# cristianpjensen/thesis-pai-reconstruction

Hardware: AMD Instinct MI355X
Metric: train images/sec (256x256, bs=64) Pix2Pix step (higher is better)
Workload: dtype bf16; 1 GPU; Pix2Pix generator+PatchGAN GAN step, 256x256x1 pairs, 64 images/GPU (BASELINE configs[1]); global_batch=64, per_gpu_batch=64, loss_type=gan, parallelism=dp1, grad_bucket_dtype=f32

## Files before the change

### include/pai_hip.h

```cpp
#ifndef PAI_HIP_H
#define PAI_HIP_H

#include <stdint.h>

#ifdef __cplusplus
extern "C" {
#endif

#define PAI_F32 0
#define PAI_BF16 1
#define PAI_U8 2

#define PAI_ACT_NONE 0
#define PAI_ACT_LRELU 1
#define PAI_ACT_RELU 2
#define PAI_ACT_TANH 3
#define PAI_ACT_SILU 4

const char* pai_last_error(void);
int pai_version(void);
int pai_build_flags(void);
int pai_device_info(int* cu_count, int* lds_bytes, char* arch_name, int arch_name_len);

#define PAI_TUNABLE_UNSET (-2147483647 - 1)
int pai_set_tunable(const char* name, int value);
int pai_get_tunable(const char* name, int default_value);

int64_t pai_order_dependent_launches(void);

typedef struct pai_conv_desc {
    int32_t dtype;
    int32_t transposed;
    int32_t N, H, W;
    int32_t C1, C2;
    int32_t Cout;
    int32_t kernel;
    int32_t stride;
    int32_t pad;
    int32_t relu1, relu2;
    int32_t epilogue_act;
    int32_t groups;
    int32_t pack_flags;
    int32_t hints;
} pai_conv_desc;
#define PAI_HINT_SOLO 1

int pai_conv_out_hw(const pai_conv_desc* d, int* OH, int* OW);
int pai_conv_fwd_stats_rows(const pai_conv_desc* d);
int pai_conv_fwd_stats_rows_max(const pai_conv_desc* d);
int pai_bn_stats_buffer_rows(int rows);

int pai_conv_kernel_id(const pai_conv_desc* d, int op);
int pai_conv_kernel_name(const pai_conv_desc* d, int op, char* name, int name_len);

int pai_create(int device_id, void** handle_out);
int pai_bind(void* handle);
int pai_destroy(void* handle);
int pai_handle_set_workspace(void* handle, void* zeroed_device_memory, int64_t bytes);
int pai_handle_set_scratch(void* handle, void* device_memory, int64_t bytes);
int pai_handle_set_wgrad_workspace(void* handle, void* device_memory, int64_t bytes);

int pai_set_workspace(void* zeroed_device_memory, int64_t bytes);
int64_t pai_conv_workspace_bytes(const pai_conv_desc* d, int op);
int pai_set_scratch(void* device_memory, int64_t bytes);
int64_t pai_conv_scratch_bytes(const pai_conv_desc* d, int op);
int pai_set_wgrad_workspace(void* device_memory, int64_t bytes);
int64_t pai_conv_wgrad_workspace_bytes(const pai_conv_desc* d);
int pai_conv_wgrad_order_free(const pai_conv_desc* d, int has_dbias);

int pai_conv_fwd(const pai_conv_desc* d, const void* x1, const void* x2, const void* w_fwd,
                 const float* bias, void* y_raw, void* y_act, float* y_f32, float* stats,
                 void* stream);

int pai_conv_dgrad(const pai_conv_desc* d, const void* dy, const void* w_dgrad, void* dx1,
                   void* dx2, int only_c2, void* stream);

int pai_conv_dgrad_f32add_ok(const pai_conv_desc* d);
int pai_conv_dgrad_f32add(const pai_conv_desc* d, const void* dy, const void* w_dgrad, const float* addend,
                          float* dx2_f32, void* stream);

int pai_conv_dgrad_act(const pai_conv_desc* d, const void* dy, const void* w_dgrad, void* dx1,
                       void* dx2, const void* a1, int act1, void* stream);

int pai_conv_dgrad_act_wthin_ok(const pai_conv_desc* d, const pai_conv_desc* d_thin, int need_dx);
int pai_conv_dgrad_act_wthin_order_free(const pai_conv_desc* d, const pai_conv_desc* d_thin);
int64_t pai_conv_dgrad_act_wthin_slab_bytes(const pai_conv_desc* d, const pai_conv_desc* d_thin);
int pai_conv_dgrad_act_wthin_kernel_name(const pai_conv_desc* d, const pai_conv_desc* d_thin, char* name, int name_len);
int pai_conv_dgrad_act_wthin(const pai_conv_desc* d, const void* dy, const void* w_dgrad, const void* a1, int act1,
                             const void* add, int act2, const pai_conv_desc* d_thin, const void* x1, const void* x2,
                             float* dw, float* dbias, int overwrite, float* slabs, int64_t slab_bytes, void* stream);

typedef struct pai_bwd_epilogue {
    const void* z;
    const void* add;
    const float* scale;
    const float* shift;
    const float* mean;
    const float* rstd;
    float* partials;
    int32_t act1, act2;
} pai_bwd_epilogue;
int pai_conv_dgrad_bn_rows_max(const pai_conv_desc* d);
int pai_conv_dgrad_bn(const pai_conv_desc* d, const void* dy, const void* w_dgrad, void* dx1,
                      void* dx2, const pai_bwd_epilogue* e, int* partial_rows, void* stream);

typedef struct pai_bn_train {
// ... 108 lines not shown

int pai_gate_partial_rows(int64_t M);
int pai_gate_hidden(int dtype, const void* ig, const void* sg, int64_t M, int K, const float* scale_i,
                    const float* shift_i, const float* scale_s, const float* shift_s, const float* w_a,
                    const float* b_a, void* h, float* logit, float* partials, void* stream);
int pai_gate_apply(int dtype, const void* x, const float* logit, int64_t M, int C, const float* scale_a,
                   const float* shift_a, void* out, float* att, void* stream);
int pai_gate_apply_bwd(int dtype, const void* dout, const void* x, const float* att, const float* logit,
                       int64_t M, int C, const float* mean_a, const float* rstd_a, void* dx_skip, float* dl,
                       float* partials, int relu_out, void* stream);
int pai_gate_hidden_bwd(int dtype, const float* dl, const float* logit, const void* h, const void* ig,
                        const void* sg, int64_t M, int K, const float* mean_a, const float* rstd_a,
                        const float* gamma_a, const float* sums_a, const float* w_a, const float* mean_i,
                        const float* rstd_i, const float* mean_s, const float* rstd_s, void* dsum,
                        float* partials_i, float* partials_s, float* dw_a, float* db_a, void* stream);
int64_t pai_gate_scratch_bytes(int64_t M, int K);

int pai_bce_logits(const float* logits, int64_t numel, float target, float loss_scale,
                   double* loss, float grad_scale, float* grad, void* stream);
int pai_l1(const float* pred, const float* target, int64_t numel, float loss_scale, double* loss,
           float grad_scale, float* grad, void* stream);
int pai_mse(const float* pred, const float* target, int64_t numel, float loss_scale, double* loss,
            float grad_scale, float* grad, void* stream);
int pai_head_loss_ok(const pai_conv_desc* d, int has_bias);
int pai_head_loss(const pai_conv_desc* d, const void* a3, const void* w_fwd, const void* w_dgrad, int n_first,
                  float target_first, float target_rest, float loss_scale, double* loss, float grad_scale,
                  float* logits, void* dl, float* dl_f32, void* du, const void* act_src, int act, void* stream);
int pai_scalar_take(double* acc, float* out, void* stream);
int pai_metrics_take(double* sums, int64_t n_images, int64_t numel, float* out3, void* stream);
int pai_tanh_bwd(int dtype, const float* pred, const float* g_a, const float* g_b, int64_t numel,
                 void* dh, void* stream);

int pai_denormalize(const float* x, const float* grad_out_or_null, int64_t numel, float* out,
                    void* stream);

int pai_ssim_sse(const float* pred, const float* target, int NC, int H, int W, int denorm,
                 double* out2, double* per_image, float* full_map, void* stream);
int pai_ssim_psnr_bwd(const float* pred, const float* target, int NC, int H, int W, int denorm,
                      float w_ssim, float w_psnr, const double* sse, float* grad, float* workspace,
                      void* stream);
int64_t pai_ssim_bwd_workspace_floats(int NC, int H, int W);
int pai_eval_planes(const float* pred, const float* target, int NC, int H, int W, int denorm,
                    double* ssim_plane, double* sse_plane, unsigned char* ssim_map_u8,
                    const unsigned char* lut_rgb, unsigned char* hot_u8, void* stream);
int pai_eval_kernel_name(int op, char* name, int name_len);

int pai_cast(int src_dtype, const void* src, int dst_dtype, void* dst, int64_t numel, void* stream);
int pai_reduce_rows(const float* partial, int rows, int C, float* out, int accumulate, void* stream);
int pai_adam(float* param, const float* grad, float* exp_avg, float* exp_avg_sq, int64_t numel,
             float lr, float beta1, float beta2, float eps, int step_count, void* stream);
int pai_adam_pack(float* param, const float* grad, float* exp_avg, float* exp_avg_sq, int64_t numel, int64_t w_off,
                  int Cout, int taps, int Cin, void* w_fwd, void* w_dgrad, float lr, float beta1, float beta2, float eps,
                  int step_count, void* stream);
int pai_adam_dev(float* param, const float* grad, float* exp_avg, float* exp_avg_sq, int64_t numel,
                 float lr, float beta1, float beta2, float eps, int64_t* step_dev, float* coeff2_dev, void* stream);
int pai_adam_multi(int count, void* const* params, const void* const* grads, void* const* exp_avgs,
                   void* const* exp_avg_sqs, const int64_t* numels, float lr, float beta1, float beta2, float eps,
                   int step_count, void* stream);
int pai_adam_multi_dev(int count, void* const* params, const void* const* grads, void* const* exp_avgs,
                       void* const* exp_avg_sqs, const int64_t* numels, float lr, float beta1, float beta2, float eps,
                       int64_t* step_dev, float* coeff2_dev, void* stream);

#define PAI_COMM_ID_BYTES 128
int pai_comm_unique_id(void* id_out_host);
int pai_comm_init(const void* id_host, int rank, int world, void** comm_out);
int pai_allreduce(void* comm, void* ptr, int64_t count, int dtype, void* stream);
int pai_comm_destroy(void* comm);

typedef struct pai_plan_s* pai_plan_t;
int pai_plan_create(pai_plan_t* out);
int pai_plan_destroy(pai_plan_t plan);
int pai_plan_begin(pai_plan_t plan);
int pai_plan_end(pai_plan_t plan);
int pai_plan_run(pai_plan_t plan, int64_t step_delta);
int pai_plan_info(pai_plan_t plan, int* launches, int* waits, int* streams, int64_t* runs);
int pai_stream_wait(void* waiting_stream, void* signalling_stream);
int pai_stream_wait_last(void* waiting_stream, void* signalling_stream);
typedef struct pai_event_s* pai_event_t;
int pai_event_create(pai_event_t* out);
int pai_event_destroy(pai_event_t ev);
int pai_event_record(pai_event_t ev, void* stream);
int pai_event_create_timing(pai_event_t* out);
int pai_event_elapsed_ms(pai_event_t start, pai_event_t stop, float* ms_host);
int pai_profile_arm(pai_event_t start, pai_event_t stop);
int pai_stream_wait_event(void* waiting_stream, pai_event_t ev);
int pai_zero_multi(int count, void* const* ptrs, const int64_t* numels, void* stream);
int pai_cast_multi(int count, int src_dtype, const void* const* srcs, int dst_dtype, void* const* dsts,
                   const int64_t* numels, void* stream);
int pai_lerp_multi(int count, void* const* dsts, const void* const* srcs, const int64_t* numels, float weight, void* stream);

int pai_filter_to_dense(const float* w_oihw, int Cout, int Cin_per_group, int taps, int groups, float* dense, void* stream);
int pai_filter_grad_from_dense(const float* dense_dw, int Cout, int Cin_per_group, int taps, int groups, float* dw_oihw,
                               void* stream);

int pai_swap_mid(int elem_bytes, const void* src, int64_t A, int B, int C, int64_t D, void* dst, void* stream);
int pai_scale(float* ptr, int64_t numel, float factor, void* stream);

int pai_resize_aa_u8(const void* src, int n, int H, int W, int S, const int* wbounds, const float* wweights, int KW,
                     const int* hbounds, const float* hweights, int KH, const int* hbounds_host, void* dst, void* stream);
int pai_batch_gather(int src_dtype, const void* cache_a, const void* cache_b, int64_t M, int64_t per_image,
                     const int64_t* indices, int count, const float* table, float* out_a, float* out_b, void* stream);
int pai_data_kernel_name(int op, int src_dtype, char* name, int name_len);

int pai_sattn_fwd(int dtype, const void* qkv, int N, int T, int heads, int ch, void* out, void* stream);
int pai_sattn_fwd_lse(int dtype, const void* qkv, int N, int T, int heads, int ch, void* out, float* lse, void* stream);
int pai_sattn_bwd(int dtype, const void* dout, const void* qkv, const void* out, const float* lse, int N, int T, int heads,
// ... 68 lines not shown
```

### thesis-pai-reconstruction_amd/attention.py

```python
from __future__ import annotations

import torch
import torch.nn as nn

from . import ops
from .engine import GradArena, UnetEngine, _BNState, _Packs, _bn_forward, to_fwd_pack_, wthin_slabs
from .ops import ACT_LRELU, ACT_NONE, ACT_RELU, ACT_TANH


class _Gate:

    def __init__(self, block: nn.Module, gen):
        self.conv_i, self.bn_i = block.input_gate[0], block.input_gate[1]
        self.conv_s, self.bn_s = block.signal_gate[0], block.signal_gate[1]
        self.conv_a, self.bn_a = block.attention[0], block.attention[1]
        self.C = self.conv_i.weight.shape[1]
        self.K = self.conv_i.weight.shape[0]
        self.pack_i = _Packs(self.conv_i, need_dgrad=True, gen=gen)
        self.pack_s = _Packs(self.conv_s, need_dgrad=True, gen=gen)

    def ordered_params(self):
        return [(self.conv_a.weight, None), (self.conv_a.bias, None), (self.bn_a.weight, None), (self.bn_a.bias, None),
                (self.bn_i.weight, None), (self.bn_i.bias, None), (self.bn_s.weight, None), (self.bn_s.bias, None),
                (self.conv_i.weight, None), (self.conv_i.bias, None), (self.conv_s.weight, None),
                (self.conv_s.bias, None)]


class AttentionUnetEngine(UnetEngine):
    overwrites_weight_grads = True

    def __init__(self, unet: nn.Module):
        super().__init__(unet)
        self.gates = [_Gate(b, self.weights_generation) for b in unet.attention_blocks]
        assert len(self.gates) == self.L - 1

    def all_packs(self):
        return self.enc_packs + self.dec_packs + [pk for g in self.gates for pk in (g.pack_i, g.pack_s)]

    def _gate(self, j):
        return self.gates[j - 1]

    def ordered_params(self):
        out = []
        L = self.L
        for j in range(L - 1, -1, -1):
            if self.dec_bn[j] is not None:
                out += [(self.dec_bn[j].weight, None), (self.dec_bn[j].bias, None)]
            out += [(self.dec_conv[j].weight, self.dec_conv[j]), (self.dec_conv[j].bias, None)]
            if j >= 1:
                out += self._gate(j).ordered_params()
        for i in range(L - 1, -1, -1):
            if self.enc_bn[i] is not None:
                out += [(self.enc_bn[i].weight, None), (self.enc_bn[i].bias, None)]
            out += [(self.enc_conv[i].weight, self.enc_conv[i]), (self.enc_conv[i].bias, None)]
        return out

    def _plan(self, N, H, W, dtype, device):
        key = (N, H, W, dtype, str(device))
        if key in self._plans:
            return self._plans[key]
        P = super()._plan(N, H, W, dtype, device)
        L = self.L
        eh, ew = P["eh"], P["ew"]
        P["dec_desc"] = []
        for j in range(L):
            hin, win = eh[L - 1 - j], ew[L - 1 - j]
            if j == 0:
                c1, c2, r1, r2 = self.enc_c[L - 1], 0, 1, 0
            else:
                c1, c2, r1, r2 = self.dec_c[j - 1], self.enc_c[L - 1 - j], 1, 1
            act = ACT_NONE
            if j == L - 1:
                r1, r2, act = 0, 0, ACT_TANH
            P["dec_desc"].append(ops.make_desc(dtype, 1, N, hin, win, c1, c2, self.dec_c[j], 2, r1, r2, act))
        P["gate_desc"] = [None]
        rows = P["stats"].numel()
        mx = P["bwd_partials"].numel()
        for j in range(1, L):
            g = self._gate(j)
            lvl = L - 1 - j
            d = ops.make_desc(dtype, 0, N, eh[lvl], ew[lvl], g.C, 0, g.K, 1, 0, 0, ACT_NONE, kernel=1)
            P["gate_desc"].append(d)
            M = N * eh[lvl] * ew[lvl]
            rows = max(rows, ops.bn_stats_buffer_rows(ops.conv_fwd_stats_rows_max(d)) * 2 * g.K,
                       ops.bn_stats_buffer_rows(ops.gate_partial_rows(M)) * 2)
            mx = max(mx, ops.gate_partial_rows(M) * 2 * g.K, ops.conv_dgrad_bn_rows_max(d) * 2 * g.C)
        P["stats"] = torch.empty(rows, dtype=torch.float32, device=device)
        P["bwd_partials"] = torch.empty(mx, dtype=torch.float32, device=device)
        P["bwd_partials2"] = torch.empty(mx, dtype=torch.float32, device=device)
        ops.ensure_workspace(max(ops.conv_workspace_bytes(d, op) for d in P["dec_desc"] + P["gate_desc"][1:]
                                 for op in (0, 1)), device)
        ops.ensure_scratch(ops.scratch_bytes_for(P["enc_desc"] + P["dec_desc"]), device)
        ops.ensure_wgrad_workspace(P["enc_desc"] + P["dec_desc"], device)
        return P

    def _new_slot(self, P):
        S = super()._new_slot(P)
        L, N, dt, dev = self.L, P["N"], P["dtype"], P["device"]
        eh, ew = P["eh"], P["ew"]
        S["b"] = [None] + [torch.empty_like(S["z"][i]) if i < L - 1 else None for i in range(1, L)]
        S["gate"] = [None]
        for j in range(1, L):
            g = self._gate(j)
            lvl = L - 1 - j
            M = N * eh[lvl] * ew[lvl]
            f32 = dict(dtype=torch.float32, device=dev)
            S["gate"].append({
                "M": M,
                "ig": torch.empty(M * g.K, dtype=dt, device=dev), "sg": torch.empty(M * g.K, dtype=dt, device=dev),
                "h": torch.empty(M * g.K, dtype=dt, device=dev), "s": torch.empty(M * g.C, dtype=dt, device=dev),
                "logit": torch.empty(M, **f32), "att": torch.empty(M, **f32),
# ... 84 lines not shown
        for j in range(L):
            wf, _ = self.dec_packs[j].get(dtype)
            d = P["dec_desc"][j]
            if j == 0:
                x1, x2 = S["z"][L - 1], None
            else:
                x1 = S["r"][j - 1]
                x2 = self._gate_forward(S, j, self._skip(S, L - 1 - j), x1, training, bn_updates, dtype)
            if j < L - 1:
                bn = self.dec_bn[j]
                M = N * S["dh"][j] * S["dw"][j]
                if training:
                    rows = ops.conv_fwd_stats_rows(d)
                    ops.conv_fwd(d, x1, x2, wf, self.dec_conv[j].bias, y_raw=S["w"][j], stats=P["stats"])
                    _bn_forward(bn, S["dbn"][j], P["stats"], rows, M, True, bn_updates)
                else:
                    ops.conv_fwd(d, x1, x2, wf, self.dec_conv[j].bias, y_raw=S["w"][j])
                    _bn_forward(bn, S["dbn"][j], None, 0, M, False, 0)
                ops.bn_apply(dtype, S["w"][j], M, self.dec_c[j], S["dbn"][j].scale, S["dbn"][j].shift, ACT_NONE,
                             S["r"][j])
                if training and self.dec_drop[j] > 0:
                    self._dropout(S, j, M, self.dec_c[j], dtype)
            else:
                S["pred"] = torch.empty_like(S["pred"])
                ops.conv_fwd(d, x1, x2, wf, self.dec_conv[j].bias, y_f32=S["pred"])
        pred = S["pred"]
        if self.out_ch != 1:
            pred = pred.view(N, H, W, self.out_ch).permute(0, 3, 1, 2)
        return pred, S

    def backward(self, S, gpred: torch.Tensor, fresh: bool = False):
        P = S["P"]
        L, N, dtype = self.L, P["N"], P["dtype"]
        eh, ew = P["eh"], P["ew"]
        G = self._grad_bufs(S)
        A = self.arena()
        hook = self.grad_ready_hook
        if self.out_ch != 1:
            gpred = gpred.permute(0, 2, 3, 1)
        gpred = gpred.contiguous()
        if gpred.dtype != torch.float32:
            gpred = gpred.float()
        side = self._side
        part, part2 = P["bwd_partials"], P["bwd_partials2"]

        def done(p):
            if hook is not None:
                hook(A, A.end_of(p))

        def wgrad(d, x1, x2, dz, conv, with_bias, last=None):
            cin, cout = conv.weight.shape[1], conv.weight.shape[0]
            dense = fresh and conv.weight.shape[2] == 4 and min(cin, cout) > 2
            with torch.cuda.stream(side.fork(d)):
                (ops.conv_wgrad_overwrite_w if dense else ops.conv_wgrad)(
                    d, x1, x2, dz, A.seg(conv.weight), A.seg(conv.bias) if with_bias else None)
                done(last if last is not None else conv.bias)

        def gate_backward(j, relu_out):
            g, gs = self._gate(j), S["gate"][j]
            d, M = P["gate_desc"][j], gs["M"]
            lvl = L - 1 - j
            x, signal = self._skip(S, lvl), S["r"][j - 1]
            ba, bi, bs = gs["bn_a"], gs["bn_i"], gs["bn_s"]
            ops.gate_apply_bwd(dtype, G["gs"][j], x, gs["att"], gs["logit"], M, g.C, ba.mean, ba.rstd, G["dxs"][j],
                               G["dl"][j], part, relu_out)
            ops.bn_bwd_finalize(part, ops.gate_partial_rows(M), 1, ba.sums, A.seg(g.bn_a.weight), A.seg(g.bn_a.bias))
            ops.gate_hidden_bwd(dtype, G["dl"][j], gs["logit"], gs["h"], gs["ig"], gs["sg"], M, g.K, ba.mean, ba.rstd,
                                g.bn_a.weight, ba.sums, g.conv_a.weight, bi.mean, bi.rstd, bs.mean, bs.rstd,
                                G["dsum"][j], part, part2, A.seg(g.conv_a.weight), A.seg(g.conv_a.bias))
            rows = ops.gate_partial_rows(M)
            ops.bn_bwd_finalize(part, rows, g.K, bi.sums, A.seg(g.bn_i.weight), A.seg(g.bn_i.bias))
            ops.bn_bwd_finalize(part2, rows, g.K, bs.sums, A.seg(g.bn_s.weight), A.seg(g.bn_s.bias))
            ops.bn_bwd_apply(dtype, G["dsum"][j], gs["ig"], M, g.K, bi.mean, bi.rstd, g.bn_i.weight, bi.sums, G["dig"][j])
            ops.bn_bwd_apply(dtype, G["dsum"][j], gs["sg"], M, g.K, bs.mean, bs.rstd, g.bn_s.weight, bs.sums, G["dsg"][j])
            wgrad(d, x, None, G["dig"][j], g.conv_i, False)
            wgrad(d, signal, None, G["dsg"][j], g.conv_s, False)
            _, wd_i = g.pack_i.get(dtype)
            _, wd_s = g.pack_s.get(dtype)
            ops.conv_dgrad_bn(d, G["dig"][j], wd_i, G["gx"][j], None, x, ACT_NONE, G["dxs"][j], ACT_NONE)
            pst = S["dbn"][j - 1]
            if (j - 1) in S["drop"]:
                ops.conv_dgrad_bn(d, G["dsg"][j], wd_s, G["gr"][j - 1], None, S["r"][j - 1], ACT_NONE,
                                  G["gr_raw"][j - 1], ACT_RELU if relu_out else ACT_NONE)
                ops.dropout2d(dtype, G["gr"][j - 1], S["drop"][j - 1], N, S["dh"][j - 1] * S["dw"][j - 1],
                              self.dec_c[j - 1], G["gr"][j - 1])
                return None
            return ops.conv_dgrad_bn(d, G["dsg"][j], wd_s, G["gr"][j - 1], None, S["w"][j - 1], ACT_NONE,
                                     G["gr_raw"][j - 1], ACT_RELU if relu_out else ACT_NONE, pst.scale, pst.shift,
                                     pst.mean, pst.rstd, part)

        j = L - 1
        dh = G["dz_head"]
        ops.tanh_bwd(dtype, S["pred"], gpred, None, dh)
        d = P["dec_desc"][j]
        wgrad(d, S["r"][j - 1], S["gate"][j]["s"], dh, self.dec_conv[j], True)
        side.mark_scratch()
        _, wd = self.dec_packs[j].get(dtype)
        ops.conv_dgrad(d, dh, wd, G["gr_raw"][j - 1], G["gs"][j])
        fused_rows = gate_backward(j, relu_out=False)
        for j in range(L - 2, -1, -1):
            bn, st, conv = self.dec_bn[j], S["dbn"][j], self.dec_conv[j]
            M = N * S["dh"][j] * S["dw"][j]
            C = self.dec_c[j]
            dz = G["dz_dec"][j]
            du = G["gr"][j]
            if fused_rows is None:
                du = G["du"][:M * C]
                ops.bn_bwd_reduce(dtype, G["gr"][j], ACT_NONE, None, ACT_NONE, None, S["w"][j], M, C, st.mean, st.rstd,
                                  du, part, st.sums, A.seg(bn.weight), A.seg(bn.bias))
            else:
                ops.bn_bwd_finalize(part, fused_rows, C, st.sums, A.seg(bn.weight), A.seg(bn.bias))
            ops.bn_bwd_apply(dtype, du, S["w"][j], M, C, st.mean, st.rstd, bn.weight, st.sums, dz)
            d = P["dec_desc"][j]
            _, wd = self.dec_packs[j].get(dtype)
            if j == 0:
                wgrad(d, S["z"][L - 1], None, dz, conv, False)
                fused_rows = ops.conv_dgrad_bn(d, dz, wd, G["dz_enc"][L - 1], None, S["z"][L - 1], ACT_RELU)
            else:
                wgrad(d, S["r"][j - 1], S["gate"][j]["s"], dz, conv, False)
                ops.conv_dgrad(d, dz, wd, G["gr_raw"][j - 1], G["gs"][j])
                fused_rows = gate_backward(j, relu_out=True)
        i = L - 1
        dz = G["dz_enc"][i]
        wgrad(P["enc_desc"][i], S["a"][i - 1], None, dz, self.enc_conv[i], True)
        _, wd = self.enc_packs[i].get(dtype)

        enc0_fused = ops.conv_dgrad_act_wthin_ok(P["enc_desc"][1], P["enc_desc"][0], False)

        def enc_dgrad(i, dz, wd):
            d = P["enc_desc"][i]
            gx = G["gx"][L - 1 - (i - 1)]
            if i - 1 == 0 and enc0_fused:
                c0, d0 = self.enc_conv[0], P["enc_desc"][0]
                ops.conv_dgrad_act_wthin(d, dz, wd, S["z"][0], ACT_LRELU, gx, ACT_NONE, d0, S["x"], None,
                                         A.seg(c0.weight), A.seg(c0.bias), wthin_slabs(P, d, d0))
                return 0
            if i - 1 == 0:
                if G["dz_enc"][0] is None:
                    G["dz_enc"][0] = torch.empty_like(S["z"][0])
                return ops.conv_dgrad_bn(d, dz, wd, G["dz_enc"][0], None, S["z"][0], ACT_LRELU, gx, ACT_NONE)
            pst = S["ebn"][i - 1]
            return ops.conv_dgrad_bn(d, dz, wd, G["ga"][i - 1], None, S["z"][i - 1], ACT_LRELU, gx, ACT_NONE,
                                     pst.scale, pst.shift, pst.mean, pst.rstd, part)

        fused_rows = enc_dgrad(i, dz, wd)
        for i in range(L - 2, 0, -1):
            bn, st, conv = self.enc_bn[i], S["ebn"][i], self.enc_conv[i]
            M = N * eh[i] * ew[i]
            C = self.enc_c[i]
            du, dz = G["ga"][i], G["dz_enc"][i]
            ops.bn_bwd_finalize(part, fused_rows, C, st.sums, A.seg(bn.weight), A.seg(bn.bias))
            ops.bn_bwd_apply(dtype, du, S["z"][i], M, C, st.mean, st.rstd, bn.weight, st.sums, dz)
            wgrad(P["enc_desc"][i], S["a"][i - 1], None, dz, conv, False)
            _, wd = self.enc_packs[i].get(dtype)
            fused_rows = enc_dgrad(i, dz, wd)
        conv0 = self.enc_conv[0]
        if not enc0_fused:
            with torch.cuda.stream(side.fork_tail()):
                c0_in, c0_out = conv0.weight.shape[1], conv0.weight.shape[0]
                (ops.conv_wgrad_overwrite_w if (fresh and min(c0_in, c0_out) > 2) else ops.conv_wgrad)(
                    P["enc_desc"][0], S["x"], None, G["dz_enc"][0], A.seg(conv0.weight), A.seg(conv0.bias))
        side.join()
        done(conv0.bias)
```

### thesis-pai-reconstruction_amd/csrc/api.hip

```cpp
#include <stdarg.h>

#include "common.h"

static thread_local char g_err[512] = "";

void pai_set_error(const char* fmt, ...) {
    va_list ap;
    va_start(ap, fmt);
    vsnprintf(g_err, sizeof(g_err), fmt, ap);
    va_end(ap);
}

extern "C" const char* pai_last_error(void) { return g_err; }
extern "C" int pai_version(void) { return 141; }

extern "C" int pai_build_flags(void) { return 0; }

extern "C" int pai_device_info(int* cu_count, int* lds_bytes, char* arch_name, int arch_name_len) {
    int dev = 0;
    hipError_t e = hipGetDevice(&dev);
    PAI_CHECK(e == hipSuccess, "hipGetDevice: %s", hipGetErrorString(e));
    hipDeviceProp_t p;
    e = hipGetDeviceProperties(&p, dev);
    PAI_CHECK(e == hipSuccess, "hipGetDeviceProperties: %s", hipGetErrorString(e));
// ... 120 lines not shown
    g->S = S;
    g->nphase = 1;
    g->ntaps = 16;
    g->OS = 1;
    g->poy[0] = g->pox[0] = 0;
    for (int kh = 0; kh < 4; ++kh)
        for (int kw = 0; kw < 4; ++kw) {
            int t = kh * 4 + kw;
            g->dy[0][t] = (signed char)(kh + off0);
            g->dx[0][t] = (signed char)(kw + off0);
            g->wt[0][t] = (signed char)t;
        }
}

static void fill_pointwise(GG* g) {
    g->S = 1; g->nphase = 1; g->ntaps = 1; g->OS = 1; g->wtaps = 1;
    g->poy[0] = g->pox[0] = 0;
    g->dy[0][0] = g->dx[0][0] = g->wt[0][0] = 0;
}

static void fill_3x3(GG* g, int sign) {
    g->S = 1; g->nphase = 1; g->ntaps = 9; g->OS = 1; g->wtaps = 9;
    g->poy[0] = g->pox[0] = 0;
    for (int kh = 0; kh < 3; ++kh)
        for (int kw = 0; kw < 3; ++kw) {
            const int t = kh * 3 + kw;
            g->dy[0][t] = (signed char)(sign * (kh - 1));
            g->dx[0][t] = (signed char)(sign * (kw - 1));
            g->wt[0][t] = (signed char)t;
        }
}

static void fill_phase_taps(GG* g) {
    g->S = 1;
    g->nphase = 4;
    g->ntaps = 4;
    g->OS = 2;
    for (int ph = 0; ph < 2; ++ph)
        for (int pw = 0; pw < 2; ++pw) {
            int p = ph * 2 + pw;
            g->poy[p] = (signed char)ph;
            g->pox[p] = (signed char)pw;
            int khs[2], offy[2], kws[2], offx[2];
            phase_taps(ph, khs, offy);
            phase_taps(pw, kws, offx);
            for (int a = 0; a < 2; ++a)
                for (int b = 0; b < 2; ++b) {
                    int t = a * 2 + b;
                    g->dy[p][t] = (signed char)offy[a];
                    g->dx[p][t] = (signed char)offx[b];
                    g->wt[p][t] = (signed char)(khs[a] * 4 + kws[b]);
                }
        }
}

int gg_build_fwd(const pai_conv_desc* d, GG* g) {
    if (check_desc(d)) return 1;
    memset(g, 0, sizeof(*g));
    g->N = d->N; g->H = d->H; g->W = d->W;
    g->C1 = d->C1; g->C2 = d->C2; g->Cin = d->C1 + d->C2;
    g->Cout = d->Cout;
    g->D1 = d->Cout; g->D2 = 0;
    g->wtaps = 16;
    g->gslice = d->groups > 1 ? 16 : 0;
    g->solo = (d->hints & PAI_HINT_SOLO) ? 1 : 0;
    g->relu1 = d->relu1; g->relu2 = d->relu2;
    int OH, OW;
    pai_conv_out_hw(d, &OH, &OW);
    g->OH = OH; g->OW = OW;
    if (d->kernel == 1) {
        g->OHg = OH; g->OWg = OW;
        fill_pointwise(g);
    } else if (d->kernel == 3) {
        g->OHg = OH; g->OWg = OW;
        fill_3x3(g, +1);
    } else if (!d->transposed) {
        g->OHg = OH; g->OWg = OW;
        fill_conv_taps(g, d->stride, -d->pad);
    } else {
        g->OHg = d->H; g->OWg = d->W;
        fill_phase_taps(g);
    }
    finish_gg(g);
    return 0;
}

int gg_build_dgrad(const pai_conv_desc* d, GG* g) {
    if (check_desc(d)) return 1;
    memset(g, 0, sizeof(*g));
    int OH, OW;
    pai_conv_out_hw(d, &OH, &OW);
    g->N = d->N; g->H = OH; g->W = OW;
    g->C1 = d->Cout; g->C2 = 0; g->Cin = d->Cout;
    g->Cout = d->C1 + d->C2;
    g->D1 = d->C1; g->D2 = d->C2;
    g->wtaps = 16;
    g->gslice = d->groups > 1 ? 16 : 0;
    g->OH = d->H; g->OW = d->W;
    if (d->kernel == 1) {
        g->OHg = d->H; g->OWg = d->W;
        fill_pointwise(g);
    } else if (d->kernel == 3) {
        g->OHg = d->H; g->OWg = d->W;
        fill_3x3(g, -1);
    } else if (!d->transposed) {
        if (d->stride == 2) {
            g->OHg = d->H / 2; g->OWg = d->W / 2;
            fill_phase_taps(g);
        } else {
            g->OHg = d->H; g->OWg = d->W;
            g->S = 1; g->nphase = 1; g->ntaps = 16; g->OS = 1;
            for (int kh = 0; kh < 4; ++kh)
                for (int kw = 0; kw < 4; ++kw) {
                    int t = kh * 4 + kw;
                    g->dy[0][t] = (signed char)(d->pad - kh);
                    g->dx[0][t] = (signed char)(d->pad - kw);
                    g->wt[0][t] = (signed char)t;
                }
        }
    } else {
        g->OHg = d->H; g->OWg = d->W;
        fill_conv_taps(g, 2, -d->pad);
    }
    finish_gg(g);
    return 0;
}

static void finish_gg(GG* g) {
    g->M = g->N * g->OHg * g->OWg;
    auto lg = [](int v) { int l = 0; while ((1 << l) < v) ++l; return (1 << l) == v ? l : -1; };
    g->lw = lg(g->OWg);
    g->lh = lg(g->OHg);
    if (g->lw < 0 || g->lh < 0) g->lw = g->lh = -1;
    g->lsw = lg(g->W); g->lsh = lg(g->H); g->ldw = lg(g->OW); g->ldh = lg(g->OH);
    if (g->lw < 0 || g->lsw < 0 || g->lsh < 0 || g->ldw < 0 || g->ldh < 0)
        g->lsw = g->lsh = g->ldw = g->ldh = -1;
}

constexpr int PAI_MAX_DEVICES = 64;
static pai_handle_s* g_active[PAI_MAX_DEVICES];
static const pai_handle_s g_empty_handle = {-1, nullptr, 0, nullptr, 0, nullptr, 0};

static int current_device() {
    int dev = 0;
    return hipGetDevice(&dev) == hipSuccess && dev >= 0 && dev < PAI_MAX_DEVICES ? dev : -1;
}

const pai_handle_s* pai_ctx() {
    const int dev = current_device();
    return dev >= 0 && g_active[dev] ? g_active[dev] : &g_empty_handle;
}

extern "C" int pai_create(int device_id, void** handle_out) {
    PAI_CHECK(handle_out != nullptr, "pai_create: null handle_out");
    PAI_CHECK(device_id >= 0 && device_id < PAI_MAX_DEVICES, "pai_create: device id %d out of range", device_id);
    pai_handle_s* h = new pai_handle_s{device_id, nullptr, 0, nullptr, 0, nullptr, 0};
    if (!g_active[device_id]) g_active[device_id] = h;
    *handle_out = h;
    return 0;
}

extern "C" int pai_bind(void* handle) {
    PAI_CHECK(handle != nullptr, "pai_bind: null handle");
    pai_handle_s* h = (pai_handle_s*)handle;
    g_active[h->device] = h;
    return 0;
}

extern "C" int pai_destroy(void* handle) {
    PAI_CHECK(handle != nullptr, "pai_destroy: null handle");
    pai_handle_s* h = (pai_handle_s*)handle;
    if (g_active[h->device] == h) g_active[h->device] = nullptr;
    delete h;
    return 0;
}

// ... 191 lines not shown
    memset(&a, 0, sizeof(a));
    a.y1 = (void*)1;
    if (op == 1 && g.D2 > 0) a.y2 = (void*)1;
    return a;
}

extern "C" int64_t pai_conv_wgrad_workspace_bytes(const pai_conv_desc* d) {
    GG g;
    if (gg_build_fwd(d, &g)) return -1;
    return pick_wgrad(d->dtype, g, false, false).workspace_bytes;
}

extern "C" int pai_conv_wgrad_order_free(const pai_conv_desc* d, int has_dbias) {
    GG g;
    if (!d || gg_build_fwd(d, &g)) return 0;
    return pick_wgrad(d->dtype, g, has_dbias != 0, false).order_free ? 1 : 0;
}

extern "C" int64_t pai_conv_workspace_bytes(const pai_conv_desc* d, int op) {
    GG g;
    if (op == 1 ? gg_build_dgrad(d, &g) : gg_build_fwd(d, &g)) return -1;
    return op == 2 ? 0 : pick_fwd(d->dtype, g, query_args(g, op)).workspace_bytes;
}

extern "C" int64_t pai_conv_scratch_bytes(const pai_conv_desc* d, int op) {
    GG g;
    if (op == 1 ? gg_build_dgrad(d, &g) : gg_build_fwd(d, &g)) return -1;
    return op == 2 ? pick_wgrad(d->dtype, g, false, false).scratch_bytes : pick_fwd(d->dtype, g, query_args(g, op)).scratch_bytes;
}

extern "C" int pai_conv_fwd_stats_rows(const pai_conv_desc* d) {
    GG g;
    if (gg_build_fwd(d, &g)) return -1;
    FwdArgs a = query_args(g, 0);
    a.stats = (float*)1;
    return pick_fwd(d->dtype, g, a).rows;
}

extern "C" int pai_conv_kernel_id(const pai_conv_desc* d, int op) {
    GG g;
    if (op == 1 ? gg_build_dgrad(d, &g) : gg_build_fwd(d, &g)) return -1;
    return op == 2 ? pick_wgrad(d->dtype, g, false, false).id : pick_fwd(d->dtype, g, query_args(g, op)).id;
}

extern "C" int pai_conv_kernel_name(const pai_conv_desc* d, int op, char* name, int name_len) {
    GG g;
    if ((op == 1 ? gg_build_dgrad(d, &g) : gg_build_fwd(d, &g)) || !name || name_len <= 0) return -1;
    const char* n = op == 2 ? pick_wgrad(d->dtype, g, false, false).name : pick_fwd(d->dtype, g, query_args(g, op)).name;
    strncpy(name, n, name_len - 1);
    name[name_len - 1] = 0;
    return 0;
}

extern "C" int pai_conv_fwd_stats_rows_max(const pai_conv_desc* d) {
    GG g;
    if (gg_build_fwd(d, &g)) return -1;
    return cdiv(g.M, 16) * g.nphase;
}

extern "C" int pai_conv_fwd(const pai_conv_desc* d, const void* x1, const void* x2,
                            const void* w_fwd, const float* bias, void* y_raw, void* y_act,
                            float* y_f32, float* stats, void* stream) {
    GG g;
    if (gg_build_fwd(d, &g)) return 1;
    PAI_CHECK(x1 && w_fwd, "pai_conv_fwd: null x1 / w");
    PAI_CHECK(d->C2 == 0 || x2, "pai_conv_fwd: C2 > 0 but x2 is null");
    PAI_CHECK(y_raw || y_act || y_f32, "pai_conv_fwd: no output requested");
    FwdArgs a;
    memset(&a, 0, sizeof(a));
    a.x1 = x1; a.x2 = x2; a.w = w_fwd; a.bias = bias;
    a.y1 = y_raw; a.y2 = nullptr; a.yact = y_act; a.yf32 = y_f32; a.stats = stats;
    a.eact = d->epilogue_act;
    return run_fwd(d->dtype, g, a, (hipStream_t)stream);
}

static int conv_wgrad_impl(const pai_conv_desc* d, const void* x1, const void* x2, const void* dy, float* dw,
                           float* dbias, int overwrite, void* stream, const float* pscale = nullptr,
                           const float* pshift = nullptr, int pact = 0);

extern "C" int pai_conv_prologue_ok(const pai_conv_desc* d) {
    GG g;
    if (gg_build_fwd(d, &g)) return 0;
    FwdArgs a = query_args(g, 0);
    a.pscale = a.pshift = (const float*)1;
    a.pact = PAI_ACT_RELU;
    return pick_fwd(d->dtype, g, a).k != FK_NONE && pick_wgrad(d->dtype, g, false, true).k != WK_NONE;
}

extern "C" int pai_conv_fwd_pro(const pai_conv_desc* d, const void* x1, const void* w_fwd, const float* bias, void* y_raw,
                                float* stats, const float* pre_scale, const float* pre_shift, int pre_act, void* stream) {
    GG g;
    if (gg_build_fwd(d, &g)) return 1;
    PAI_CHECK(x1 && w_fwd && y_raw && pre_scale && pre_shift, "pai_conv_fwd_pro: null pointer");
    PAI_CHECK(pre_act == PAI_ACT_NONE || pre_act == PAI_ACT_RELU, "pai_conv_fwd_pro: pre_act=%d (none or ReLU)", pre_act);
    PAI_CHECK(d->C2 == 0, "pai_conv_fwd_pro: one source tensor only");
    FwdArgs a;
    memset(&a, 0, sizeof(a));
    a.x1 = x1; a.w = w_fwd; a.bias = bias;
    a.y1 = y_raw;
    a.stats = stats;
    a.pscale = pre_scale; a.pshift = pre_shift; a.pact = pre_act;
    return run_fwd(d->dtype, g, a, (hipStream_t)stream);
}

extern "C" int pai_conv_wgrad_pro(const pai_conv_desc* d, const void* x1, const void* dy, float* dw, float* dbias,
                                  int overwrite, const float* pre_scale, const float* pre_shift, int pre_act, void* stream) {
// ... 262 lines not shown
                                       e->rstd, gamma, dz, s);
    if (int rc = pai_bn_bwd_finalize(e->partials, rows, g.D1, sums, dgamma, dbeta, stream)) return rc;
    return pai_bn_bwd_apply(d->dtype, du_scratch, e->z, Mo, g.D1, e->mean, e->rstd, gamma, sums, dz, stream);
}


extern "C" int pai_conv_wgrad(const pai_conv_desc* d, const void* x1, const void* x2,
                              const void* dy, float* dw, float* dbias, void* stream) {
    return conv_wgrad_impl(d, x1, x2, dy, dw, dbias, 0, stream);
}

extern "C" int pai_conv_wgrad_overwrite(const pai_conv_desc* d, const void* x1, const void* x2,
                                        const void* dy, float* dw, float* dbias, void* stream) {
    return conv_wgrad_impl(d, x1, x2, dy, dw, dbias, 1, stream);
}

extern "C" int pai_conv_wgrad_overwrite_w(const pai_conv_desc* d, const void* x1, const void* x2,
                                          const void* dy, float* dw, float* dbias, void* stream) {
    return conv_wgrad_impl(d, x1, x2, dy, dw, dbias, 2, stream);
}

static int conv_wgrad_impl(const pai_conv_desc* d, const void* x1, const void* x2, const void* dy, float* dw,
                           float* dbias, int overwrite, void* stream, const float* pscale, const float* pshift, int pact) {
    GG g;
    if (gg_build_fwd(d, &g)) return 1;
    PAI_CHECK(x1 && dy && dw, "pai_conv_wgrad: null pointer");
    PAI_CHECK(d->C2 == 0 || x2, "pai_conv_wgrad: C2 > 0 but x2 is null");
    WgradArgs a;
    a.x1 = x1; a.x2 = x2; a.dy = dy; a.dw = dw; a.dbias = dbias; a.overwrite = 0; a.overwrite_bias = 0; a.slab = nullptr;
    a.pscale = pscale; a.pshift = pshift; a.pact = pact;
    hipStream_t s = (hipStream_t)stream;
    const WgradPick p = pick_wgrad(d->dtype, g, dbias != nullptr, pscale != nullptr);
    PAI_CHECK(p.k != WK_NONE, "pai_conv_wgrad_pro: this layer takes no prologue (ask pai_conv_prologue_ok: the grouped 3 x 3 weight "
                              "gradient needs its workspace, pai_set_wgrad_workspace)");
    float* bias_rows = nullptr;
    if (pai_deterministic()) {
        const pai_handle_s* h = pai_ctx();
        const bool thin = p.k >= WK_THIN_CONV && p.k <= WK_THIN_CONV3T;
        PAI_CHECK(!thin || (h->scratch && h->scratch_bytes >= p.scratch_bytes),
                  "pai_conv_wgrad: deterministic mode needs %lld bytes of scratch for the partial tiles of this thin layer "
                  "(pai_set_scratch; pai_conv_scratch_bytes, op 2)", (long long)p.scratch_bytes);
        const int64_t dwb = (int64_t)g.Cout * g.wtaps * g.Cin * 4;
        const int64_t slabs = p.k == WK_GROUPED3 ? grouped3_wgrad_part_bytes(g)
                              : (p.k == WK_MFMA && p.mfma.variant < WGRAD_PATCH128 && p.mfma.ksplit > 1) ? p.mfma.ksplit * dwb : 0;
        const int64_t rows = p.colsum_bias ? p.bias_part_bytes : 0;
        const int64_t have = h->wslab ? h->wslab_bytes & ~(int64_t)3 : 0;
        PAI_CHECK(slabs + rows == 0 || have >= slabs + rows,
                  "pai_conv_wgrad: deterministic mode needs %lld bytes of weight-gradient workspace (%lld for the pixel-split slabs, "
                  "%lld for the partial rows of the bias gradient; pai_set_wgrad_workspace, pai_conv_wgrad_workspace_bytes)",
                  (long long)(slabs + rows), (long long)slabs, (long long)rows);
        if (rows) bias_rows = (float*)((char*)h->wslab + (have - rows));
    }
    if (overwrite && p.overwrites) {
        a.overwrite = 1;
        a.overwrite_bias = p.k != WK_GROUPED3 && overwrite == 1;
    } else if (overwrite) {
        hipError_t e = pai::memset_async(dw, 0, (size_t)g.Cout * g.wtaps * g.Cin * sizeof(float), s);
        PAI_CHECK(e == hipSuccess, "pai_conv_wgrad_overwrite: hipMemsetAsync: %s", hipGetErrorString(e));
        if (dbias && overwrite == 1) {
            e = pai::memset_async(dbias, 0, (size_t)g.Cout * sizeof(float), s);
            PAI_CHECK(e == hipSuccess, "pai_conv_wgrad_overwrite: hipMemsetAsync: %s", hipGetErrorString(e));
        }
    }
    if (!p.order_free) pai_note_order_dependent();
    if (p.colsum_bias) {
        if (int rc = launch_colsum_det(d->dtype, dy, (int64_t)g.N * g.OH * g.OW, g.Cout, dbias, overwrite != 1, bias_rows, s)) return rc;
        a.dbias = nullptr;
    }
    switch (p.k) {
        case WK_GROUPED3: return launch_grouped3_wgrad(g, a, p.part, s);
        case WK_THIN_CONV: return launch_thin_wgrad_conv(g, a, s);
        case WK_THIN_CONVT: return launch_thin_wgrad_convt(g, a, s);
        case WK_THIN_CONV1: return launch_thin_wgrad_conv1(g, a, s);
        case WK_THIN_CONV3: return launch_thin_wgrad_conv3(g, a, s);
        case WK_THIN_CONV3T: return launch_thin_wgrad_conv3t(g, a, s);
        case WK_ROWDOT: return launch_wgrad_rowdot(d->dtype, g, a, s);
        case WK_MFMA: return launch_wgrad_mfma(g, a, p.mfma, s);
        default: return launch_wgrad_simt(d->dtype, g, a, s);
    }
}
```

### thesis-pai-reconstruction_amd/csrc/common.h

```cpp
#pragma once
#include <hip/hip_runtime.h>
#include <stdint.h>
#include <stdio.h>
#include <string.h>

#include "../../include/pai_hip.h"
#include "plan.h"

typedef unsigned short bf16_t;

void pai_set_error(const char* fmt, ...);

#define PAI_CHECK(cond, ...)                 \
    do {                                     \
        if (!(cond)) {                       \
            pai_set_error(__VA_ARGS__);      \
            return 1;                        \
        }                                    \
    } while (0)

#define PAI_LAUNCH_CHECK()                                              \
    do {                                                                \
        hipError_t e_ = hipGetLastError();                              \
        if (e_ != hipSuccess) {                                         \
// ... 68 lines not shown
__device__ __forceinline__ float act_apply(float v, int act) {
    switch (act) {
        case PAI_ACT_LRELU: return v > 0.f ? v : 0.2f * v;
        case PAI_ACT_RELU: return !(v <= 0.f) ? v : 0.f;
        case PAI_ACT_TANH: return tanhf(v);
        default: return v;
    }
}
__device__ __forceinline__ float act_grad(float a, int act) {
    switch (act) {
        case PAI_ACT_LRELU: return a > 0.f ? 1.f : 0.2f;
        case PAI_ACT_RELU: return a > 0.f ? 1.f : 0.f;
        default: return 1.f;
    }
}

__device__ __forceinline__ float wave_sum(float v) {
#pragma unroll
    for (int o = 32; o > 0; o >>= 1) v += __shfl_xor(v, o, 64);
    return v;
}

static inline int cdiv(int64_t a, int64_t b) { return (int)((a + b - 1) / b); }

struct PerDeviceOnce {
    bool done[32] = {};
    bool first() {
        int dev = 0;
        if (hipGetDevice(&dev) != hipSuccess || dev < 0 || dev >= 32) return true;
        if (done[dev]) return false;
        done[dev] = true;
        return true;
    }
};

struct GG {
    int N, H, W;
    int C1, C2, Cin;
    int OHg, OWg;
    int Cout;
    int S;
    int nphase, ntaps;
    int OH, OW, OS;
    int D1, D2;
    int wtaps;
    int relu1, relu2;
    int M;
    int lw, lh;
    int lsw, lsh, ldw, ldh;
    signed char dy[4][16], dx[4][16], wt[4][16];
    signed char poy[4], pox[4];
    int gslice;
    int solo;
};

struct PatchGeo {
    int groups;
    int TY, TX;
    signed char by[4][4], bx[4][4];
    unsigned toff4[4][4];
    unsigned wt4[4][4];
    unsigned wt_lo[4], wt_hi[4], toff2[4];
};

int gg_build_fwd(const pai_conv_desc* d, GG* g);
int gg_build_dgrad(const pai_conv_desc* d, GG* g);

struct FwdArgs {
    const void *x1, *x2, *w;
    const float* bias;
    void *y1, *y2;
    void* yact;
    float* yf32;
    float* stats;
    int eact;
    int skip_d1;
    const void* bz;
    const void* badd;
    const float *bscale, *bshift, *bmean, *brstd;
    int bact1, bact2;
    float* bpart;
    const float *pscale, *pshift;
    int pact;
};
bool bn_fuse_small_ok(int rows, int64_t M, int C);
int launch_bn_fin_apply(int dtype, const float* stats, int rows, int C, int64_t count, const float* gamma, const float* beta,
                        float eps, float momentum, int n_updates, float* running_mean, float* running_var, int64_t* nbt,
                        float* mean, float* rstd, float* scale, float* shift, const void* z, int act, void* out,
                        hipStream_t s);
int launch_bn_bwd_fin_apply(int dtype, const float* partials, int rows, int C, float* sums, float* dgamma, float* dbeta,
                            const void* du, const void* z, int64_t M, const float* mean, const float* rstd,
                            const float* gamma, void* dz, hipStream_t s);
int ew_stream_bn_apply(int dtype, const void* z, int64_t M, int C, const float* scale, const float* shift, int act, void* out,
                       hipStream_t s);
int ew_stream_bn2_add_act(int dtype, const void* za, const float* sca, const float* sha, const void* zb, const float* scb,
                          const float* shb, int64_t M, int C, int act_a, int act, void* out, hipStream_t s);
int ew_stream_add_act(int dtype, const void* a, const void* b, int64_t numel, int act, void* out, hipStream_t s);
int ew_stream_bn_bwd_reduce(int dtype, const void* g, int act, const void* z, int64_t M, int C, const float* scale,
                            const float* shift, const float* mean, const float* rstd, float* partials, int rows, hipStream_t s);
int ew_stream_bn_bwd_apply(int dtype, const void* g, int act, const void* z, int64_t M, int C, const float* scale,
                           const float* shift, const float* mean, const float* rstd, const float* gamma, const float* sums,
                           void* dz, hipStream_t s);
int ew_stream_bn2_bwd_reduce(int dtype, const void* d, int act_a, const void* za, const void* zb, int64_t M, int C,
                             const float* scale_a, const float* shift_a, const float* mean_a, const float* rstd_a,
                             const float* mean_b, const float* rstd_b, float* part_a, float* part_b, int rows, hipStream_t s);
int ew_stream_bn2_bwd_apply(int dtype, const void* d, int act_a, const void* za, const void* zb, int64_t M, int C,
                            const float* scale_a, const float* shift_a, const float* mean_a, const float* rstd_a,
// ... 31 lines not shown
int launch_fwd_mfma(const GG& g, const FwdArgs& a, const MfmaPlan& p, hipStream_t s, const WThin* wt = nullptr);
int launch_wthin_reduce(const float* slab, int S, int T, float* dw, float* dbias, int overwrite_w, int overwrite_bias, hipStream_t s);
MfmaPlan wgrad_mfma_plan(const GG& g, bool has_dbias, bool has_prologue);
bool wgrad_pro_ok(int dtype, const GG& g);
struct pai_handle_s {
    int device;
    float* workspace;
    int64_t workspace_bytes;
    float* scratch;
    int64_t scratch_bytes;
    float* wslab;
    int64_t wslab_bytes;
};
const pai_handle_s* pai_ctx();
int fwd_simt_mtiles(const GG& g);
bool fwd_mfma_ok(int dtype, const GG& g, const FwdArgs& a);
bool pw_ok(int dtype, const GG& g, const FwdArgs& a);
int pw_rows(const GG& g);
int launch_pw(const GG& g, const FwdArgs& a, hipStream_t s);
bool pwx_ok(int dtype, const GG& g, const FwdArgs& a);
int pwx_rows(const GG& g);
int launch_pwx(const GG& g, const FwdArgs& a, hipStream_t s);
const char* pwx_kernel_name(const GG& g);
bool fwd_rowdot_ok(const GG& g, const FwdArgs& a);
bool small_ok(int dtype, const GG& g, const FwdArgs& a);
int small_rows(const GG& g);
int launch_small(const GG& g, const FwdArgs& a, hipStream_t s);
bool grouped3_ok(int dtype, const GG& g, const FwdArgs& a);
int grouped3_rows(const GG& g);
int launch_grouped3(const GG& g, const FwdArgs& a, hipStream_t s);

bool thin_fwd_ok(int dtype, const GG& g, const FwdArgs& a);
bool thin_dgrad_ok(int dtype, const GG& g, const FwdArgs& a);
bool thin_dgrad_shape_ok(int dtype, const GG& g);
int64_t thin_dgrad_scratch_bytes(const GG& g, const FwdArgs& a);
int launch_thin_fwd(const GG& g, const FwdArgs& a, hipStream_t s);
bool head_dgrad_ok(int dtype, const GG& g, const FwdArgs& a);
int launch_head_dgrad(const GG& g, const FwdArgs& a, hipStream_t s);
int thin_fwd_bwd_rows(int dtype, const GG& g, const FwdArgs& a, int act1, const void* add, const float* scale);
int launch_thin_dgrad(const GG& g, const FwdArgs& a, hipStream_t s);
bool thin_up_f32add_ok(int dtype, const GG& g);

struct WgradArgs {
    const void *x1, *x2, *dy;
    float* dw;
    float* dbias;
    int overwrite;
    int overwrite_bias;
    float* slab;
    const float *pscale, *pshift;
    int pact;
};
float* wgrad_slab_acquire(int64_t bytes);
int launch_wgrad_slab_sum(float* dw, const float* slab, int nsplits, int64_t n, int overwrite, hipStream_t s);
bool grouped3_wgrad_ok(int dtype, const GG& g, const float* dbias);
int64_t grouped3_wgrad_part_bytes(const GG& g);
int launch_grouped3_wgrad(const GG& g, const WgradArgs& a, float* part, hipStream_t s);
int launch_eval_planes(const float* pred, const float* target, int NC, int H, int W, int denorm, double* ssim_plane,
                       double* sse_plane, unsigned char* map_u8, const unsigned char* lut_rgb, unsigned char* hot_u8,
                       hipStream_t stream);
const char* eval_planes_kernel_name();
bool wgrad3_ok(const GG& g);
MfmaPlan wgrad3_plan(const GG& g, bool has_dbias);
int launch_wgrad3(const GG& g, const WgradArgs& a, const MfmaPlan& p, hipStream_t s);
int wgrad_simt_splits(const GG& g, int* rows);
int launch_wgrad_simt(int dtype, const GG& g, const WgradArgs& a, hipStream_t s);
int launch_wgrad_rowdot(int dtype, const GG& g, const WgradArgs& a, hipStream_t s);
int launch_wgrad_mfma(const GG& g, const WgradArgs& a, const MfmaPlan& p, hipStream_t s);
bool wgrad_mfma_ok(int dtype, const GG& g);
bool thin_wgrad_conv_ok(int dtype, const GG& g);
bool thin_wgrad_convt_ok(int dtype, const GG& g);
int launch_thin_wgrad_conv(const GG& g, const WgradArgs& a, hipStream_t s);
int launch_thin_wgrad_convt(const GG& g, const WgradArgs& a, hipStream_t s);
bool thin_wgrad_conv1_ok(int dtype, const GG& g);
int launch_thin_wgrad_conv1(const GG& g, const WgradArgs& a, hipStream_t s);
bool thin_wgrad_conv3_ok(int dtype, const GG& g);
int launch_thin_wgrad_conv3(const GG& g, const WgradArgs& a, hipStream_t s);
bool thin_wgrad_conv3t_ok(int dtype, const GG& g);
int launch_thin_wgrad_conv3t(const GG& g, const WgradArgs& a, hipStream_t s);
int64_t thin_wgrad_scratch_bytes(int64_t M, int T, int WC);
```

### thesis-pai-reconstruction_amd/csrc/gg_mfma.hip

```cpp
#include <type_traits>

#include "gg_tile.h"


bool fwd_mfma_ok(int dtype, const GG& g, const FwdArgs& a) {
    if (dtype != PAI_BF16) return false;
    if (g.C1 % 64 || g.C2 % 64) return false;
    if (g.Cout % 64) return false;
    if (g.D2 > 0 && (g.D1 % 64)) return false;
    if (a.yf32) return false;
    if (a.skip_d1) return false;
    if ((a.y1 || a.y2) && a.yact) return false;
    if (a.yact && a.eact != PAI_ACT_NONE && a.eact != PAI_ACT_LRELU && a.eact != PAI_ACT_RELU) return false;
    return true;
}

struct FwdCfg { int bn, ksplit; };

static FwdCfg fwd_cfg(const GG& g) {
    FwdCfg c;
    c.bn = ((g.Cout % 128) == 0 && (g.D2 == 0 || (g.D1 % 128) == 0)) ? 128 : 64;
    c.ksplit = 1;
    const int ntiles = g.Cout / c.bn;
    const int niter = g.ntaps * g.Cin / MBK;
// ... 1035 lines not shown
        p.block = waves * 64;
        const size_t lds = patch_bytes + (size_t)c.bn * 128 * (db ? 2 : 1);
        const size_t epi = prow * ((size_t)c.bn * 2 + 16) + waves * 2 * c.bn * sizeof(float);
        p.lds = lds > epi ? lds : epi;
    } else {
        p.block = p.bm / 64 * 128;
        p.lds = fwd_lds_bytes(p.bm, c.bn, db);
    }
    p.grid = p.mtiles * p.ntiles * g.nphase * c.ksplit;
    return p;
}

bool fwd_mfma_wthin(MfmaPlan* p, int T) {
    if (p->variant != FWD_PATCH128N || p->ntiles != 1 || (T != 1 && T != 2)) return false;
    p->variant = T == 1 ? FWD_WTHIN1 : FWD_WTHIN2;
    p->name = fwd_mfma_names[p->variant];
    const size_t epi = 128 * (64 * 2 + 16) + 4 * 2 * 64 * sizeof(float) + (size_t)T * WTH_XPLANE;
    if (epi > p->lds) p->lds = epi;
    return true;
}

static int fwd_lds_opt_in();
int launch_fwd_mfma(const GG& g, const FwdArgs& a, const MfmaPlan& p, hipStream_t s, const WThin* wt) {
    float* ws = pai_ctx()->workspace;
    const bool wthin = p.variant == FWD_WTHIN1 || p.variant == FWD_WTHIN2;
    PAI_CHECK(wthin == (wt != nullptr), "launch_fwd_mfma: the weight-gradient store and its arguments go together");
    const WThin wta = wt ? *wt : WThin{};
    if (p.lds > 64 * 1024 && fwd_lds_opt_in()) return 1;
#define FWD_LAUNCH_TILE(k, ...) PAI_LAUNCH((k<__VA_ARGS__>), p.grid, p.block, p.lds, s, g, a, p.mtiles, p.ntiles, p.ksplit, ws)
#define FWD_LAUNCH_PATCH(k, ...) PAI_LAUNCH((k<__VA_ARGS__>), p.grid, p.block, p.lds, s, g, a, p.pg, p.mtiles, p.ntiles)
#define FWD_LAUNCH_WTHIN(k, ...) PAI_LAUNCH((k<__VA_ARGS__>), p.grid, p.block, p.lds, s, g, a, p.pg, p.mtiles, p.ntiles, wta)
#define X(id, form, k, ...) case id: FWD_LAUNCH_##form(k, __VA_ARGS__); break;
    switch (p.variant) { FWD_MFMA_VARIANTS(X) }
#undef X
#undef FWD_LAUNCH_TILE
#undef FWD_LAUNCH_PATCH
#undef FWD_LAUNCH_WTHIN
    PAI_LAUNCH_CHECK();
    if (p.ksplit > 1)
        PAI_LAUNCH(splitk_finish_k, dim3(p.rows, g.nphase, cdiv(g.Cout, FIN_COLS)), dim3(256), 0, s, g, a, ws, p.rows, p.ksplit);
    PAI_LAUNCH_CHECK();
    return 0;
}
static int fwd_lds_opt_in() {
    static PerDeviceOnce attr_set;
    if (!attr_set.first()) return 0;
    const hipError_t e = hipFuncSetAttribute(reinterpret_cast<const void*>(&gg_fwd_patch_k<256, 128, true>),
                                             hipFuncAttributeMaxDynamicSharedMemorySize, 80 * 1024);
    PAI_CHECK(e == hipSuccess, "hipFuncSetAttribute(max dynamic LDS): %s", hipGetErrorString(e));
    return 0;
}

bool pw_ok(int dtype, const GG& g, const FwdArgs& a) {
    if (dtype != PAI_BF16 || g.ntaps != 1 || g.nphase != 1 || g.C2 != 0 || g.D2 != 0) return false;
    if (!((g.C1 == 64 && g.Cout == 32) || (g.C1 == 32 && g.Cout == 64))) return false;
    if (a.yf32 || a.skip_d1) return false;
    if ((a.y1 != nullptr) == (a.yact != nullptr)) return false;
    if (a.yact && a.eact != PAI_ACT_NONE && a.eact != PAI_ACT_LRELU && a.eact != PAI_ACT_RELU) return false;
    return true;
}

int pw_rows(const GG& g) {
    int64_t b = ((int64_t)g.M + 63) / 64;
    return (int)(b > 2048 ? 2048 : (b < 1 ? 1 : b));
}

template <int CIN, int COUT>
__global__ __launch_bounds__(256) void pw_k(GG g, FwdArgs a, int groups_per_wave) {
    constexpr int KB = CIN / 32, NTT = COUT / 16, CL = COUT / 4, NCH = CL / 8;
    __shared__ float sred[4][2][COUT];
    const int tid = threadIdx.x, lane = tid & 63, wid = tid >> 6;
    const int fr = lane & 15, fq = lane >> 4;
    const bf16_t* x = (const bf16_t*)a.x1;
    const bf16_t* w = (const bf16_t*)a.w;
    bf16_t* y = (bf16_t*)(a.yact ? a.yact : a.y1);
    const float eslope = act_slope(a.yact ? a.eact : PAI_ACT_NONE);
    bf8_t wf[NTT][KB];
#pragma unroll
    for (int nt = 0; nt < NTT; ++nt)
#pragma unroll
        for (int kb = 0; kb < KB; ++kb)
            wf[nt][kb] = *(const bf8_t*)(w + (size_t)(CL * (fr >> 2) + 4 * nt + (fr & 3)) * CIN + kb * 32 + fq * 8);
    const int c0 = CL * fq;
    float bias_v[CL], s1[CL], s2[CL];
#pragma unroll
    for (int c = 0; c < CL; ++c) { bias_v[c] = a.bias ? a.bias[c0 + c] : 0.f; s1[c] = s2[c] = 0.f; }
    const bool bwd = a.bz != nullptr && !a.yact;
    const bool bsum = bwd && a.bpart;
    const bf16_t* bzp = (const bf16_t*)a.bz;
    const bf16_t* bap = (const bf16_t*)a.badd;
    BwdParams BP[NCH];
    if (bwd) {
#pragma unroll
        for (int h = 0; h < NCH; ++h) bwd_load_params(a, c0 + 8 * h, BP[h]);
    }
    const int64_t ngroups = ((int64_t)g.M + 15) / 16;
    const int64_t g0 = ((int64_t)blockIdx.x * 4 + wid) * groups_per_wave;
    for (int64_t gi = g0; gi < g0 + groups_per_wave && gi < ngroups; ++gi) {
        const int64_t pix = gi * 16 + fr;
        const bool valid = pix < g.M;
        const int64_t pc = valid ? pix : 0;
        bf8_t xb[KB];
#pragma unroll
        for (int kb = 0; kb < KB; ++kb) {
            xb[kb] = *(const bf8_t*)(x + pc * CIN + kb * 32 + fq * 8);
            if (g.relu1) xb[kb] = relu_frag(xb[kb]);
        }
// ... 25 lines not shown
            }
            pk[2 * nt] = pk2bf(v[0], v[1]);
            pk[2 * nt + 1] = pk2bf(v[2], v[3]);
        }
#pragma unroll
        for (int h = 0; h < NCH; ++h) {
            uint4 o = make_uint4(pk[4 * h], pk[4 * h + 1], pk[4 * h + 2], pk[4 * h + 3]);
            if (bwd && valid)
                o = bwd_chunk(o, zq[h], aq[h], bap != nullptr, a.bscale != nullptr, bsum, a.bact1, a.bact2, BP[h],
                              s1 + 8 * h, s2 + 8 * h);
            if (valid) *(uint4*)(y + pix * COUT + c0 + 8 * h) = o;
        }
    }
    float* prow = a.stats ? a.stats : (bsum ? a.bpart : nullptr);
    if (prow) {
#pragma unroll
        for (int c = 0; c < CL; ++c) {
            float u = s1[c], q = s2[c];
            u += __builtin_bit_cast(float, __builtin_amdgcn_update_dpp(0, __builtin_bit_cast(int, u), 0xB1, 0xF, 0xF, false));
            q += __builtin_bit_cast(float, __builtin_amdgcn_update_dpp(0, __builtin_bit_cast(int, q), 0xB1, 0xF, 0xF, false));
            u += __builtin_bit_cast(float, __builtin_amdgcn_update_dpp(0, __builtin_bit_cast(int, u), 0x4E, 0xF, 0xF, false));
            q += __builtin_bit_cast(float, __builtin_amdgcn_update_dpp(0, __builtin_bit_cast(int, q), 0x4E, 0xF, 0xF, false));
            u += __builtin_bit_cast(float, __builtin_amdgcn_update_dpp(0, __builtin_bit_cast(int, u), 0x141, 0xF, 0xF, false));
            q += __builtin_bit_cast(float, __builtin_amdgcn_update_dpp(0, __builtin_bit_cast(int, q), 0x141, 0xF, 0xF, false));
            u += __builtin_bit_cast(float, __builtin_amdgcn_update_dpp(0, __builtin_bit_cast(int, u), 0x140, 0xF, 0xF, false));
            q += __builtin_bit_cast(float, __builtin_amdgcn_update_dpp(0, __builtin_bit_cast(int, q), 0x140, 0xF, 0xF, false));
            if (fr == 0) { sred[wid][0][c0 + c] = u; sred[wid][1][c0 + c] = q; }
        }
        __syncthreads();
        if (tid < COUT) {
            float u = 0.f, q = 0.f;
#pragma unroll
            for (int wv = 0; wv < 4; ++wv) { u += sred[wv][0][tid]; q += sred[wv][1][tid]; }
            float* dst = prow + (size_t)blockIdx.x * 2 * COUT;
            dst[tid] = u;
            dst[COUT + tid] = a.stats ? q : a.brstd[tid] * (q - a.bmean[tid] * u);
        }
    }
}

int launch_pw(const GG& g, const FwdArgs& a, hipStream_t s) {
    const int blocks = pw_rows(g);
    const int64_t ngroups = ((int64_t)g.M + 15) / 16;
    const int gpw = (int)((ngroups + (int64_t)blocks * 4 - 1) / ((int64_t)blocks * 4));
    if (g.C1 == 64) PAI_LAUNCH((pw_k<64, 32>), dim3(blocks), dim3(256), 0, s, g, a, gpw);
    else PAI_LAUNCH((pw_k<32, 64>), dim3(blocks), dim3(256), 0, s, g, a, gpw);
    PAI_LAUNCH_CHECK();
    return 0;
}

bool wgrad_mfma_ok(int dtype, const GG& g) {
    if (dtype != PAI_BF16) return false;
    if (g.lsw < 0) return false;
    if (g.ntaps == 1 && g.C2 == 0 && ((g.C1 == 64 && g.Cout == 32) || (g.C1 == 32 && g.Cout == 64))) return true;
    if (g.ntaps == 1 && g.C2 == 0 && g.C1 == 64 && (g.Cout % 64) == 0) return true;
    if (g.nphase == 1 && g.S == 1 && g.C2 == 0 && (g.C1 % 8) == 0 && (g.Cout % 8) == 0 && (g.C1 < 64 || g.Cout < 64))
        return true;
    if (g.C1 % 64 || g.C2 % 64) return false;
    if (g.Cout % 64) return false;
    return true;
}

__device__ __forceinline__ int tr_swz(int row) { return ((row & 3) << 2) | ((row >> 2) & 3); }
__device__ __forceinline__ unsigned tr_off(int row, int ch) { return (unsigned)(256 * row + 16 * (ch ^ tr_swz(row))); }

template <int BMC>
__global__ __launch_bounds__(256) void gg_wgrad_mfma_k(GG g, WgradArgs a, int cotiles, int jtiles,
                                                       int splits, int rows_per_split, int stage_lds) {
    constexpr int MT = BMC / 32;
    constexpr int BUF = 64 * 256;
    extern __shared__ __attribute__((aligned(16))) unsigned char smem[];
    unsigned char* Ys = smem;
    unsigned char* Xs = smem + BUF;

    const int tid = threadIdx.x, lane = tid & 63;
    const int wid = __builtin_amdgcn_readfirstlane(tid >> 6);
    const int wm = wid >> 1, wn = wid & 1;
    int bid = xcd_remap(blockIdx.x, gridDim.x);
    const int jt = bid % jtiles; bid /= jtiles;
    const int cot = bid % cotiles; bid /= cotiles;
    const int split = bid % splits;
    const int ph = bid / splits;
    const int co0 = cot * BMC, j0 = jt * 128;
    const bool stage_out = stage_lds != 0;

    const bf16_t* x1 = (const bf16_t*)a.x1;
    const bf16_t* x2 = (const bf16_t*)a.x2;
    const bf16_t* dy = (const bf16_t*)a.dy;
    const bf16_t* zero = (const bf16_t*)g_zero_line;

    const int sc = lane & 15, sr = wid * 4 + (lane >> 4);
    const int gch = sc ^ tr_swz(sr);
    const int J = g.ntaps * g.Cin;
    const bool xvalid = j0 + gch * 8 < J;
    const int jc = xvalid ? j0 + gch * 8 : 0;
    const int xt = jc / g.Cin;
    const int xci = jc - xt * g.Cin;
    const int ddy = g.dy[ph][xt], ddx = g.dx[ph][xt];
    const bf16_t* xsrc;
    int xcs, xcc, xrelu;
    if (xci < g.C1) { xsrc = x1; xcs = g.C1; xcc = xci; xrelu = g.relu1; }
    else { xsrc = x2; xcs = g.C2; xcc = xci - g.C1; xrelu = g.relu2; }
    const bool yvalid = gch < BMC / 8 && (co0 + gch * 8) < g.Cout;
    const bool relu_any = g.relu1 || g.relu2;

    const int mbeg = split * rows_per_split;
    const int mend = min(g.M, mbeg + rows_per_split);
    const int niter = (mend - mbeg + 63) / 64;
// ... 404 lines not shown
                    else if (splits == 1) {
                        if (a.overwrite) *pw = acc[mt][nt][r];
                        else *pw += acc[mt][nt][r];
                    } else {
                        atomicAdd(pw, acc[mt][nt][r]);
                    }
                }
            }
        }
    }
}

int launch_colsum(int dtype, const void* x, int64_t rows, int C, float* out, hipStream_t s);

static bool wgrad_patch_shape_ok(const GG& g) {
    const int64_t xb = (int64_t)g.N * g.H * g.W * (g.C1 > g.C2 ? g.C1 : g.C2) * 2, yb = (int64_t)g.N * g.OH * g.OW * g.Cout * 2;
    if (xb >= (1ll << 31) || yb >= (1ll << 31)) return false;
    return g.lw >= 4 && g.lh >= 2 && (g.C1 % 32) == 0 && (g.C2 % 32) == 0 && (g.Cout % 64) == 0 && g.Cin >= 64;
}

static bool wgrad_mfma_uses_patch(const GG& g, PatchGeo* pg) {
    return pai_tunable("wgrad_patch", 1) && wgrad_patch_shape_ok(g) && patch_geo(g, 4, pg);
}

static bool wgrad_mfma_big(const GG& g, bool patch) {
    if ((g.Cout % 128) != 0) return false;
    const int narrow = pai_tunable("wgrad_narrow", 512);
    if (narrow && !patch) {
        const int tiles128 = (g.Cout / 128) * cdiv(g.ntaps * g.Cin, 128) * g.nphase;
        if (tiles128 <= narrow && g.M <= 2048) return false;
    }
    return true;
}

static int wgrad_mfma_splits(const GG& g, bool patch, int tiles, int* rows_out) {
    const int target_tun = pai_tunable("wgrad_target", 0);
    const double gflop = 2.0 * (double)g.M * g.nphase * g.Cout * g.ntaps * g.Cin * 1e-9;
    const int target_def = (patch && gflop >= 100.0) ? 1024 : 512;
    const int target = target_tun ? target_tun : target_def;
    int splits = cdiv(target, tiles);
    const int max_splits = cdiv(g.M, pai_tunable("wgrad_minrows", 512));
    if (splits > max_splits) splits = max_splits;
    if (splits < 1) splits = 1;
    const int unsplit_rows = pai_tunable("wgrad_unsplit_rows", 2048);
    if ((tiles >= 256 && g.M <= unsplit_rows) || (tiles >= 512 && g.M <= 2 * unsplit_rows)) splits = 1;
    if (pai_deterministic()) splits = 1;
    int rows = cdiv(cdiv(g.M, splits), 64) * 64;
    splits = cdiv(g.M, rows);
    *rows_out = rows;
    return splits;
}

bool wgrad_pro_ok(int dtype, const GG& g) {
    return wgrad_mfma_ok(dtype, g) && g.ntaps == 1 && g.nphase == 1 && g.C2 == 0 && !g.gslice && !g.relu1 && !wgrad3_ok(g);
}

MfmaPlan wgrad_mfma_plan(const GG& g, bool has_dbias, bool has_prologue) {
    MfmaPlan p = wgrad3_plan(g, has_dbias);
    if (p.variant) return p;
    const bool patch = wgrad_mfma_uses_patch(g, &p.pg), big = wgrad_mfma_big(g, patch);
    p.bm = big ? 128 : 64;
    p.mtiles = big ? g.Cout / 128 : cdiv(g.Cout, 64);
    p.ntiles = cdiv(g.ntaps * g.Cin, 128);
    const int tiles = p.mtiles * p.ntiles * g.nphase;
    p.ksplit = wgrad_mfma_splits(g, patch, tiles, &p.rows);
    p.overwrites = !patch && p.ksplit == 1;
    p.block = 256;
    if (patch && !has_prologue) {
        p.variant = big ? WGRAD_PATCH128 : WGRAD_PATCH64;
        p.name = big ? "gg_wgrad_patch_k<128>" : "gg_wgrad_patch_k<64>";
        p.rows /= 64;
        p.ksplit = cdiv(g.M / 64, p.rows);
        p.lds = 64 * 256 + 128 * 64;
    } else {
        p.variant = big ? WGRAD_TILE128 : WGRAD_TILE64;
        p.name = big ? "gg_wgrad_mfma_k<128>" : "gg_wgrad_mfma_k<64>";
        p.db = p.ksplit == 1 && g.ntaps == 1 && g.nphase == 1 && (g.Cin % 4) == 0 && !g.gslice && pai_tunable("wgrad_stage", 1) != 0;
        p.lds = p.db ? 64 * 132 * 4 : 2 * 64 * 256;
    }
    p.grid = tiles * p.ksplit;
    return p;
}

int launch_wgrad_mfma(const GG& g, const WgradArgs& a, const MfmaPlan& p, hipStream_t s) {
    if (p.variant < WGRAD_PATCH128) return launch_wgrad3(g, a, p, s);
    const bool tile = p.variant == WGRAD_TILE128 || p.variant == WGRAD_TILE64;
    if (tile && a.overwrite_bias && a.dbias && g.nphase > 1) {
        hipError_t e = pai::memset_async(a.dbias, 0, (size_t)g.Cout * sizeof(float), s);
        PAI_CHECK(e == hipSuccess, "launch_wgrad_mfma: hipMemsetAsync: %s", hipGetErrorString(e));
    }
    switch (p.variant) {
        case WGRAD_PATCH128: PAI_LAUNCH(gg_wgrad_patch_k<128>, p.grid, p.block, p.lds, s, g, a, p.pg, p.mtiles, p.ntiles, p.ksplit, p.rows); break;
        case WGRAD_PATCH64: PAI_LAUNCH(gg_wgrad_patch_k<64>, p.grid, p.block, p.lds, s, g, a, p.pg, p.mtiles, p.ntiles, p.ksplit, p.rows); break;
        case WGRAD_TILE128: PAI_LAUNCH(gg_wgrad_mfma_k<128>, p.grid, p.block, p.lds, s, g, a, p.mtiles, p.ntiles, p.ksplit, p.rows, p.db); break;
        default: PAI_LAUNCH(gg_wgrad_mfma_k<64>, p.grid, p.block, p.lds, s, g, a, p.mtiles, p.ntiles, p.ksplit, p.rows, p.db); break;
    }
    PAI_LAUNCH_CHECK();
    return 0;
}
```

### thesis-pai-reconstruction_amd/csrc/gg_pw.hip

```cpp
#include "common.h"
#include "gg_tile.h"

namespace {
constexpr int PWX_MAX_BLOCKS = 4096;

__device__ __forceinline__ float dpp_add16(float u) {
    u += __builtin_bit_cast(float, __builtin_amdgcn_update_dpp(0, __builtin_bit_cast(int, u), 0xB1, 0xF, 0xF, false));
    u += __builtin_bit_cast(float, __builtin_amdgcn_update_dpp(0, __builtin_bit_cast(int, u), 0x4E, 0xF, 0xF, false));
    u += __builtin_bit_cast(float, __builtin_amdgcn_update_dpp(0, __builtin_bit_cast(int, u), 0x141, 0xF, 0xF, false));
    u += __builtin_bit_cast(float, __builtin_amdgcn_update_dpp(0, __builtin_bit_cast(int, u), 0x140, 0xF, 0xF, false));
    return u;
}
}

bool pwx_shape_ok(int cin, int cout) {
    return (cin == 64 && (cout == 64 || cout == 128 || cout == 256)) || (cin == 128 && (cout == 64 || cout == 128)) ||
           (cin == 256 && cout == 64) ||
           (pai_tunable("pwx_split", 1) && ((cin == 128 && cout == 256) || (cin == 256 && cout == 128)));
}

bool pwx_ok(int dtype, const GG& g, const FwdArgs& a) {
    if (dtype != PAI_BF16 || g.ntaps != 1 || g.nphase != 1 || g.S != 1 || g.OS != 1 || g.gslice) return false;
    if (!pwx_shape_ok(g.Cin, g.Cout) || (g.C1 % 32) || (g.C2 % 32)) return false;
    if (g.D2 ? ((g.D1 % 8) || (g.D2 % 8) || g.D1 + g.D2 != g.Cout) : false) return false;
    if (g.relu1 || g.relu2 || a.yf32 || a.skip_d1) return false;
    if (a.bz && (g.D2 || a.badd || !a.bscale || !a.bshift || a.stats || a.pscale ||
                 (a.bpart && !(a.bmean && a.brstd)) || (a.bact1 != PAI_ACT_NONE && a.bact1 != PAI_ACT_RELU)))
        return false;
    if (a.pscale && (g.C2 || !a.pshift || (a.pact != PAI_ACT_NONE && a.pact != PAI_ACT_RELU))) return false;
    if (!a.y1 || a.yact) return false;
    if ((int64_t)g.M < 16384) return false;
    return pai_tunable("pwx", 1) != 0;
}

int pwx_rows(const GG& g) {
    const int64_t b = ((int64_t)g.M + 255) / 256;
    const int64_t cap = pai_tunable("pwx_blocks", g.M >= (1 << 21) ? PWX_MAX_BLOCKS : 256);
    return (int)(b > cap ? cap : (b < 1 ? 1 : b));
}

template <int CIN, int COUT, int T, int MODE, bool PRE, int NSPLIT = 1>
__global__ __launch_bounds__(256) void pwx_k(GG g, FwdArgs a, int groups_per_wave) {
    constexpr bool STATS = MODE != 0;
    constexpr int KB = CIN / 32, NTT = COUT / 16, CL = COUT / 4, NCH = CL / 8, CALL = COUT * NSPLIT;
    __shared__ __attribute__((aligned(16))) float sbias[CALL];
    __shared__ float sred[4][2][STATS ? COUT : 1];
    __shared__ __attribute__((aligned(16))) float sbwd[3][MODE == 2 ? CALL : 4];
    __shared__ __attribute__((aligned(16))) float spre[2][PRE ? CIN : 4];
    const int tid = threadIdx.x, lane = tid & 63, wid = tid >> 6;
    const int fr = lane & 15, fq = lane >> 4;
    const int cbase = (wid % NSPLIT) * COUT;
    const int pw = wid / NSPLIT;
    const bf16_t* x1 = (const bf16_t*)a.x1;
    const bf16_t* x2 = (const bf16_t*)a.x2;
    const bf16_t* w = (const bf16_t*)a.w + (size_t)cbase * CIN;
    const int C1 = g.C1, C2 = g.C2;
    for (int c = tid; c < CALL; c += 256) sbias[c] = a.bias ? a.bias[c] : 0.f;
    if (PRE) {
        for (int c = tid; c < CIN; c += 256) { spre[0][c] = a.pscale[c]; spre[1][c] = a.pshift[c]; }
    }
    const float plo = a.pact == PAI_ACT_RELU ? 0.f : -INFINITY;
    if (MODE == 2) {
        for (int c = tid; c < CALL; c += 256) {
            sbwd[0][c] = a.bscale[c];
            sbwd[1][c] = a.bshift[c];
            sbwd[2][c] = a.bmean ? a.bmean[c] : 0.f;
        }
    }
    const bf16_t* bzp = (const bf16_t*)a.bz;
    const bool brelu = a.bact1 == PAI_ACT_RELU;
    bf8_t wf[NTT][KB];
#pragma unroll
    for (int nt = 0; nt < NTT; ++nt)
#pragma unroll
        for (int kb = 0; kb < KB; ++kb)
// ... 194 lines not shown
```

### thesis-pai-reconstruction_amd/csrc/gg_tile.h

```cpp
#pragma once
#include <stdlib.h>

#include "common.h"

typedef __attribute__((ext_vector_type(8))) __bf16 bf8_t;
typedef __attribute__((ext_vector_type(4))) __bf16 bf4_t;
typedef __attribute__((ext_vector_type(4))) float f4_t;
typedef __attribute__((ext_vector_type(2))) short s2_t;
typedef __attribute__((ext_vector_type(4))) unsigned u4_t;

constexpr int MBK = 64;

static __device__ uint4 g_zero_line[16];

#define GLDS16(gptr, lptr)                                                                      \
    __builtin_amdgcn_global_load_lds((const __attribute__((address_space(1))) void*)(gptr),    \
                                     (__attribute__((address_space(3))) void*)(lptr), 16, 0, 0)

typedef __attribute__((ext_vector_type(8))) short s8_t;

#ifndef RELU_ABL
#define RELU_ABL 0
#endif
__device__ __forceinline__ bf8_t relu_frag(bf8_t f) {
// ... 74 lines not shown
template <int BN, int CPR, int NW>
__device__ __forceinline__ void bwd_write_partials(float* sred, const float* s1, const float* s2, int tid,
                                                   float* row_dst, int D1, const float* mean, const float* rstd) {
    const int lane = tid & 63, wid = tid >> 6;
#pragma unroll
    for (int k = 0; k < 8; ++k) {
        float a = s1[k], b = s2[k];
#pragma unroll
        for (int o = CPR; o < 64; o <<= 1) { a += __shfl_xor(a, o, 64); b += __shfl_xor(b, o, 64); }
        if (lane < CPR) {
            sred[(wid * 2 + 0) * BN + lane * 8 + k] = a;
            sred[(wid * 2 + 1) * BN + lane * 8 + k] = b;
        }
    }
    __syncthreads();
    if (tid < BN) {
        float a = 0.f, b = 0.f;
#pragma unroll
        for (int w = 0; w < NW; ++w) { a += sred[(w * 2 + 0) * BN + tid]; b += sred[(w * 2 + 1) * BN + tid]; }
        row_dst[tid] = a;
        row_dst[D1 + tid] = rstd[tid] * (b - mean[tid] * a);
    }
}

constexpr int PATCH_W = 17;
template <int BM, int WN = 2, int WPX = 64> struct PatchDims {
    static constexpr int TH = BM / 16;
    static constexpr int PIX = (TH + 1) * PATCH_W;
    static constexpr int NTHR = BM / WPX * 64 * WN;
    static constexpr int RPP = NTHR / 8;
    static constexpr int PJ = (PIX + RPP - 1) / RPP;
    static constexpr int BYTES = PJ * RPP * 128;
};

static inline void patch_geo_pack(PatchGeo* pg) {
    for (int ph = 0; ph < 4; ++ph) {
        pg->wt_lo[ph] = pg->wt_hi[ph] = pg->toff2[ph] = 0;
        for (int q = 0; q < 4; ++q)
            for (int k = 0; k < 4; ++k) {
                const unsigned slot = (pg->wt4[ph][q] >> (8 * k)) & 15u, to = (pg->toff4[ph][q] >> (8 * k)) & 0xffu;
                if (q < 2) pg->wt_lo[ph] |= slot << (16 * q + 4 * k); else pg->wt_hi[ph] |= slot << (16 * (q - 2) + 4 * k);
                pg->toff2[ph] |= ((to / PATCH_W) * 2u + (to % PATCH_W)) << (8 * q + 2 * k);
            }
    }
}
static inline bool patch_geo_raw(const GG& g, int th, PatchGeo* pg, int tw);
static inline bool patch_geo(const GG& g, int th, PatchGeo* pg, int tw = 16) {
    if (!patch_geo_raw(g, th, pg, tw)) return false;
    patch_geo_pack(pg);
    return true;
}
static inline bool patch_geo_raw(const GG& g, int th, PatchGeo* pg, int tw) {
    if ((g.OWg % tw) || (g.OHg % th)) return false;
    memset(pg, 0, sizeof(*pg));
    pg->TY = g.OHg / th;
    pg->TX = g.OWg / tw;
    if (g.S == 1 && g.ntaps == 4) {
        pg->groups = 1;
        for (int ph = 0; ph < g.nphase; ++ph) {
            int by = 127, bx = 127;
            for (int t = 0; t < 4; ++t) { by = g.dy[ph][t] < by ? g.dy[ph][t] : by; bx = g.dx[ph][t] < bx ? g.dx[ph][t] : bx; }
            unsigned seen = 0;
            for (int t = 0; t < 4; ++t) {
                const int ty = g.dy[ph][t] - by, tx = g.dx[ph][t] - bx;
                if (ty > 1 || tx > 1) return false;
                const int k = ty * 2 + tx;
                if (seen & (1u << k)) return false;
                seen |= 1u << k;
                pg->toff4[ph][0] |= (unsigned)(ty * PATCH_W + tx) << (8 * k);
                pg->wt4[ph][0] |= (unsigned)g.wt[ph][t] << (8 * k);
            }
            if (seen != 15u) return false;
            pg->by[ph][0] = (signed char)by;
            pg->bx[ph][0] = (signed char)bx;
        }
        return true;
    }
    if (g.S == 2 && g.ntaps == 16 && g.nphase == 1) {
        pg->groups = 4;
        int ymin = 127, xmin = 127;
        for (int t = 0; t < 16; ++t) { ymin = g.dy[0][t] < ymin ? g.dy[0][t] : ymin; xmin = g.dx[0][t] < xmin ? g.dx[0][t] : xmin; }
        for (int q = 0; q < 4; ++q) {
            const int by = ymin + (q >> 1), bx = xmin + (q & 1);
            int n = 0;
            unsigned seen = 0;
            for (int t = 0; t < 16; ++t) {
                const int ry = g.dy[0][t] - by, rx = g.dx[0][t] - bx;
                if (ry < 0 || rx < 0 || (ry & 1) || (rx & 1)) continue;
                const int ty = ry / 2, tx = rx / 2;
                if (ty > 1 || tx > 1 || n == 4) return false;
                const int k = ty * 2 + tx;
                if (seen & (1u << k)) return false;
                seen |= 1u << k;
                pg->toff4[0][q] |= (unsigned)(ty * PATCH_W + tx) << (8 * k);
                pg->wt4[0][q] |= (unsigned)g.wt[0][t] << (8 * k);
                ++n;
            }
            if (n != 4 || seen != 15u) return false;
            pg->by[0][q] = (signed char)by;
            pg->bx[0][q] = (signed char)bx;
        }
        return true;
    }
    return false;
}

// ... 33 lines not shown
```

### thesis-pai-reconstruction_amd/csrc/misc.hip

```cpp
#include "common.h"

template <typename S, typename D>
__global__ __launch_bounds__(256) void cast_k(const S* src, D* dst, int64_t numel) {
    for (int64_t i = (int64_t)blockIdx.x * 256 + threadIdx.x; i < numel; i += (int64_t)gridDim.x * 256)
        Conv<D>::st(dst + i, Conv<S>::ld(src + i));
}

extern "C" int pai_cast(int src_dtype, const void* src, int dst_dtype, void* dst, int64_t numel,
                        void* stream) {
    PAI_CHECK(src && dst, "pai_cast: null pointer");
    int64_t blocks = (numel + 1023) / 1024;
    if (blocks > 4096) blocks = 4096;
    if (blocks < 1) blocks = 1;
    hipStream_t s = (hipStream_t)stream;
    dim3 g((int)blocks), b(256);
    if (src_dtype == PAI_F32 && dst_dtype == PAI_BF16)
        PAI_LAUNCH((cast_k<float, bf16_t>), g, b, 0, s, (const float*)src, (bf16_t*)dst, numel);
    else if (src_dtype == PAI_BF16 && dst_dtype == PAI_F32)
        PAI_LAUNCH((cast_k<bf16_t, float>), g, b, 0, s, (const bf16_t*)src, (float*)dst, numel);
    else if (src_dtype == PAI_F32 && dst_dtype == PAI_F32)
        PAI_LAUNCH((cast_k<float, float>), g, b, 0, s, (const float*)src, (float*)dst, numel);
    else if (src_dtype == PAI_BF16 && dst_dtype == PAI_BF16)
        PAI_LAUNCH((cast_k<bf16_t, bf16_t>), g, b, 0, s, (const bf16_t*)src, (bf16_t*)dst, numel);
    else
// ... 284 lines not shown
}

extern "C" int pai_colsum(int dtype, const void* x, int64_t rows, int C, float* out, void* stream) {
    PAI_CHECK(dtype == PAI_F32 || dtype == PAI_BF16, "pai_colsum: bad dtype %d", dtype);
    PAI_CHECK(x && out && rows > 0 && C > 0, "pai_colsum: bad arguments");
    if (pai_deterministic()) {
        const int64_t need = colsum_part_bytes(rows, C);
        const pai_handle_s* ctx = pai_ctx();
        PAI_CHECK(ctx->scratch && ctx->scratch_bytes >= need,
                  "pai_colsum: deterministic mode needs %lld bytes of scratch for the partial rows (pai_set_scratch; pai_colsum_scratch_bytes)",
                  (long long)need);
        return launch_colsum_det(dtype, x, rows, C, out, 1, ctx->scratch, (hipStream_t)stream);
    }
    return launch_colsum(dtype, x, rows, C, out, (hipStream_t)stream);
}

__device__ __forceinline__ void adam1(float& p, float& m, float& v, float g, float lr_over_bc1, float beta1, float beta2,
                                      float omb1, float omb2, float eps, float inv_sqrt_bc2) {
#pragma clang fp contract(off)
    const float mi = __builtin_fmaf(beta1, m, omb1 * g);
    const float vi = __builtin_fmaf(beta2, v, omb2 * g * g);
    m = mi;
    v = vi;
    p = p - lr_over_bc1 * mi / __builtin_fmaf(sqrtf(vi), inv_sqrt_bc2, eps);
}

__global__ __launch_bounds__(256) void adam_k(float* p, const float* g, float* m, float* v, int64_t numel,
                                              float lr_over_bc1, float beta1, float beta2, float omb1, float omb2,
                                              float eps, float inv_sqrt_bc2) {
    for (int64_t i = (int64_t)blockIdx.x * 256 + threadIdx.x; i < numel; i += (int64_t)gridDim.x * 256) {
        adam1(p[i], m[i], v[i], g[i], lr_over_bc1, beta1, beta2, omb1, omb2, eps, inv_sqrt_bc2);
    }
}

extern "C" int pai_adam(float* param, const float* grad, float* exp_avg, float* exp_avg_sq, int64_t numel,
                        float lr, float beta1, float beta2, float eps, int step_count, void* stream) {
    PAI_CHECK(param && grad && exp_avg && exp_avg_sq && step_count >= 1, "pai_adam: bad arguments");
    float lr_over_bc1, inv_sqrt_bc2;
    pai::adam_coeffs(lr, beta1, beta2, step_count, &lr_over_bc1, &inv_sqrt_bc2);
    int64_t blocks = (numel + 1023) / 1024;
    if (blocks > 8192) blocks = 8192;
    if (blocks < 1) blocks = 1;
    pai::plan_mark_adam(5, 11, lr, beta1, beta2, step_count);
    PAI_LAUNCH(adam_k, dim3((int)blocks), dim3(256), 0, (hipStream_t)stream, param, grad, exp_avg,
                       exp_avg_sq, numel, lr_over_bc1, beta1, beta2, (float)(1.0 - (double)beta1),
                       (float)(1.0 - (double)beta2), eps, inv_sqrt_bc2);
    PAI_LAUNCH_CHECK();
    return 0;
}

__global__ __launch_bounds__(256) void adam_pack64_k(float* p, const float* g, float* m, float* v, int64_t numel,
                                                     int64_t w_off, int Cout, int taps, int Cin, bf16_t* wf, bf16_t* wd,
                                                     int ntiles, float lr_over_bc1, float beta1, float beta2, float omb1,
                                                     float omb2, float eps, float inv_sqrt_bc2) {
    __shared__ float tile[64][65];
    const int tid = threadIdx.x;
    if ((int)blockIdx.x >= ntiles) {
        const int64_t wn = (int64_t)Cout * taps * Cin;
        const int64_t rest = numel - wn;
        for (int64_t k = (int64_t)(blockIdx.x - ntiles) * 256 + tid; k < rest; k += (int64_t)(gridDim.x - ntiles) * 256) {
            const int64_t i = k < w_off ? k : k + wn;
            adam1(p[i], m[i], v[i], g[i], lr_over_bc1, beta1, beta2, omb1, omb2, eps, inv_sqrt_bc2);
        }
        return;
    }
    const int nci = Cin / 64, nco = Cout / 64;
    const int lb = blockIdx.x;
    const int ci0 = (lb % nci) * 64, co0 = ((lb / nci) % nco) * 64, t = lb / (nci * nco);
    const int q = tid & 15, r0 = tid >> 4;
#pragma unroll
    for (int j = 0; j < 4; ++j) {
        const int r = r0 + 16 * j;
        const int64_t i = w_off + ((int64_t)(co0 + r) * taps + t) * Cin + ci0 + 4 * q;
        const float4 g4 = *(const float4*)(g + i);
        float4 m4 = *(const float4*)(m + i), v4 = *(const float4*)(v + i), p4 = *(const float4*)(p + i);
        float* pe = &p4.x; float* me = &m4.x; float* ve = &v4.x; const float* ge = &g4.x;
#pragma unroll
        for (int e = 0; e < 4; ++e) {
            adam1(pe[e], me[e], ve[e], ge[e], lr_over_bc1, beta1, beta2, omb1, omb2, eps, inv_sqrt_bc2);
            tile[r][4 * q + e] = pe[e];
        }
        *(float4*)(m + i) = m4;
        *(float4*)(v + i) = v4;
        *(float4*)(p + i) = p4;
    }
    __syncthreads();
    const int c = tid & 7, s0 = tid >> 3;
#pragma unroll
    for (int j = 0; j < 2; ++j) {
        const int r = s0 + 32 * j;
        if (wf) {
            unsigned u[4];
#pragma unroll
            for (int e = 0; e < 4; ++e) u[e] = pk2bf(tile[r][8 * c + 2 * e], tile[r][8 * c + 2 * e + 1]);
            *(uint4*)(wf + ((size_t)(co0 + r) * taps + t) * Cin + ci0 + 8 * c) = make_uint4(u[0], u[1], u[2], u[3]);
        }
        if (wd) {
            unsigned u[4];
#pragma unroll
            for (int e = 0; e < 4; ++e) u[e] = pk2bf(tile[8 * c + 2 * e][r], tile[8 * c + 2 * e + 1][r]);
            *(uint4*)(wd + ((size_t)(ci0 + r) * taps + t) * Cout + co0 + 8 * c) = make_uint4(u[0], u[1], u[2], u[3]);
        }
    }
}

extern "C" int pai_adam_pack(float* param, const float* grad, float* exp_avg, float* exp_avg_sq, int64_t numel,
                             int64_t w_off, int Cout, int taps, int Cin, void* w_fwd, void* w_dgrad, float lr,
                             float beta1, float beta2, float eps, int step_count, void* stream) {
    PAI_CHECK(param && grad && exp_avg && exp_avg_sq && step_count >= 1 && (w_fwd || w_dgrad), "pai_adam_pack: bad arguments");
    PAI_CHECK(Cin > 0 && Cout > 0 && taps > 0 && (Cin % 64) == 0 && (Cout % 64) == 0,
              "pai_adam_pack: Cin=%d, Cout=%d must be multiples of 64 (bf16 packs)", Cin, Cout);
    const int64_t wn = (int64_t)Cout * taps * Cin;
    PAI_CHECK(w_off >= 0 && (w_off % 4) == 0 && w_off + wn <= numel, "pai_adam_pack: weight [%lld, %lld) outside the range of %lld",
              (long long)w_off, (long long)(w_off + wn), (long long)numel);
    PAI_CHECK((((uintptr_t)param | (uintptr_t)grad | (uintptr_t)exp_avg | (uintptr_t)exp_avg_sq | (uintptr_t)w_fwd | (uintptr_t)w_dgrad) & 15) == 0,
              "pai_adam_pack: pointers must be 16-byte aligned");
    const int64_t ntiles = (int64_t)(Cin / 64) * (Cout / 64) * taps;
    const int64_t rest = numel - wn;
    int64_t extra = (rest + 1023) / 1024;
    if (extra > 256) extra = 256;
    PAI_CHECK(ntiles + extra < (1ll << 31), "pai_adam_pack: too many tiles");
    float lr_over_bc1, inv_sqrt_bc2;
    pai::adam_coeffs(lr, beta1, beta2, step_count, &lr_over_bc1, &inv_sqrt_bc2);
    pai::plan_mark_adam(12, 18, lr, beta1, beta2, step_count);
    PAI_LAUNCH(adam_pack64_k, dim3((unsigned)(ntiles + extra)), dim3(256), 0, (hipStream_t)stream, param, grad,
                       exp_avg, exp_avg_sq, numel, w_off, Cout, taps, Cin, (bf16_t*)w_fwd, (bf16_t*)w_dgrad, (int)ntiles,
                       lr_over_bc1, beta1, beta2, (float)(1.0 - (double)beta1), (float)(1.0 - (double)beta2), eps,
                       inv_sqrt_bc2);
    PAI_LAUNCH_CHECK();
    return 0;
}

__global__ void adam_coeff_k(long long* step, float* coeff, float lr, float beta1, float beta2) {
    const long long t = *step + 1;
    *step = t;
    const double bc1 = 1.0 - pow((double)beta1, (double)t);
    const double bc2 = 1.0 - pow((double)beta2, (double)t);
    coeff[0] = (float)((double)lr / bc1);
    coeff[1] = (float)(1.0 / sqrt(bc2));
}

__global__ __launch_bounds__(256) void adam_dev_k(float* p, const float* g, float* m, float* v, int64_t numel,
                                                  const float* coeff, float beta1, float beta2, float omb1, float omb2,
                                                  float eps) {
    const float lr_over_bc1 = coeff[0], inv_sqrt_bc2 = coeff[1];
    for (int64_t i = (int64_t)blockIdx.x * 256 + threadIdx.x; i < numel; i += (int64_t)gridDim.x * 256) {
        adam1(p[i], m[i], v[i], g[i], lr_over_bc1, beta1, beta2, omb1, omb2, eps, inv_sqrt_bc2);
    }
}

extern "C" int pai_adam_dev(float* param, const float* grad, float* exp_avg, float* exp_avg_sq, int64_t numel,
                            float lr, float beta1, float beta2, float eps, int64_t* step_dev, float* coeff2_dev,
                            void* stream) {
    PAI_CHECK(param && grad && exp_avg && exp_avg_sq && step_dev && coeff2_dev, "pai_adam_dev: null pointer");
    hipStream_t s = (hipStream_t)stream;
    PAI_LAUNCH(adam_coeff_k, dim3(1), dim3(1), 0, s, (long long*)step_dev, coeff2_dev, lr, beta1, beta2);
    PAI_LAUNCH_CHECK();
    int64_t blocks = (numel + 1023) / 1024;
    if (blocks > 8192) blocks = 8192;
    if (blocks < 1) blocks = 1;
    PAI_LAUNCH(adam_dev_k, dim3((int)blocks), dim3(256), 0, s, param, grad, exp_avg, exp_avg_sq, numel,
                       (const float*)coeff2_dev, beta1, beta2, (float)(1.0 - (double)beta1), (float)(1.0 - (double)beta2), eps);
    PAI_LAUNCH_CHECK();
    return 0;
}

#define ADAM_CHUNK 48
struct AdamChunk {
    float* p[ADAM_CHUNK];
    const float* g[ADAM_CHUNK];
    float* m[ADAM_CHUNK];
    float* v[ADAM_CHUNK];
    int64_t n[ADAM_CHUNK];
};

typedef float f32x4_t __attribute__((ext_vector_type(4)));
template <bool NT>
__device__ __forceinline__ void adam_tensor(float* p, const float* g, float* m, float* v, int64_t numel, float lr_over_bc1,
                                            float beta1, float beta2, float omb1, float omb2, float eps, float inv_sqrt_bc2) {
    const bool vec = (((uintptr_t)p | (uintptr_t)g | (uintptr_t)m | (uintptr_t)v) & 15) == 0;
    const int64_t n4 = vec ? numel / 4 : 0;
    auto ld = [](const f32x4_t* q) { return NT ? __builtin_nontemporal_load(q) : *q; };
    auto st = [](f32x4_t* q, f32x4_t x) { if (NT) __builtin_nontemporal_store(x, q); else *q = x; };
// ... 96 lines not shown
                          (params[i0 + i] && grads[i0 + i] && exp_avgs[i0 + i] && exp_avg_sqs[i0 + i] && numels[i0 + i] > 0),
                      "pai_adam_multi: null tensor %d", i0 + i);
            c.p[i] = (float*)params[i0 + i];
            c.g[i] = (const float*)grads[i0 + i];
            c.m[i] = (float*)exp_avgs[i0 + i];
            c.v[i] = (float*)exp_avg_sqs[i0 + i];
            c.n[i] = numels[i0 + i];
            if (c.n[i] > big) big = c.n[i];
        }
        int64_t bx = (big + 2047) / 2048;
        if (bx > 2048) bx = 2048;
        pai::plan_mark_adam(1, 7, lr, beta1, beta2, step_count);
        PAI_LAUNCH(adam_multi_k, dim3((unsigned)bx, (unsigned)nt), dim3(256), 0, (hipStream_t)stream, c,
                           lr_over_bc1, beta1, beta2, (float)(1.0 - (double)beta1), (float)(1.0 - (double)beta2), eps,
                           inv_sqrt_bc2);
        PAI_LAUNCH_CHECK();
    }
    return 0;
}

#define ZERO_CHUNK 96
struct ZeroChunk {
    float* p[ZERO_CHUNK];
    int64_t n[ZERO_CHUNK];
};

__global__ __launch_bounds__(256) void zero_multi_k(ZeroChunk c) {
    float* p = c.p[blockIdx.y];
    const int64_t n = c.n[blockIdx.y];
    for (int64_t i = (int64_t)blockIdx.x * 256 + threadIdx.x; i < n; i += (int64_t)gridDim.x * 256) p[i] = 0.f;
}

extern "C" int pai_zero_multi(int count, void* const* ptrs, const int64_t* numels, void* stream) {
    PAI_CHECK(count >= 0 && (count == 0 || (ptrs && numels)), "pai_zero_multi: bad arguments");
    for (int i0 = 0; i0 < count; i0 += ZERO_CHUNK) {
        const int nt = count - i0 < ZERO_CHUNK ? count - i0 : ZERO_CHUNK;
        ZeroChunk c;
        memset(&c, 0, sizeof(c));
        int64_t big = 1;
        for (int i = 0; i < nt; ++i) {
            PAI_CHECK(numels[i0 + i] == 0 || (ptrs[i0 + i] && numels[i0 + i] > 0), "pai_zero_multi: null tensor %d", i0 + i);
            c.p[i] = (float*)ptrs[i0 + i];
            c.n[i] = numels[i0 + i];
            if (c.n[i] > big) big = c.n[i];
        }
        int64_t bx = (big + 1023) / 1024;
        if (bx > 256) bx = 256;
        PAI_LAUNCH(zero_multi_k, dim3((unsigned)bx, (unsigned)nt), dim3(256), 0, (hipStream_t)stream, c);
        PAI_LAUNCH_CHECK();
    }
    return 0;
}

struct LerpChunk {
    float* d[ADAM_CHUNK];
    const float* s[ADAM_CHUNK];
    int64_t n[ADAM_CHUNK];
};

__device__ __forceinline__ float ema1(float sh, float p, float w) {
#pragma clang fp contract(off)
    const float t = (sh - p) * w;
    return sh - t;
}

__global__ __launch_bounds__(256) void lerp_multi_k(LerpChunk c, float w) {
    float* d = c.d[blockIdx.y];
    const float* s = c.s[blockIdx.y];
    const int64_t n = c.n[blockIdx.y];
    for (int64_t i = (int64_t)blockIdx.x * 256 + threadIdx.x; i < n; i += (int64_t)gridDim.x * 256) {
        d[i] = ema1(d[i], s[i], w);
    }
}

extern "C" int pai_lerp_multi(int count, void* const* dsts, const void* const* srcs, const int64_t* numels, float weight,
                              void* stream) {
    PAI_CHECK(count >= 0 && (count == 0 || (dsts && srcs && numels)), "pai_lerp_multi: bad arguments");
    for (int i0 = 0; i0 < count; i0 += ADAM_CHUNK) {
        const int nt = count - i0 < ADAM_CHUNK ? count - i0 : ADAM_CHUNK;
        LerpChunk c;
        memset(&c, 0, sizeof(c));
        int64_t big = 1;
        for (int i = 0; i < nt; ++i) {
            PAI_CHECK(numels[i0 + i] == 0 || (dsts[i0 + i] && srcs[i0 + i] && numels[i0 + i] > 0), "pai_lerp_multi: null tensor %d", i0 + i);
            c.d[i] = (float*)dsts[i0 + i];
            c.s[i] = (const float*)srcs[i0 + i];
            c.n[i] = numels[i0 + i];
            if (c.n[i] > big) big = c.n[i];
        }
        int64_t bx = (big + 1023) / 1024;
        if (bx > 2048) bx = 2048;
        PAI_LAUNCH(lerp_multi_k, dim3((unsigned)bx, (unsigned)nt), dim3(256), 0, (hipStream_t)stream, c, weight);
        PAI_LAUNCH_CHECK();
    }
    return 0;
}

__global__ __launch_bounds__(256) void scale_k(float* p, int64_t n4, int64_t n, float f) {
    for (int64_t i = (int64_t)blockIdx.x * 256 + threadIdx.x; i < n4; i += (int64_t)gridDim.x * 256) {
        float4 v = ((float4*)p)[i];
        v.x *= f; v.y *= f; v.z *= f; v.w *= f;
        ((float4*)p)[i] = v;
    }
    if (blockIdx.x == 0 && threadIdx.x < (n & 3)) p[n4 * 4 + threadIdx.x] *= f;
}

// ... 147 lines not shown
```

### thesis-pai-reconstruction_amd/engine.py

```python
from __future__ import annotations

import os
from typing import Callable, List, Optional

import torch
import torch.nn as nn

from . import ops
from .ops import ACT_LRELU, ACT_NONE, ACT_RELU, ACT_TANH

BN_EPS_DEFAULT = 1e-5


def _fwd_pack_strides(mod) -> tuple:
    if isinstance(mod, nn.ConvTranspose2d):
        cin, cout, kh, kw = mod.weight.shape
        return (1, kh * kw * cin, kw * cin, cin)
    cout, cin, kh, kw = mod.weight.shape
    return (kh * kw * cin, 1, kw * cin, cin)


def _strides_match(t: torch.Tensor, want: tuple) -> bool:
    return all(s == w or n == 1 for s, w, n in zip(t.stride(), want, t.shape))


def to_fwd_pack_(mod) -> None:
    w = mod.weight
    if _strides_match(w, _fwd_pack_strides(mod)) and w.permute(_phys_perm(mod)).is_contiguous():
        return
    with torch.no_grad():
        w.data = w.data.permute(_phys_perm(mod)).contiguous().permute(_logical_perm(mod))


def _phys_perm(mod):
    return (1, 2, 3, 0) if isinstance(mod, nn.ConvTranspose2d) else (0, 2, 3, 1)


def _logical_perm(mod):
    return (3, 0, 1, 2) if isinstance(mod, nn.ConvTranspose2d) else (0, 3, 1, 2)


def _cin_cout(mod):
    if isinstance(mod, nn.ConvTranspose2d):
        return mod.weight.shape[0], mod.weight.shape[1]
    return mod.weight.shape[1], mod.weight.shape[0]


class GradArena:

    ALIGN = 64

    def __init__(self, entries, device):
        self.offsets = {}
        off = 0
        for p, _ in entries:
            self.offsets[id(p)] = (off, p.numel())
            off += (p.numel() + self.ALIGN - 1) // self.ALIGN * self.ALIGN
        self.flat = torch.zeros(off, dtype=torch.float32, device=device)
        self.views = {}
        self.params = []
        self._zero_small = self._zero_all = None
        self._small = []
        for p, mod in entries:
            o, n = self.offsets[id(p)]
            seg = self.flat[o:o + n]
            if mod is not None and p.dim() == 4:
                cin, cout = _cin_cout(mod)
                v = seg.view(cout, 4, 4, cin).permute(_logical_perm(mod))
                if min(cin, cout) <= 2:
                    self._small.append(seg)
            else:
                v = seg.view(p.shape)
                self._small.append(seg)
            self.views[id(p)] = v
            self.params.append(p)

    def view(self, p):
        return self.views[id(p)]

    def seg(self, p):
        o, n = self.offsets[id(p)]
        return self.flat[o:o + n]

    def end_of(self, p) -> int:
        o, n = self.offsets[id(p)]
        return (o + n + self.ALIGN - 1) // self.ALIGN * self.ALIGN

    def begin_backward(self, params, overwrite_weights: bool = False) -> bool:
        grads = [p.grad for p in params if p.requires_grad]
        if all(g is None for g in grads):
            if overwrite_weights and self._small:
                if self.flat.is_cuda:
                    if self._zero_small is None:
                        self._zero_small = ops.ZeroList(self._small)
                    self._zero_small()
                else:
                    torch._foreach_zero_(self._small)
            elif self.flat.is_cuda:
                if self._zero_all is None:
                    self._zero_all = ops.ZeroList([self.flat])
                self._zero_all()
            else:
                self.flat.zero_()
            return True
        for p in params:
            if p.requires_grad and (p.grad is None or p.grad.data_ptr() != self.view(p).data_ptr()):
                raise ops.PaiError("gradient arena: parameters carry foreign .grad tensors; call "
                                   "zero_grad(set_to_none=True) before backward")
        return False

    def attach(self, params) -> None:
        for p in params:
            if p.requires_grad:
                p.grad = self.view(p)

    def adopt_parameters(self) -> bool:
        dev = self.flat.device
        if any(p.device != dev for p in self.params):
            return False
        if getattr(self, "pflat", None) is not None and self.params_adopted():
            return True
        pflat = torch.zeros_like(self.flat)
        with torch.no_grad():
            for p in self.params:
                o, n = self.offsets[id(p)]
                v = self.views[id(p)]
                pv = pflat[o:o + n].as_strided(v.shape, v.stride(), o)
                pv.copy_(p.data)
                p.data = pv
        self.pflat = pflat
        if getattr(self, "mflat", None) is None:
            self.mflat = torch.zeros_like(self.flat)
            self.vflat = torch.zeros_like(self.flat)
        return True

    def params_adopted(self) -> bool:
        pf = getattr(self, "pflat", None)
        if pf is None:
            return False
        base = pf.data_ptr()
        return all(p.data_ptr() == base + 4 * self.offsets[id(p)][0] for p in self.params)

    def moment_views(self, p):
        o, n = self.offsets[id(p)]
        v = self.views[id(p)]
        return (self.mflat[o:o + n].as_strided(v.shape, v.stride(), o),
                self.vflat[o:o + n].as_strided(v.shape, v.stride(), o))


class _Packs:

    def __init__(self, mod, need_dgrad: bool, gen):
        self.mod = mod
        self.need_dgrad = need_dgrad
        self.gen = gen
        self.version = None
        self.dtype = None
        self.wf = None
        self.wd = None

    def _stale(self, dtype):
        w = self.mod.weight
        return self.version != (w._version, w.data_ptr(), self.gen[0]) or self.dtype != dtype

    def _prepare(self, dtype):
        to_fwd_pack_(self.mod)
        w = self.mod.weight
        cin, cout = _cin_cout(self.mod)
        if dtype == torch.float32:
            self.wf = w
            wf_out = None
        else:
            if self.wf is None or self.wf.dtype != dtype or self.wf is w:
                self.wf = torch.empty(w.numel(), dtype=dtype, device=w.device)
            wf_out = self.wf
        wd_out = None
        if self.need_dgrad:
            if self.wd is None or self.wd.dtype != dtype:
                self.wd = torch.empty(w.numel(), dtype=dtype, device=w.device)
            wd_out = self.wd
        return w, cout, w.shape[2] * w.shape[3], cin, wf_out, wd_out

    def _mark(self, dtype):
        w = self.mod.weight
        self.version = (w._version, w.data_ptr(), self.gen[0])
        self.dtype = dtype

    def spare(self):
        if self.dtype != torch.bfloat16 or self.wf is None or self.wf is self.mod.weight:
            return None
        if getattr(self, "_spare", None) is None:
            self._spare = (torch.empty_like(self.wf), torch.empty_like(self.wd) if self.wd is not None else None)
        return self._spare

    def commit(self):
        (self.wf, self.wd), self._spare = self._spare, (self.wf, self.wd)
        self._mark(self.dtype)

    def commit_replayed(self):
        self.commit()

    def get(self, dtype):
        if self._stale(dtype):
            w, cout, taps, cin, wf_out, wd_out = self._prepare(dtype)
            if wf_out is not None or wd_out is not None:
                ops.pack_weights(dtype, w, cout, taps, cin, wf_out, wd_out)
            self._mark(dtype)
        return self.wf, self.wd


def refresh_packs(packs, dtype) -> None:
    if dtype != torch.bfloat16:
        return
    batch, todo = [], []
    for pk in packs:
        if not pk._stale(dtype):
            continue
        cin, cout = _cin_cout(pk.mod)
        if cin % 64 or cout % 64:
            continue
        item = pk._prepare(dtype)
        batch.append(item)
        todo.append(pk)
    if batch:
        ops.pack_weights_multi(batch)
        for pk in todo:
            pk._mark(dtype)


def pack_targets(arena, packs):
    out = []
    for pk in packs:
        cin, cout = _cin_cout(pk.mod)
        if cin % 64 or cout % 64 or id(pk.mod.weight) not in arena.offsets:
            continue
        o, n = arena.offsets[id(pk.mod.weight)]
        out.append((o, n, cout, n // (cin * cout), cin, pk))
    out.sort(key=lambda t: t[0])
    return out


class _BNState:

    def __init__(self, C, device):
        self.mean = torch.empty(C, dtype=torch.float32, device=device)
        self.rstd = torch.empty(C, dtype=torch.float32, device=device)
        self.scale = torch.empty(C, dtype=torch.float32, device=device)
        self.shift = torch.empty(C, dtype=torch.float32, device=device)
        self.sums = torch.empty(2 * C, dtype=torch.float32, device=device)
# ... 89 lines not shown
        self.dec_packs = [_Packs(c, need_dgrad=True, gen=self.weights_generation) for c in self.dec_conv]
        self._plans = {}
        self._arena: Optional[GradArena] = None
        self._side = _SideStream()
        self.grad_ready_hook: Optional[Callable[[GradArena, int], None]] = None
        self.debug_capture: Optional[dict] = None

    def _dbg(self, name, t):
        if self.debug_capture is not None:
            self.debug_capture[name] = t.detach().clone()

    def _dropout(self, S, j, M, C, dtype):
        p = self.dec_drop[j]
        N = S["P"]["N"]
        if self.dropout_mask_fn is not None:
            mask = self.dropout_mask_fn(j, N, C, p, S["r"][j].device).to(torch.float32).contiguous()
        else:
            keep = torch.full((N, C), 1.0 - p, dtype=torch.float32, device=S["r"][j].device)
            mask = torch.bernoulli(keep) / (1.0 - p)
        S["drop"][j] = mask
        ops.dropout2d(dtype, S["r"][j], mask, N, M // N, C, S["r"][j])

    def ordered_params(self):
        out = []
        L = self.L
        for j in range(L - 1, -1, -1):
            if self.dec_bn[j] is not None:
                out += [(self.dec_bn[j].weight, None), (self.dec_bn[j].bias, None)]
            out += [(self.dec_conv[j].weight, self.dec_conv[j]), (self.dec_conv[j].bias, None)]
        for i in range(L - 1, -1, -1):
            if self.enc_bn[i] is not None:
                out += [(self.enc_bn[i].weight, None), (self.enc_bn[i].bias, None)]
            out += [(self.enc_conv[i].weight, self.enc_conv[i]), (self.enc_conv[i].bias, None)]
        return out

    def arena(self) -> GradArena:
        dev = self.enc_conv[0].weight.device
        if self._arena is None or self._arena.flat.device != dev:
            for c in self.enc_conv + self.dec_conv:
                to_fwd_pack_(c)
            self._arena = GradArena(self.ordered_params(), dev)
        return self._arena

    def pack_targets(self):
        arena = self.arena()
        if getattr(self, "_pt_cache", (None, None))[0] is not arena:
            self._pt_cache = (arena, pack_targets(arena, self.enc_packs + self.dec_packs))
        return self._pt_cache[1]

    def all_packs(self):
        return self.enc_packs + self.dec_packs

    def _plan(self, N, H, W, dtype, device):
        key = (N, H, W, dtype, str(device))
        if key in self._plans:
            return self._plans[key]
        L = self.L
        if H % (1 << L) or W % (1 << L):
            raise ops.PaiError(f"input {H}x{W} must be divisible by 2^{L}")
        P = {"N": N, "H": H, "W": W, "dtype": dtype, "device": device, "slots": [], "free": []}
        eh = [H >> (i + 1) for i in range(L)]
        ew = [W >> (i + 1) for i in range(L)]
        P["eh"], P["ew"] = eh, ew
        P["enc_desc"] = []
        cin = self.in_ch
        for i in range(L):
            hin = H >> i
            win = W >> i
            act = ACT_LRELU if i == 0 else ACT_NONE
            P["enc_desc"].append(ops.make_desc(dtype, 0, N, hin, win, cin, 0, self.enc_c[i], 2, 0, 0, act))
            cin = self.enc_c[i]
        P["dec_desc"] = []
        for j in range(L):
            hin, win = eh[L - 1 - j], ew[L - 1 - j]
            if j == 0:
                c1, c2, r1, r2 = self.enc_c[L - 1], 0, 1, 0
            else:
                c1, c2 = self.dec_c[j - 1], self.enc_c[L - 1 - j]
                r1, r2 = 0, 1
            act = ACT_NONE
            if j == L - 1:
                r1, r2, act = 0, 0, ACT_TANH
            P["dec_desc"].append(ops.make_desc(dtype, 1, N, hin, win, c1, c2, self.dec_c[j], 2, r1, r2, act))
        rows = 1
        for i in range(L):
            if self.enc_bn[i] is not None:
                rows = max(rows, ops.bn_stats_buffer_rows(ops.conv_fwd_stats_rows_max(P["enc_desc"][i]))
                           * 2 * self.enc_c[i])
        for j in range(L):
            if self.dec_bn[j] is not None:
                rows = max(rows, ops.bn_stats_buffer_rows(ops.conv_fwd_stats_rows_max(P["dec_desc"][j]))
                           * 2 * self.dec_c[j])
        P["stats"] = torch.empty(rows, dtype=torch.float32, device=device)
        mx = 1
        for i in range(L):
            if self.enc_bn[i] is not None:
                mx = max(mx, ops.bn_bwd_partial_rows(N * eh[i] * ew[i]) * 2 * self.enc_c[i])
        for j in range(L):
            if self.dec_bn[j] is not None:
                mx = max(mx, ops.bn_bwd_partial_rows(N * 4 * eh[L - 1 - j] * ew[L - 1 - j]) * 2 * self.dec_c[j])
        for i in range(2, L):
            if self.enc_bn[i - 1] is not None:
                mx = max(mx, ops.conv_dgrad_bn_rows_max(P["enc_desc"][i]) * 2 * self.enc_c[i - 1])
        for j in range(1, L):
            if self.dec_bn[j - 1] is not None:
                mx = max(mx, ops.conv_dgrad_bn_rows_max(P["dec_desc"][j]) * 2 * self.dec_c[j - 1])
        P["bwd_partials"] = torch.empty(mx, dtype=torch.float32, device=device)
        ops.ensure_workspace(max(ops.conv_workspace_bytes(d, op) for d in P["enc_desc"] + P["dec_desc"]
                                 for op in (0, 1)), device)
        ops.ensure_scratch(ops.scratch_bytes_for(P["enc_desc"] + P["dec_desc"]), device)
        ops.ensure_wgrad_workspace(P["enc_desc"] + P["dec_desc"], device)
        self._plans[key] = P
        return P
# ... 97 lines not shown
            if j == 0:
                x1, x2 = S["z"][L - 1], None
            else:
                x1 = S["r"][j - 1]
                skip = L - 1 - j
                x2 = S["a"][skip] if skip > 0 else S["z"][0]
                if j == L - 1:
                    x2 = S["z"][0]
            if j < L - 1:
                bn = self.dec_bn[j]
                M = N * S["dh"][j] * S["dw"][j]
                act = ACT_RELU if j < L - 2 else ACT_NONE
                if training:
                    _conv_bn_train(d, x1, x2, wf, self.dec_conv[j].bias, S["w"][j], S["r"][j], act, bn, S["dbn"][j],
                                   bn_updates, P["stats"])
                else:
                    ops.conv_fwd(d, x1, x2, wf, self.dec_conv[j].bias, y_raw=S["w"][j])
                    _bn_forward(bn, S["dbn"][j], None, 0, M, False, 0)
                    ops.bn_apply(dtype, S["w"][j], M, self.dec_c[j], S["dbn"][j].scale, S["dbn"][j].shift, act,
                                 S["r"][j])
                if training and self.dec_drop[j] > 0:
                    self._dropout(S, j, M, self.dec_c[j], dtype)
            else:
                S["pred"] = torch.empty_like(S["pred"])
                ops.conv_fwd(d, x1, x2, wf, self.dec_conv[j].bias, y_f32=S["pred"])
        if L == 1:
            raise ops.PaiError("Unet needs at least two levels")
        pred = S["pred"]
        if self.out_ch != 1:
            pred = pred.view(N, H, W, self.out_ch).permute(0, 3, 1, 2)
        return pred, S

    def backward(self, S, gpred: torch.Tensor, fresh: bool = False):
        P = S["P"]
        L, N, dtype = self.L, P["N"], P["dtype"]
        eh, ew = P["eh"], P["ew"]
        G = self._grad_bufs(S)
        A = self.arena()
        hook = self.grad_ready_hook
        if self.out_ch != 1:
            gpred = gpred.permute(0, 2, 3, 1)
        gpred = gpred.contiguous()
        if gpred.dtype != torch.float32:
            gpred = gpred.float()

        def done(p):
            if hook is not None:
                hook(A, A.end_of(p))

        side = self._side

        conv_wgrad = ops.conv_wgrad_overwrite_w if fresh else ops.conv_wgrad

        batch_n = int(os.environ.get("PAI_WGRAD_BATCH", "3"))
        held = []

        def flush_held():
            if held:
                with torch.cuda.stream(side.fork()):
                    for run in held:
                        run()
                held.clear()

        def wgrad(d, x1, x2, dz, conv, with_bias):
            def run():
                thin = min(_cin_cout(conv)) <= 2
                fn = ops.conv_wgrad if thin else conv_wgrad
                fn(d, x1, x2, dz, A.seg(conv.weight), A.seg(conv.bias) if with_bias else None)
                if thin:
                    side.mark_scratch()
                done(conv.bias)
            if batch_n > 1 and dz.numel() // max(1, conv.weight.shape[1] if isinstance(conv, nn.ConvTranspose2d) else conv.weight.shape[0]) <= int(os.environ.get("PAI_WGRAD_BATCH_PIX", "1024")):
                held.append(run)
                if len(held) >= batch_n:
                    flush_held()
                return
            flush_held()
            with torch.cuda.stream(side.fork(d)):
                run()

        j = L - 1
        dh = G["dz_head"]
        ops.tanh_bwd(dtype, S["pred"], gpred, None, dh)
        d = P["dec_desc"][j]
        x1 = S["r"][j - 1]
        x2 = S["z"][0]
        wgrad(d, x1, x2, dh, self.dec_conv[j], True)
        _, wd = self.dec_packs[j].get(dtype)
        part = P["bwd_partials"]
        fused_rows = None
        if (j - 1) in S["drop"] or self.dec_bn[j - 1] is None:
            ops.conv_dgrad(d, dh, wd, G["gr"][j - 1], G["gskip"][0])
            if (j - 1) in S["drop"]:
                ops.dropout2d(dtype, G["gr"][j - 1], S["drop"][j - 1], N, S["dh"][j - 1] * S["dw"][j - 1], self.dec_c[j - 1],
                              G["gr"][j - 1])
        else:
            pst, pbn = S["dbn"][j - 1], self.dec_bn[j - 1]
            ops.conv_dgrad_bn_apply(d, dh, wd, G["gr"][j - 1], G["gskip"][0], S["w"][j - 1], ACT_NONE, None, ACT_NONE,
                                    None, None, pst.mean, pst.rstd, part, pbn.weight, pst.sums, A.seg(pbn.weight),
                                    A.seg(pbn.bias), G["dz_dec"][j - 1])
            fused_rows = -1
        for j in range(L - 2, -1, -1):
            bn, st, conv = self.dec_bn[j], S["dbn"][j], self.dec_conv[j]
            M = N * S["dh"][j] * S["dw"][j]
            C = self.dec_c[j]
            n = M * C
            act = ACT_RELU if j < L - 2 else ACT_NONE
            dz = G["dz_dec"][j]
            if fused_rows is None:
                du = G["du"][:n] if act != ACT_NONE else G["gr"][j]
                ops.bn_bwd_reduce(dtype, G["gr"][j], act, None, ACT_NONE, S["r"][j] if act != ACT_NONE else None,
                                  S["w"][j], M, C, st.mean, st.rstd, du if act != ACT_NONE else None, part, st.sums,
                                  A.seg(bn.weight), A.seg(bn.bias))
                ops.bn_bwd_apply(dtype, du, S["w"][j], M, C, st.mean, st.rstd, bn.weight, st.sums, dz)
            self._dbg(f"dec{j}.dz", dz)
            d = P["dec_desc"][j]
            if j == 0:
                x1, x2 = S["z"][L - 1], None
            else:
                skip = L - 1 - j
                x1, x2 = S["r"][j - 1], (S["a"][skip] if skip > 0 else S["z"][0])
            wgrad(d, x1, x2, dz, conv, False)
            _, wd = self.dec_packs[j].get(dtype)
            if j == 0:
                fused_rows = ops.conv_dgrad_bn(d, dz, wd, G["dz_enc"][L - 1], None, S["z"][L - 1], ACT_RELU)
            elif (j - 1) in S["drop"]:
                ops.conv_dgrad(d, dz, wd, G["gr"][j - 1], G["gskip"][L - 1 - j])
                ops.dropout2d(dtype, G["gr"][j - 1], S["drop"][j - 1], N, S["dh"][j - 1] * S["dw"][j - 1],
                              self.dec_c[j - 1], G["gr"][j - 1])
                fused_rows = None
            else:
                pst, pbn = S["dbn"][j - 1], self.dec_bn[j - 1]
                ops.conv_dgrad_bn_apply(d, dz, wd, G["gr"][j - 1], G["gskip"][L - 1 - j], S["w"][j - 1], ACT_RELU, None,
                                        ACT_NONE, pst.scale, pst.shift, pst.mean, pst.rstd, part, pbn.weight, pst.sums,
                                        A.seg(pbn.weight), A.seg(pbn.bias), G["dz_dec"][j - 1])
                fused_rows = -1
        i = L - 1
        conv = self.enc_conv[i]
        dz = G["dz_enc"][i]
        d = P["enc_desc"][i]
        wgrad(d, S["a"][i - 1], None, dz, conv, True)
        _, wd = self.enc_packs[i].get(dtype)

        enc0_fused = ops.conv_dgrad_act_wthin_ok(P["enc_desc"][1], P["enc_desc"][0], False)

        def enc_dgrad(i, dz, wd):
            d = P["enc_desc"][i]
            if i - 1 == 0 and enc0_fused:
                c0, d0 = self.enc_conv[0], P["enc_desc"][0]
                ops.conv_dgrad_act_wthin(d, dz, wd, S["z"][0], ACT_LRELU, G["gskip"][0], ACT_NONE, d0, S["x"], None,
                                         A.seg(c0.weight), A.seg(c0.bias), wthin_slabs(P, d, d0))
                return 0
            if i - 1 == 0:
                if G["dz_enc"][0] is None:
                    G["dz_enc"][0] = torch.empty_like(S["z"][0])
                return ops.conv_dgrad_bn(d, dz, wd, G["dz_enc"][0], None, S["z"][0], ACT_LRELU, G["gskip"][0], ACT_NONE)
            pst, pbn = S["ebn"][i - 1], self.enc_bn[i - 1]
            ops.conv_dgrad_bn_apply(d, dz, wd, G["ga"][i - 1], None, S["z"][i - 1], ACT_LRELU, G["gskip"][i - 1], ACT_RELU,
                                    pst.scale, pst.shift, pst.mean, pst.rstd, part, pbn.weight, pst.sums,
                                    A.seg(pbn.weight), A.seg(pbn.bias), G["dz_enc"][i - 1])
            return -1

        fused_rows = enc_dgrad(i, dz, wd)
        for i in range(L - 2, 0, -1):
            bn, st, conv = self.enc_bn[i], S["ebn"][i], self.enc_conv[i]
            M = N * eh[i] * ew[i]
            C = self.enc_c[i]
            dz = G["dz_enc"][i]
            d = P["enc_desc"][i]
            wgrad(P["enc_desc"][i], S["a"][i - 1], None, dz, conv, False)
            _, wd = self.enc_packs[i].get(dtype)
            fused_rows = enc_dgrad(i, dz, wd)
        conv0 = self.enc_conv[0]
        flush_held()
        if not enc0_fused:
            with torch.cuda.stream(side.fork_tail()):
                (ops.conv_wgrad if min(_cin_cout(conv0)) <= 2 else conv_wgrad)(
                    P["enc_desc"][0], S["x"], None, G["dz_enc"][0], A.seg(conv0.weight), A.seg(conv0.bias))
        side.join()
        done(conv0.bias)


def wthin_slabs(P, d, d_thin):
    if "wthin_slabs" not in P:
        P["wthin_slabs"] = torch.empty(ops.conv_dgrad_act_wthin_slab_bytes(d, d_thin) // 4, dtype=torch.float32,
                                       device=P["device"])
    return P["wthin_slabs"]


class DiscEngine:
    def __init__(self, disc: nn.Module):
        seq = disc.discriminator
        self.convs = [seq[i].block[0] for i in range(4)] + [seq[4]]
        self.in_ch = self.convs[0].weight.shape[1] // 2
        self.chans = [c.weight.shape[0] for c in self.convs]
        self.weights_generation = [0]
        self.packs = [_Packs(c, need_dgrad=True, gen=self.weights_generation) for c in self.convs]
        self._plans = {}
        self._arena = None
        self._side = _SideStream()
        self.grad_ready_hook = None

    def ordered_params(self):
        out = [(self.convs[4].weight, self.convs[4])]
        for k in range(3, -1, -1):
            out += [(self.convs[k].weight, self.convs[k]), (self.convs[k].bias, None)]
        return out

    def arena(self) -> GradArena:
        dev = self.convs[0].weight.device
        if self._arena is None or self._arena.flat.device != dev:
            for c in self.convs:
                to_fwd_pack_(c)
            self._arena = GradArena(self.ordered_params(), dev)
        return self._arena

    def pack_targets(self):
        arena = self.arena()
        if getattr(self, "_pt_cache", (None, None))[0] is not arena:
            self._pt_cache = (arena, pack_targets(arena, self.packs))
        return self._pt_cache[1]

    def all_packs(self):
        return self.packs

    def _plan(self, N, H, W, dtype, device):
        key = (N, H, W, dtype, str(device))
        if key in self._plans:
            return self._plans[key]
# ... 116 lines not shown
        S["head_done"] = need_grad
        return S

    def _wgrad_desc(self, P, k):
        if os.environ.get("PAI_D_WGRAD_SOLO", "1") in ("", "0"):
            return P["desc"][k]
        solo = P.setdefault("desc_solo", {})
        if k not in solo:
            import copy
            d = copy.copy(P["desc"][k])
            d.hints = 1
            solo[k] = d
        return solo[k]

    def backward(self, S, glogits, need_params: bool, need_dy: bool, fresh: bool = False, head_done: bool = False,
                 addend=None):
        conv_wgrad = ops.conv_wgrad_overwrite_w if fresh else ops.conv_wgrad
        P = S["P"]
        N, H, W, dtype, dev = P["N"], P["H"], P["W"], P["dtype"], P["device"]
        G = self._grads(S)
        A = self.arena() if need_params else None
        hook = self.grad_ready_hook
        if head_done:
            if not S.get("head_done"):
                raise ops.PaiError("DiscEngine.backward(head_done=True) without a forward_loss that kept its gradients")
            dl = G["dl"]
        else:
            glogits = glogits.contiguous().float()
            if dtype == torch.float32:
                dl = glogits.reshape(-1)
            else:
                ops.cast(glogits, G["dl"])
                dl = G["dl"]
        d = P["desc"][4]
        side = self._side
        gy = None
        if need_params:
            with torch.cuda.stream(side.fork(d)):
                ops.conv_wgrad(d, S["a"][3], None, dl, A.seg(self.convs[4].weight), None)
                if hook is not None:
                    hook(A, A.end_of(self.convs[4].weight))
            side.mark_scratch()
        _, wd = self.packs[4].get(dtype)
        if not head_done:
            ops.conv_dgrad_act(d, dl, wd, G["du"][3], None, S["a"][3], ACT_LRELU)
        wthin = need_params and not need_dy and ops.conv_dgrad_act_wthin_ok(P["desc"][1], P["desc"][0], need_dy)
        for k in range(3, -1, -1):
            conv = self.convs[k]
            d = P["desc"][k]
            if wthin and k == 0:
                break
            if need_params and k == 0:
                with torch.cuda.stream(side.fork_tail()):
                    (ops.conv_wgrad if min(_cin_cout(conv)) <= 2 else conv_wgrad)(
                        d, S["xin"], S["yin"], self._du0(S), A.seg(conv.weight), A.seg(conv.bias))
            elif need_params:
                with torch.cuda.stream(side.fork(d)):
                    conv_wgrad(self._wgrad_desc(P, k), S["a"][k - 1], None, G["du"][k], A.seg(conv.weight), A.seg(conv.bias))
                    if hook is not None:
                        hook(A, A.end_of(conv.bias))
            if k == 1 and wthin:
                _, wd = self.packs[1].get(dtype)
                c0, d0 = self.convs[0], P["desc"][0]
                ops.conv_dgrad_act_wthin(d, G["du"][1], wd, S["a"][0], ACT_LRELU, None, ACT_NONE, d0, S["xin"], S["yin"],
                                         A.seg(c0.weight), A.seg(c0.bias), wthin_slabs(P, d, d0))
            elif k > 0:
                _, wd = self.packs[k].get(dtype)
                ops.conv_dgrad_act(d, G["du"][k], wd, self._du0(S) if k == 1 else G["du"][k - 1], None, S["a"][k - 1], ACT_LRELU)
            elif need_dy:
                _, wd = self.packs[0].get(dtype)
                if addend is not None and self.in_ch == 1 and self.fused_enabled() and addend.dtype == torch.float32 \
                        and addend.is_contiguous() and addend.numel() == N * H * W and ops.conv_dgrad_f32add_ok(d):
                    gy = torch.empty(N * H * W, dtype=torch.float32, device=dev)
                    ops.conv_dgrad_f32add(d, self._du0(S), wd, addend, gy)
                else:
                    ops.conv_dgrad(d, self._du0(S), wd, None, G["dy"], only_c2=True)
        side.join()
        if need_params and hook is not None:
            hook(A, A.end_of(self.convs[0].bias))
        if not need_dy:
            return None
        if gy is not None:
            return gy.view(N, 1, H, W)
        gy = torch.empty(N * H * W * self.in_ch, dtype=torch.float32, device=dev)
        ops.cast(G["dy"], gy)
        gy = gy.view(N, 1, H, W) if self.in_ch == 1 else gy.view(N, H, W, self.in_ch).permute(0, 3, 1, 2)
        if addend is not None:
            if gy.is_contiguous() and gy.numel() % 8 == 0:
                ops.add_act(torch.float32, gy, addend, ops.ACT_NONE, gy)
            else:
                gy = gy + addend
        return gy
```

### thesis-pai-reconstruction_amd/lib.py

```python
from __future__ import annotations

import ctypes as C
import os

HERE = os.path.dirname(os.path.abspath(__file__))
LIB_PATH = os.environ.get("PAI_HIP_LIB") or os.path.join(HERE, "libpai_hip.so")

F32, BF16 = 0, 1
U8 = 2
ACT_NONE, ACT_LRELU, ACT_RELU, ACT_TANH = 0, 1, 2, 3
ACT_SILU = 4
HINT_SOLO = 1


class PaiError(RuntimeError):
    pass


class ConvDesc(C.Structure):
    _fields_ = [("dtype", C.c_int32), ("transposed", C.c_int32),
                ("N", C.c_int32), ("H", C.c_int32), ("W", C.c_int32),
                ("C1", C.c_int32), ("C2", C.c_int32), ("Cout", C.c_int32),
                ("kernel", C.c_int32), ("stride", C.c_int32), ("pad", C.c_int32),
                ("relu1", C.c_int32), ("relu2", C.c_int32), ("epilogue_act", C.c_int32),
                ("groups", C.c_int32), ("pack_flags", C.c_int32), ("hints", C.c_int32)]


class BwdEpilogue(C.Structure):
    _fields_ = [("z", C.c_void_p), ("add", C.c_void_p), ("scale", C.c_void_p), ("shift", C.c_void_p),
                ("mean", C.c_void_p), ("rstd", C.c_void_p), ("partials", C.c_void_p),
                ("act1", C.c_int32), ("act2", C.c_int32)]


class BnTrain(C.Structure):
    _fields_ = [("gamma", C.c_void_p), ("beta", C.c_void_p), ("eps", C.c_float), ("momentum", C.c_float),
                ("n_updates", C.c_int32), ("running_mean", C.c_void_p), ("running_var", C.c_void_p),
                ("num_batches_tracked", C.c_void_p), ("mean", C.c_void_p), ("rstd", C.c_void_p),
                ("scale", C.c_void_p), ("shift", C.c_void_p)]


_P = C.c_void_p
_I = C.c_int
_L = C.c_int64
_F = C.c_float
_U32 = C.c_uint32
_U64 = C.c_uint64
_D = C.POINTER(ConvDesc)

SIGNATURES = {
    "pai_last_error": (C.c_char_p, []),
    "pai_version": (_I, []),
    "pai_device_info": (_I, [C.POINTER(_I), C.POINTER(_I), C.c_char_p, _I]),
    "pai_set_tunable": (_I, [C.c_char_p, _I]),
    "pai_get_tunable": (_I, [C.c_char_p, _I]),
    "pai_order_dependent_launches": (_L, []),
    "pai_create": (_I, [_I, C.POINTER(C.c_void_p)]),
    "pai_bind": (_I, [C.c_void_p]),
    "pai_destroy": (_I, [C.c_void_p]),
    "pai_handle_set_workspace": (_I, [C.c_void_p, C.c_void_p, C.c_int64]),
    "pai_handle_set_scratch": (_I, [C.c_void_p, C.c_void_p, C.c_int64]),
    "pai_handle_set_wgrad_workspace": (_I, [C.c_void_p, C.c_void_p, C.c_int64]),
    "pai_conv_out_hw": (_I, [_D, C.POINTER(_I), C.POINTER(_I)]),
    "pai_conv_fwd_stats_rows": (_I, [_D]),
    "pai_conv_fwd_stats_rows_max": (_I, [_D]),
    "pai_bn_stats_buffer_rows": (_I, [_I]),
    "pai_conv_kernel_id": (_I, [_D, _I]),
    "pai_conv_kernel_name": (_I, [_D, _I, C.c_char_p, _I]),
    "pai_set_workspace": (_I, [_P, _L]),
    "pai_conv_workspace_bytes": (_L, [_D, _I]),
    "pai_set_scratch": (_I, [_P, _L]),
    "pai_conv_scratch_bytes": (_L, [_D, _I]),
    "pai_set_wgrad_workspace": (_I, [_P, _L]),
    "pai_conv_wgrad_workspace_bytes": (_L, [_D]),
    "pai_conv_wgrad_order_free": (_I, [_D, _I]),
    "pai_conv_fwd": (_I, [_D, _P, _P, _P, _P, _P, _P, _P, _P, _P]),
    "pai_conv_dgrad": (_I, [_D, _P, _P, _P, _P, _I, _P]),
    "pai_conv_dgrad_act": (_I, [_D, _P, _P, _P, _P, _P, _I, _P]),
    "pai_conv_dgrad_act_wthin_ok": (_I, [_D, _D, _I]),
    "pai_conv_dgrad_act_wthin_order_free": (_I, [_D, _D]),
    "pai_conv_dgrad_act_wthin_slab_bytes": (_L, [_D, _D]),
    "pai_conv_dgrad_act_wthin_kernel_name": (_I, [_D, _D, C.c_char_p, _I]),
    "pai_conv_dgrad_act_wthin": (_I, [_D, _P, _P, _P, _I, _P, _I, _D, _P, _P, _P, _P, _I, _P, _L, _P]),
    "pai_conv_dgrad_f32add_ok": (_I, [_D]),
    "pai_conv_dgrad_f32add": (_I, [_D, _P, _P, _P, _P, _P]),
    "pai_head_loss_ok": (_I, [_D, _I]),
    "pai_head_loss": (_I, [_D, _P, _P, _P, _I, _F, _F, _F, _P, _F, _P, _P, _P, _P, _P, _I, _P]),
    "pai_conv_dgrad_bn_rows_max": (_I, [_D]),
    "pai_conv_dgrad_bn": (_I, [_D, _P, _P, _P, _P, C.POINTER(BwdEpilogue), C.POINTER(_I), _P]),
    "pai_bn_bwd_finalize": (_I, [_P, _I, _I, _P, _P, _P, _P]),
    "pai_conv_fwd_bn": (_I, [_D, _P, _P, _P, _P, _P, _P, _I, C.POINTER(BnTrain), _P, _P]),
    "pai_conv_dgrad_bn_apply": (_I, [_D, _P, _P, _P, _P, C.POINTER(BwdEpilogue), _P, _P, _P, _P, _P, _P]),
    "pai_conv_bn_fused": (_I, [_D, _I]),
    "pai_conv_wgrad": (_I, [_D, _P, _P, _P, _P, _P, _P]),
    "pai_conv_wgrad_overwrite": (_I, [_D, _P, _P, _P, _P, _P, _P]),
    "pai_conv_wgrad_overwrite_w": (_I, [_D, _P, _P, _P, _P, _P, _P]),
    "pai_conv_prologue_ok": (_I, [_D]),
    "pai_conv_fwd_pro": (_I, [_D, _P, _P, _P, _P, _P, _P, _P, _I, _P]),
    "pai_conv_wgrad_pro": (_I, [_D, _P, _P, _P, _P, _I, _P, _P, _I, _P]),
    "pai_pack_weights": (_I, [_I, _P, _I, _I, _I, _P, _P, _P]),
    "pai_build_flags": (_I, []),
    "pai_pack_weights_multi": (_I, [_I, _P, _P, _P, _P, _P, _P, _P]),
    "pai_bn_finalize": (_I, [_P, _I, _I, _L, _P, _P, _F, _F, _I, _P, _P, _P, _P, _P, _P, _P, _P]),
    "pai_bn_eval_coeffs": (_I, [_I, _P, _P, _P, _P, _F, _P, _P, _P]),
    "pai_bn_apply": (_I, [_I, _P, _L, _I, _P, _P, _I, _P, _P]),
    "pai_bn2_add_act": (_I, [_I, _P, _P, _P, _P, _P, _P, _L, _I, _I, _I, _P, _P]),
    "pai_bn_bwd_partial_rows": (_I, [_L]),
    "pai_bn_bwd_reduce": (_I, [_I, _P, _I, _P, _I, _P, _P, _L, _I, _P, _P, _P, _P, _P, _P, _P, _P]),
    "pai_bn_bwd_reduce_affine": (_I, [_I, _P, _I, _P, _I, _P, _L, _I, _P, _P, _P, _P, _P, _P, _P, _P, _P, _P]),
    "pai_bn_bwd_apply": (_I, [_I, _P, _P, _L, _I, _P, _P, _P, _P, _P, _P]),
    "pai_bn_bwd_apply_affine": (_I, [_I, _P, _I, _P, _L, _I, _P, _P, _P, _P, _P, _P, _P, _P]),
    "pai_act_bwd": (_I, [_I, _P, _I, _P, _I, _P, _L, _P, _P]),
    "pai_maxpool2": (_I, [_I, _P, _I, _I, _I, _I, _P, _P, _P]),
    "pai_maxpool2_bwd": (_I, [_I, _P, _P, _I, _I, _I, _I, _P, _P]),
    "pai_upsample2": (_I, [_I, _P, _I, _I, _I, _I, _P, _P]),
    "pai_upsample2_bwd": (_I, [_I, _P, _I, _I, _I, _I, _P, _P]),
    "pai_add_act": (_I, [_I, _P, _P, _L, _I, _P, _P]),
    "pai_bn2_bwd_reduce": (_I, [_I, _P, _I, _P, _P, _L, _I, _P, _P, _P, _P, _P, _P, _P, _P, _P, _P, _P]),
    "pai_bn2_bwd_apply": (_I, [_I, _P, _I, _P, _P, _L, _I, _P, _P, _P, _P, _P, _P, _P, _P, _P, _P, _P, _P, _P]),
    "pai_instnorm_fwd": (_I, [_I, _P, _I, _I, _I, _F, _I, _P, _P, _P, _P]),
    "pai_instnorm_bwd": (_I, [_I, _P, _P, _I, _I, _I, _I, _P, _P, _P, _P]),
    "pai_dropout2d": (_I, [_I, _P, _P, _I, _L, _I, _P, _P]),
    "pai_layernorm_partial_rows": (_I, [_L]),
    "pai_layernorm_fwd": (_I, [_I, _P, _P, _L, _I, _P, _P, _F, _P, _I, _P, _P, _P, _P, _P]),
    "pai_layernorm_bwd": (_I, [_I, _P, _P, _L, _I, _P, _P, _P, _P, _P, _P, _P]),
    "pai_gelu": (_I, [_I, _P, _L, _P, _P]),
    "pai_gelu_bwd": (_I, [_I, _P, _P, _L, _P, _P]),
    "pai_mha_fwd": (_I, [_I, _P, _I, _I, _I, _I, _P, _P, _P, _P]),
    "pai_mha_bwd": (_I, [_I, _P, _P, _P, _I, _I, _I, _I, _P, _P, _P, _P]),
    "pai_mha_kernel_name": (_I, [_I, _I, _I, _I, C.c_char_p, _I]),
    "pai_subsample2": (_I, [_I, _P, _I, _I, _I, _I, _P, _P]),
    "pai_subsample2_bwd": (_I, [_I, _P, _I, _I, _I, _I, _P, _P]),
    "pai_bn_stats_rows": (_I, [_L]),
    "pai_bn_stats": (_I, [_I, _P, _L, _I, _P, _P]),
    "pai_colsum": (_I, [_I, _P, _L, _I, _P, _P]),
    "pai_colsum_scratch_bytes": (_L, [_L, _I]),
    "pai_gate_partial_rows": (_I, [_L]),
    "pai_gate_scratch_bytes": (_L, [_L, _I]),
    "pai_gate_hidden": (_I, [_I, _P, _P, _L, _I, _P, _P, _P, _P, _P, _P, _P, _P, _P, _P]),
    "pai_gate_apply": (_I, [_I, _P, _P, _L, _I, _P, _P, _P, _P, _P]),
    "pai_gate_apply_bwd": (_I, [_I, _P, _P, _P, _P, _L, _I, _P, _P, _P, _P, _P, _I, _P]),
    "pai_gate_hidden_bwd": (_I, [_I, _P, _P, _P, _P, _P, _L, _I] + [_P] * 15),
    "pai_bce_logits": (_I, [_P, _L, _F, _F, _P, _F, _P, _P]),
    "pai_l1": (_I, [_P, _P, _L, _F, _P, _F, _P, _P]),
    "pai_mse": (_I, [_P, _P, _L, _F, _P, _F, _P, _P]),
    "pai_scalar_take": (_I, [_P, _P, _P]),
    "pai_metrics_take": (_I, [_P, _L, _L, _P, _P]),
    "pai_tanh_bwd": (_I, [_I, _P, _P, _P, _L, _P, _P]),
    "pai_denormalize": (_I, [_P, _P, _L, _P, _P]),
    "pai_ssim_sse": (_I, [_P, _P, _I, _I, _I, _I, _P, _P, _P, _P]),
    "pai_ssim_psnr_bwd": (_I, [_P, _P, _I, _I, _I, _I, _F, _F, _P, _P, _P, _P]),
    "pai_ssim_bwd_workspace_floats": (_L, [_I, _I, _I]),
    "pai_eval_planes": (_I, [_P, _P, _I, _I, _I, _I, _P, _P, _P, _P, _P, _P]),
    "pai_eval_kernel_name": (_I, [_I, C.c_char_p, _I]),
    "pai_cast": (_I, [_I, _P, _I, _P, _L, _P]),
    "pai_reduce_rows": (_I, [_P, _I, _I, _P, _I, _P]),
    "pai_adam": (_I, [_P, _P, _P, _P, _L, _F, _F, _F, _F, _I, _P]),
    "pai_adam_dev": (_I, [_P, _P, _P, _P, _L, _F, _F, _F, _F, _P, _P, _P]),
    "pai_adam_pack": (_I, [_P, _P, _P, _P, _L, _L, _I, _I, _I, _P, _P, _F, _F, _F, _F, _I, _P]),
    "pai_comm_unique_id": (_I, [_P]),
    "pai_comm_init": (_I, [_P, _I, _I, C.POINTER(_P)]),
    "pai_allreduce": (_I, [_P, _P, _L, _I, _P]),
    "pai_comm_destroy": (_I, [_P]),
    "pai_adam_multi": (_I, [_I, _P, _P, _P, _P, _P, _F, _F, _F, _F, _I, _P]),
    "pai_adam_multi_dev": (_I, [_I, _P, _P, _P, _P, _P, _F, _F, _F, _F, _P, _P, _P]),
    "pai_plan_create": (_I, [C.POINTER(_P)]),
    "pai_plan_destroy": (_I, [_P]),
    "pai_plan_begin": (_I, [_P]),
    "pai_plan_end": (_I, [_P]),
    "pai_plan_run": (_I, [_P, _L]),
    "pai_plan_info": (_I, [_P, C.POINTER(_I), C.POINTER(_I), C.POINTER(_I), C.POINTER(_L)]),
    "pai_stream_wait": (_I, [_P, _P]),
    "pai_stream_wait_last": (_I, [_P, _P]),
    "pai_event_create": (_I, [C.POINTER(_P)]),
    "pai_event_destroy": (_I, [_P]),
    "pai_event_record": (_I, [_P, _P]),
    "pai_event_create_timing": (_I, [C.POINTER(_P)]),
    "pai_event_elapsed_ms": (_I, [_P, _P, C.POINTER(_F)]),
    "pai_profile_arm": (_I, [_P, _P]),
    "pai_stream_wait_event": (_I, [_P, _P]),
    "pai_zero_multi": (_I, [_I, _P, _P, _P]),
    "pai_lerp_multi": (_I, [_I, _P, _P, _P, _F, _P]),
    "pai_scale": (_I, [_P, _L, _F, _P]),
    "pai_cast_multi": (_I, [_I, _I, _P, _I, _P, _P, _P]),
    "pai_filter_to_dense": (_I, [_P, _I, _I, _I, _I, _P, _P]),
    "pai_filter_grad_from_dense": (_I, [_P, _I, _I, _I, _I, _P, _P]),
    "pai_swap_mid": (_I, [_I, _P, C.c_int64, _I, _I, C.c_int64, _P, _P]),
    "pai_resize_aa_u8": (_I, [_P, _I, _I, _I, _I, _P, _P, _I, _P, _P, _I, _P, _P, _P]),
    "pai_batch_gather": (_I, [_I, _P, _P, _L, _L, _P, _I, _P, _P, _P, _P]),
    "pai_data_kernel_name": (_I, [_I, _I, C.c_char_p, _I]),
    "pai_sattn_fwd": (_I, [_I, _P, _I, _I, _I, _I, _P, _P]),
    "pai_sattn_fwd_lse": (_I, [_I, _P, _I, _I, _I, _I, _P, _P, _P]),
    "pai_sattn_bwd": (_I, [_I, _P, _P, _P, _P, _I, _I, _I, _I, _P, _P, _P]),
    "pai_sattn_kernel_name": (_I, [_I, _I, _I, C.c_char_p, _I]),
    "pai_affine_act": (_I, [_I, _P, _L, _I, _I, _P, _P, _I, _I, _P, _P]),
    "pai_film_coeffs": (_I, [_I, _I, _I, _P, _P, _P, _L, _P, _P, _P]),
    "pai_avgpool2": (_I, [_I, _P, _I, _I, _I, _I, _P, _P]),
    "pai_avgpool2_bwd": (_I, [_I, _P, _I, _I, _I, _I, _P, _P]),
    "pai_silu_bwd": (_I, [_I, _P, _P, _L, _P, _P]),
    "pai_gamma_embedding": (_I, [_I, _P, _I, _I, _P, _P]),
    "pai_palette_step": (_I, [_I, _P, _P, _P, _L, _I, _I, _I, _F, _F, _F, _F, _F, _F, _P, _P, _P]),
    "pai_film_norm_slabs": (_I, [_L]),
    "pai_film_norm_ws_floats": (_L, [_I, _L, _I]),
    "pai_film_norm_fwd": (_I, [_I, _P, _L, _I, _I, _P, _P, _P, _P, _P, _L, _P, _F, _I, _P, _P]),
    "pai_film_norm_bwd": (_I, [_I, _P, _P, _L, _I, _I, _P, _P, _P, _P, _P, _L, _P, _F, _I, _P, _P, _P, _P, _P, _P]),
    "pai_palette_noise": (_I, [_P, _P, _P, _P, _P, _P, _I, _I, _L, _I, _P, _P, _P, _P]),
    "pai_palette_objective_slabs": (_I, [_L]),
    "pai_palette_objective_ws_floats": (_L, [_I, _L]),
    "pai_palette_objective": (_I, [_P, _P, _P, _P, _P, _P, _I, _I, _L, _I, _I, _F, _P, _P, _P, _P]),
    "pai_philox_fill": (_I, [_I, _P, _L, _U64, _U32, _U32, _U32, _U32, _P]),
    "pai_film_norm_fwd_rng": (_I, [_I, _P, _L, _I, _I, _P, _P, _P, _P, _P, _L, _U64, _U32, _U32, _U32, _F, _I, _P, _P]),
    "pai_film_norm_bwd_rng": (_I, [_I, _P, _P, _L, _I, _I, _P, _P, _P, _P, _P, _L, _U64, _U32, _U32, _U32, _F, _I, _P, _P, _P, _P,
# ... 39 lines not shown
```

### thesis-pai-reconstruction_amd/ops.py

```python
from __future__ import annotations

import ctypes as C

import threading
from typing import Optional

import torch

from . import lib as L
from .lib import ACT_LRELU, ACT_NONE, ACT_RELU, ACT_SILU, ACT_TANH, BF16, F32, U8, ConvDesc, PaiError


def code_of(dtype: torch.dtype) -> int:
    if dtype == torch.float32:
        return F32
    if dtype == torch.bfloat16:
        return BF16
    raise PaiError(f"unsupported storage dtype {dtype}")


_TLS = threading.local()


def _stream():
# ... 20 lines not shown
        return None
    if not t.is_cuda:
        raise PaiError("pai ops need HIP device tensors (no CPU fallback exists)")
    if dtype is not None and t.dtype != dtype:
        raise PaiError(f"expected {dtype}, got {t.dtype}")
    return t.data_ptr()


def make_desc(dtype, transposed, N, H, W, C1, C2, Cout, stride=2, relu1=0, relu2=0, act=ACT_NONE,
              kernel=4, groups=1) -> ConvDesc:
    d = ConvDesc()
    d.dtype = code_of(dtype)
    d.transposed = int(transposed)
    d.N, d.H, d.W, d.C1, d.C2, d.Cout = N, H, W, C1, C2, Cout
    d.kernel, d.stride, d.pad = {4: (4, stride, 1), 3: (3, 1, 1), 1: (1, 1, 0)}[kernel]
    d.relu1, d.relu2, d.epilogue_act = int(relu1), int(relu2), int(act)
    d.groups = int(groups) if groups and groups > 1 else 0
    return d


def conv_out_hw(d: ConvDesc):
    oh, ow = C.c_int(), C.c_int()
    L.check(L.load().pai_conv_out_hw(C.byref(d), C.byref(oh), C.byref(ow)), "pai_conv_out_hw")
    return oh.value, ow.value


def conv_fwd_stats_rows(d: ConvDesc) -> int:
    r = L.load().pai_conv_fwd_stats_rows(C.byref(d))
    if r < 0:
        L.check(1, "pai_conv_fwd_stats_rows")
    return r


def conv_fwd_stats_rows_max(d: ConvDesc) -> int:
    return L.load().pai_conv_fwd_stats_rows_max(C.byref(d))


def bn_stats_buffer_rows(rows: int) -> int:
    return L.load().pai_bn_stats_buffer_rows(rows)


PROFILE = None


def conv_kernel_id(d: ConvDesc, op: int) -> int:
    return L.load().pai_conv_kernel_id(C.byref(d), op)


def conv_kernel_name(d: ConvDesc, op: int) -> str:
    buf = C.create_string_buffer(96)
    if L.load().pai_conv_kernel_name(C.byref(d), op, buf, 96) != 0:
        L.check(1, "pai_conv_kernel_name")
    return buf.value.decode()


def conv_flops(d: ConvDesc) -> int:
    groups = max(1, int(getattr(d, "groups", 1)))
    if d.transposed:
        return 2 * d.N * d.H * d.W * 16 * (d.C1 + d.C2) * d.Cout // groups
    oh = (d.H + 2 * d.pad - d.kernel) // d.stride + 1
    ow = (d.W + 2 * d.pad - d.kernel) // d.stride + 1
    return 2 * d.N * oh * ow * d.kernel * d.kernel * (d.C1 + d.C2) * d.Cout // groups


class LaunchTimer:

    def __init__(self):
        self.h0, self.h1 = C.c_void_p(), C.c_void_p()
        L.check(L.load().pai_event_create_timing(C.byref(self.h0)), "pai_event_create_timing")
        L.check(L.load().pai_event_create_timing(C.byref(self.h1)), "pai_event_create_timing")

    def arm(self):
        L.check(L.load().pai_profile_arm(self.h0, self.h1), "pai_profile_arm")

    @staticmethod
    def disarm():
        L.check(L.load().pai_profile_arm(None, None), "pai_profile_arm")

    def elapsed_time(self, _other=None) -> float:
        ms = C.c_float()
        L.check(L.load().pai_event_elapsed_ms(self.h0, self.h1, C.byref(ms)), "pai_event_elapsed_ms")
        return ms.value

    def __del__(self):
        try:
            L.load().pai_event_destroy(self.h0)
            L.load().pai_event_destroy(self.h1)
        except Exception:
            pass


class _Timed:

    def __init__(self, d, op):
        self.on = PROFILE is not None
        if self.on:
            self.d, self.op = d, op
            self.t = LaunchTimer()

    def __enter__(self):
        if self.on:
            self.t.arm()

    def __exit__(self, *exc):
        if self.on:
            LaunchTimer.disarm()
# ... 664 lines not shown
def ssim_psnr_bwd(pred, target, NC, H, W, denorm, w_ssim, w_psnr, sse, grad, workspace):
    L.check(L.load().pai_ssim_psnr_bwd(_p(pred, torch.float32), _p(target, torch.float32), NC, H, W, int(denorm),
                                       float(w_ssim), float(w_psnr), _p(sse, torch.float64),
                                       _p(grad, torch.float32), _p(workspace, torch.float32), _stream()),
            "pai_ssim_psnr_bwd")


def cast(src, dst):
    assert src.numel() == dst.numel()
    L.check(L.load().pai_cast(code_of(src.dtype), _p(src), code_of(dst.dtype), _p(dst), src.numel(), _stream()),
            "pai_cast")


def cast_multi(pairs) -> None:
    pairs = list(pairs)
    ok = len(pairs) > 1 and len(pairs) <= 8 and len({(s.dtype, d.dtype) for s, d in pairs}) == 1 and all(
        s.numel() == d.numel() and s.numel() % 8 == 0 and s.data_ptr() % 16 == 0 and d.data_ptr() % 16 == 0 and s.is_cuda
        and d.is_cuda and s.is_contiguous() and d.is_contiguous() for s, d in pairs)
    if not ok:
        for s, d in pairs:
            cast(s, d)
        return
    n = len(pairs)
    srcs = (C.c_void_p * n)(*[s.data_ptr() for s, _ in pairs])
    dsts = (C.c_void_p * n)(*[d.data_ptr() for _, d in pairs])
    numels = (C.c_int64 * n)(*[s.numel() for s, _ in pairs])
    L.check(L.load().pai_cast_multi(n, code_of(pairs[0][0].dtype), srcs, code_of(pairs[0][1].dtype), dsts, numels, _stream()),
            "pai_cast_multi")


def reduce_rows(partial, rows, C_, out, accumulate=False):
    L.check(L.load().pai_reduce_rows(_p(partial, torch.float32), rows, C_, _p(out, torch.float32),
                                     int(accumulate), _stream()), "pai_reduce_rows")


def adam(param, grad, exp_avg, exp_avg_sq, lr, beta1, beta2, eps, step):
    with _TimedBytes("adam", 28 * param.numel()):
        L.check(L.load().pai_adam(_p(param, torch.float32), _p(grad, torch.float32), _p(exp_avg, torch.float32),
                                  _p(exp_avg_sq, torch.float32), param.numel(), lr, beta1, beta2, eps, step,
                                  _stream()), "pai_adam")


def adam_pack(param, grad, exp_avg, exp_avg_sq, w_off, cout, taps, cin, w_fwd, w_dgrad, lr, beta1, beta2, eps, step):
    dt = torch.bfloat16
    packs = 2 * cout * taps * cin * ((w_fwd is not None) + (w_dgrad is not None))
    with _TimedBytes("adam", 28 * param.numel() + packs):
        L.check(L.load().pai_adam_pack(_p(param, torch.float32), _p(grad, torch.float32), _p(exp_avg, torch.float32),
                                       _p(exp_avg_sq, torch.float32), param.numel(), int(w_off), cout, taps, cin,
                                       _p(w_fwd, dt) if w_fwd is not None else None,
                                       _p(w_dgrad, dt) if w_dgrad is not None else None, lr, beta1, beta2, eps, step,
                                       _stream()), "pai_adam_pack")


def adam_dev(param, grad, exp_avg, exp_avg_sq, lr, beta1, beta2, eps, step_dev, coeff_dev):
    L.check(L.load().pai_adam_dev(_p(param, torch.float32), _p(grad, torch.float32), _p(exp_avg, torch.float32),
                                  _p(exp_avg_sq, torch.float32), param.numel(), lr, beta1, beta2, eps,
                                  _p(step_dev, torch.int64), _p(coeff_dev, torch.float32), _stream()), "pai_adam_dev")


def adam_multi(params, grads, exp_avgs, exp_avg_sqs, lr, beta1, beta2, eps, step):
    n = len(params)
    for t in (*params, *grads, *exp_avgs, *exp_avg_sqs):
        if not t.is_cuda or t.dtype != torch.float32 or not t.is_contiguous():
            raise PaiError("adam_multi needs contiguous fp32 HIP tensors")
    arr = lambda ts: (C.c_void_p * n)(*[t.data_ptr() for t in ts])
    numels = (C.c_int64 * n)(*[p.numel() for p in params])
    with _TimedBytes("adam", 28 * sum(p.numel() for p in params)):
        L.check(L.load().pai_adam_multi(n, arr(params), arr(grads), arr(exp_avgs), arr(exp_avg_sqs), numels, lr, beta1,
                                        beta2, eps, step, _stream()), "pai_adam_multi")


def adam_multi_dev(params, grads, exp_avgs, exp_avg_sqs, lr, beta1, beta2, eps, step_dev, coeff_dev):
    n = len(params)
    for t in (*params, *grads, *exp_avgs, *exp_avg_sqs):
        if not t.is_cuda or t.dtype != torch.float32 or not t.is_contiguous():
            raise PaiError("adam_multi_dev needs contiguous fp32 HIP tensors")
    arr = lambda ts: (C.c_void_p * n)(*[t.data_ptr() for t in ts])
    numels = (C.c_int64 * n)(*[p.numel() for p in params])
    L.check(L.load().pai_adam_multi_dev(n, arr(params), arr(grads), arr(exp_avgs), arr(exp_avg_sqs), numels, lr, beta1,
                                        beta2, eps, _p(step_dev, torch.int64), _p(coeff_dev, torch.float32), _stream()),
            "pai_adam_multi_dev")


def _raw(stream) -> int:
    return stream.cuda_stream if hasattr(stream, "cuda_stream") else int(stream)


def stream_wait(waiting, signalling) -> None:
    L.check(L.load().pai_stream_wait(_raw(waiting), _raw(signalling)), "pai_stream_wait")


def stream_wait_last(waiting, signalling) -> None:
    L.check(L.load().pai_stream_wait_last(_raw(waiting), _raw(signalling)), "pai_stream_wait_last")


class Event:

    def __init__(self):
        self._h = C.c_void_p()
        L.check(L.load().pai_event_create(C.byref(self._h)), "pai_event_create")

    def record(self, stream=None):
        L.check(L.load().pai_event_record(self._h, _raw(stream) if stream is not None else _stream()), "pai_event_record")

    def wait(self, stream=None):
        L.check(L.load().pai_stream_wait_event(_raw(stream) if stream is not None else _stream(), self._h),
# ... 416 lines not shown
```

### thesis-pai-reconstruction_amd/optim.py

```python
from __future__ import annotations

import os

import torch

from . import ops


class ArenaAdam(torch.optim.Adam):
    def __init__(self, params, engine, lr=2e-4, betas=(0.5, 0.999), eps=1e-7):
        super().__init__(list(params), lr=lr, betas=betas, eps=eps, foreach=True)
        self._engine = engine
        self._arena_steps = 0
        self._dev_step = None
        self._dev_coeff = None
        self._streamed = None
        self._stream_step = 0
        self._reducer = None
        self._fuse_packs = os.environ.get("PAI_ADAM_PACK", "1") not in ("", "0")
        self._pack_targets = None
        self._packs_written = []
        self._last_commits = []

    def enable_device_step(self):
        if self._dev_step is None:
            dev = self.param_groups[0]["params"][0].device
            self._dev_step = torch.tensor(self.total_steps, dtype=torch.int64, device=dev)
            self._dev_coeff = torch.zeros(2, dtype=torch.float32, device=dev)

    def note_replays(self, n: int = 1):
        self._arena_steps += n

    def plan_state(self):
        eng = self._engine
        arena = eng.arena()
        if self._dev_step is not None or self._streamed is not None or not arena.params_adopted():
            return None
        if len(self.param_groups) != 1:
            return None
        g = self.param_groups[0]
        ptrs = []
        for pk in eng.all_packs():
            if pk.wf is None or pk.dtype is None:
                return None
            ptrs.append(pk.wf.data_ptr())
        mode, _ = self._stream_mode()
        if mode == "hook" and self._fuse_packs:
            for t in eng.pack_targets():
                if t[5].dtype == torch.bfloat16 and t[5]._stale(t[5].dtype):
                    return None
        return (mode, float(g["lr"]), float(g["betas"][0]), float(g["betas"][1]), float(g["eps"]), arena.flat.data_ptr(),
                arena.pflat.data_ptr(), tuple(ptrs))

    def plan_commits(self):
        return list(self._last_commits)

    def plan_replayed(self, commits):
        self._arena_steps += 1
        self._engine.weights_generation[0] += 1
        for pk in commits:
            pk.commit_replayed()

    def arm_streaming(self) -> bool:
        mode, reducer = self._stream_mode()
        if mode is None:
            return False
        arena = self._engine.arena()
        self._pack_targets = None
        if reducer is not None:
            if not reducer.subscribe(arena, self._on_reduced):
                return False
            self._reducer = reducer
        else:
            self._engine.grad_ready_hook = self._on_ready
            targets = getattr(self._engine, "pack_targets", None)
            self._pack_targets = targets() if (targets is not None and self._fuse_packs) else None
        self._packs_written = []
        self._streamed = 0
        self._stream_step = self.total_steps + 1
        return True

    def _stream_mode(self):
        if os.environ.get("PAI_NO_STREAM_ADAM", "0") not in ("", "0"):
            return None, None
        hook = getattr(self._engine, "grad_ready_hook", None)
        if hook is not None and getattr(hook, "__func__", None) is getattr(self._on_ready, "__func__", object()) \
                and getattr(hook, "__self__", None) is self:
            hook = None
        reducer = getattr(hook, "__self__", None) if hook is not None else None
        if self._dev_step is not None or (hook is not None and not hasattr(reducer, "subscribe")):
            return None, None
        group = self.param_groups[0]
        if len(self.param_groups) != 1 or group["weight_decay"] != 0 or group["amsgrad"] or group["maximize"]:
            return None, None
        params = group["params"]
        if not params or not params[0].is_cuda:
            return None, None
        arena = self._engine.arena()
        if len(params) != len(arena.params) or not arena.params_adopted():
            return None, None
        if reducer is not None:
            if os.environ.get("PAI_DDP_STREAM_ADAM", "0") in ("", "0") or reducer.world < 2:
                return None, None
            return "reducer", reducer
        return "hook", None

    def _adam_range(self, arena, a, b, step):
        group = self.param_groups[0]
        if b > a:
            ops.adam(arena.pflat[a:b], arena.flat[a:b], arena.mflat[a:b], arena.vflat[a:b], float(group["lr"]),
                     float(group["betas"][0]), float(group["betas"][1]), float(group["eps"]), step)

    def _adam_range_packing(self, arena, a, b, step):
        inside = [t for t in (self._pack_targets or ()) if a <= t[0] and t[0] + t[1] <= b]
        group = self.param_groups[0]
        cur = a
        for k, (o, n, cout, taps, cin, pk) in enumerate(inside):
            spare = pk.spare()
            if spare is None:
                continue
            end = inside[k + 1][0] if k + 1 < len(inside) else b
            ops.adam_pack(arena.pflat[cur:end], arena.flat[cur:end], arena.mflat[cur:end], arena.vflat[cur:end], o - cur,
                          cout, taps, cin, spare[0], spare[1], float(group["lr"]), float(group["betas"][0]),
                          float(group["betas"][1]), float(group["eps"]), step)
            self._packs_written.append(pk)
            cur = end
        self._adam_range(arena, cur, b, step)

    def _on_ready(self, arena, end_offset):
        if int(end_offset) < self._streamed:
            raise ops.PaiError("ArenaAdam: a streaming step is armed and a second backward pass reached this arena "
                               "before step(); use one backward pass per optimizer step or do not arm_streaming()")
        with torch.no_grad():
            self._adam_range_packing(arena, self._streamed, int(end_offset), self._stream_step)
        self._streamed = max(self._streamed, int(end_offset))

    def _on_reduced(self, arena, lo, hi):
        if lo != self._streamed:
            raise ops.PaiError(f"ArenaAdam: reduced bucket [{lo}, {hi}) does not continue the updated range "
                               f"[0, {self._streamed})")
        with torch.no_grad():
            self._adam_range(arena, lo, hi, self._stream_step)
        self._streamed = hi

    def _disarm(self):
        if getattr(self._engine, "grad_ready_hook", None) == self._on_ready:
            self._engine.grad_ready_hook = None
        reducer = getattr(self, "_reducer", None)
        if reducer is not None:
            reducer.unsubscribe(self._engine.arena())
            self._reducer = None
        self._streamed = None

    def _arena_ready(self):
        group = self.param_groups[0]
        if len(self.param_groups) != 1 or group["weight_decay"] != 0 or group["amsgrad"] or group["maximize"]:
            return None
        params = group["params"]
        if not params or not params[0].is_cuda:
            return None
        arena = self._engine.arena()
        if len(params) != len(arena.params) or not arena.adopt_parameters():
            return None
        for p in params:
            if p.grad is None or p.grad.data_ptr() != arena.view(p).data_ptr():
                return None
        return arena

    def _mirror_state(self, arena):
        for p in self.param_groups[0]["params"]:
            st = self.state[p]
            if "exp_avg" not in st:
                m, v = arena.moment_views(p)
                st["step"] = torch.tensor(0.0, dtype=torch.float32)
                st["exp_avg"], st["exp_avg_sq"] = m, v
            st["step"] += self._arena_steps
        self._arena_steps = 0

    @property
    def total_steps(self) -> int:
        any_state = next(iter(self.state.values()), None)
        done = int(any_state["step"]) if any_state and "step" in any_state else 0
        return done + self._arena_steps

    @torch.no_grad()
    def step(self, closure=None):
        streamed = self._streamed
        if streamed is not None:
            self._disarm()
        self._last_commits = []
        arena = self._arena_ready()
        if arena is None:
            if streamed:
                raise ops.PaiError("ArenaAdam: a streaming step was armed and partly applied, but the gradients are "
                                   "not the arena's any more")
            if self._arena_steps:
                self._mirror_state(self._engine.arena())
            return super().step(closure)
        group = self.param_groups[0]
        if streamed is not None:
            self._adam_range(arena, streamed, arena.flat.numel(), self._stream_step)
            self._arena_steps += 1
            self._engine.weights_generation[0] += 1
            for pk in self._packs_written:
                pk.commit()
            self._last_commits = self._packs_written
            self._packs_written = []
            return None
        if self._dev_step is not None:
            ops.adam_dev(arena.pflat, arena.flat, arena.mflat, arena.vflat, float(group["lr"]), float(group["betas"][0]),
                         float(group["betas"][1]), float(group["eps"]), self._dev_step, self._dev_coeff)
        else:
            step = self.total_steps + 1
            ops.adam(arena.pflat, arena.flat, arena.mflat, arena.vflat, float(group["lr"]), float(group["betas"][0]),
                     float(group["betas"][1]), float(group["eps"]), step)
        self._arena_steps += 1
        self._engine.weights_generation[0] += 1
        return None

    def state_dict(self):
        if self._arena_steps:
            self._mirror_state(self._engine.arena())
        return super().state_dict()

    def load_state_dict(self, state_dict):
        if self._arena_steps:
            self._mirror_state(self._engine.arena())
        super().load_state_dict(state_dict)
        params = self.param_groups[0]["params"]
        if not params or not params[0].is_cuda:
            return
        arena = self._engine.arena()
        if len(params) != len(arena.params) or not arena.adopt_parameters():
            return
        with torch.no_grad():
            for p in params:
                st = self.state.get(p)
                if not st or "exp_avg" not in st:
                    continue
                m, v = arena.moment_views(p)
                m.copy_(st["exp_avg"].to(m.device).reshape(m.shape))
                v.copy_(st["exp_avg_sq"].to(v.device).reshape(v.shape))
                st["exp_avg"], st["exp_avg_sq"] = m, v
                st["step"] = torch.as_tensor(float(st["step"]), dtype=torch.float32)
        self._arena_steps = 0
        if self._dev_step is not None:
            self._dev_step.fill_(self.total_steps)


class MultiAdam(torch.optim.Adam):

    def __init__(self, params, lr=2e-4, betas=(0.5, 0.999), eps=1e-7):
        super().__init__(list(params), lr=lr, betas=betas, eps=eps, foreach=True)
        self._dev_step = None
        self._dev_coeff = None
        self._arena_steps = 0

    def _total_steps(self) -> int:
        st = next(iter(self.state.values()), None)
        return (int(st["step"]) if st and "step" in st else 0) + self._arena_steps

    def enable_device_step(self):
        if self._dev_step is None:
            dev = self.param_groups[0]["params"][0].device
            self._dev_step = torch.tensor(self._total_steps(), dtype=torch.int64, device=dev)
            self._dev_coeff = torch.zeros(2, dtype=torch.float32, device=dev)

    def note_replays(self, n: int = 1):
        self._arena_steps += n

    @property
    def total_steps(self) -> int:
        return self._total_steps()

    def plan_state(self):
        if len(self.param_groups) != 1 or self._dev_step is not None:
            return None
        group = self.param_groups[0]
        if group["weight_decay"] != 0 or group["amsgrad"] or group["maximize"]:
            return None
        ps = [p for p in group["params"] if p.requires_grad]
        if not ps or any("exp_avg" not in self.state.get(p, ()) for p in ps):
            return None
        return ("multi", float(group["lr"]), tuple(float(b) for b in group["betas"]), float(group["eps"]), len(ps))

    def plan_commits(self):
        return [(p, p.grad) for p in self.param_groups[0]["params"] if p.grad is not None]

    def plan_replayed(self, commits):
        self._arena_steps += 1
        for p, g in commits:
            if p.grad is not g:
                p.grad = g

    def _mirror_steps(self):
        if self._arena_steps:
            for st in self.state.values():
# ... 70 lines not shown
```

### thesis-pai-reconstruction_amd/plan.py

```python
from __future__ import annotations

import os

import torch
from torch.utils._python_dispatch import TorchDispatchMode

from . import ops

_NO_KERNEL = {
    "empty", "empty_like", "empty_strided", "new_empty", "new_empty_strided", "view", "_unsafe_view", "reshape", "alias",
    "detach", "detach_", "as_strided", "permute", "transpose", "t", "slice", "select", "expand", "squeeze", "unsqueeze",
    "unbind", "split", "split_with_sizes", "narrow", "contiguous", "_reshape_alias", "view_as", "lift_fresh",
    "is_pinned", "record_stream", "sym_size", "sym_stride", "sym_numel", "sym_storage_offset", "size", "stride",
    "numel", "dim", "is_contiguous", "unfold", "diagonal", "flatten", "unflatten", "movedim", "chunk", "set_",
    "result_type", "_has_compatible_shallow_copy_type", "is_same_size", "is_nonzero", "_to_copy_noop",
}


_ACTIVE = None


def host_op(fn):
    rec = _ACTIVE
    if rec is None:
# ... 135 lines not shown
            if len(self.plans) >= self.max_plans:
                oldest = min(self.plans, key=lambda k: self.plans[k].last_use)
                del self.plans[oldest]
                self.evictions += 1
            return self._record(sig, batch, batch_idx)
        rec.last_use = self.calls
        if not self._replayable(rec):
            self.plans.clear()
            return m.training_step(batch, batch_idx)
        return self._replay(rec, batch)

    def _total_steps(self):
        return tuple(opt.total_steps for opt in self.model._all_optimizers())

    def _record(self, sig, batch, batch_idx):
        m = self.model
        rec = _Recorded()
        rec.static = tuple(torch.empty_like(b) for b in batch)
        for s, b in zip(rec.static, batch):
            s.copy_(b)
        rec.step0 = self._total_steps()
        before = m._pai_opt_steps
        logs, orig_log = [], m.log

        def record_log(name, value, *a, **k):
            logs.append((name, value.detach() if torch.is_tensor(value) else value, a, k))
            return orig_log(name, value, *a, **k)
        m.log = record_log
        global _ACTIVE
        recorder = _Recorder()
        try:
            with recorder:
                recorder.begin()
                _ACTIVE = recorder
                try:
                    out = m.training_step(rec.static, batch_idx)
                finally:
                    _ACTIVE = None
                    recorder.end()
        finally:
            del m.log
        rec.items = recorder.items
        rec.keep = recorder.keep
        rec.logs = logs
        rec.opt_steps = m._pai_opt_steps - before
        rec.commits = [opt.plan_commits() for opt in m._all_optimizers()]
        self.records += 1
        if recorder.foreign:
            kinds = sorted(set(recorder.foreign))
            self.disabled = ("the step launches kernels outside the C ABI (" + ", ".join(kinds[:8]) +
                             (", ..." if len(kinds) > 8 else "") + "): it cannot be replayed from a plan")
            self.plans.clear()
            return out
        after = self._total_steps()
        if any(b - a != 1 for a, b in zip(rec.step0, after)):
            self.disabled = "an optimizer did not take exactly one step in the recorded call"
            self.plans.clear()
            return out
        rec.last_use = self.calls
        self.plans[sig] = rec
        return out

    def _replayable(self, rec) -> bool:
        now = self._total_steps()
        delta = now[0] - rec.step0[0]
        return delta >= 0 and all(n - s0 == delta for n, s0 in zip(now, rec.step0))

    def _replay(self, rec, batch):
        m = self.model
        for s, b in zip(rec.static, batch):
            if s.data_ptr() != b.data_ptr():
                s.copy_(b, non_blocking=True)
        now = self._total_steps()
        delta = now[0] - rec.step0[0]
        if any(n - s0 != delta for n, s0 in zip(now, rec.step0)) or delta < 0:
            raise ops.PaiError("PlannedStep: the optimizers' step counts moved apart since the plan was recorded")
        for it in rec.items:
            if it[0] == "plan":
                it[1].run(delta)
            elif it[2].cuda_stream == torch.cuda.current_stream().cuda_stream:
                it[1]()
            else:
                with torch.cuda.stream(it[2]):
                    it[1]()
        for opt, commits in zip(m._all_optimizers(), rec.commits):
            opt.plan_replayed(commits)
        m._pai_opt_steps += rec.opt_steps
        for name, value, a, k in rec.logs:
            m.log(name, value, *a, **k)
        self.replays += 1
        return None

    def describe(self) -> dict:
        return {"plans": len(self.plans), "records": self.records, "replays": self.replays, "evictions": self.evictions,
                "disabled": self.disabled,
                "nodes": [r.info() for r in self.plans.values()]}


def enabled_by_default() -> bool:
    return os.environ.get("PAI_PLAN", "1") not in ("", "0")
```

Before: 11770 images/s.

## Prune dead 4x4 conv taps that only ever read padding, and skip their Adam updates

Builds a per-phase live-tap mask for 4x4 convs, where at small spatial sizes some taps only ever touch padding. It compacts the tap tables so the forward and dgrad kernels loop over fewer taps. Weight-gradient zeroing and the fused Adam+pack kernel then skip dead taps, since their gradients are always zero, and the weight and moment state of those taps is left untouched. This saves MFMA work and optimizer bandwidth on the deep 2x2/1x1 layers. The cost is extra bookkeeping: the tiled patch paths are disabled for pruned geometries, and it relies on dead taps staying exactly zero (guards, plan settling, and moment folding on load).

```diff
diff --git a/include/pai_hip.h b/include/pai_hip.h
--- a/include/pai_hip.h
+++ b/include/pai_hip.h
@@ -52,6 +52,7 @@
 
 int pai_conv_kernel_id(const pai_conv_desc* d, int op);
 int pai_conv_kernel_name(const pai_conv_desc* d, int op, char* name, int name_len);
+int pai_conv_live_taps(const pai_conv_desc* d, int op, uint32_t* mask_per_phase);
 
 int pai_create(int device_id, void** handle_out);
 int pai_bind(void* handle);
@@ -266,6 +267,9 @@
 int pai_adam_pack(float* param, const float* grad, float* exp_avg, float* exp_avg_sq, int64_t numel, int64_t w_off,
                   int Cout, int taps, int Cin, void* w_fwd, void* w_dgrad, float lr, float beta1, float beta2, float eps,
                   int step_count, void* stream);
+int pai_adam_pack_taps(float* param, const float* grad, float* exp_avg, float* exp_avg_sq, int64_t numel, int64_t w_off,
+                       int Cout, int taps, int Cin, void* w_fwd, void* w_dgrad, float lr, float beta1, float beta2,
+                       float eps, int step_count, uint32_t tap_mask, void* stream);
 int pai_adam_dev(float* param, const float* grad, float* exp_avg, float* exp_avg_sq, int64_t numel,
                  float lr, float beta1, float beta2, float eps, int64_t* step_dev, float* coeff2_dev, void* stream);
 int pai_adam_multi(int count, void* const* params, const void* const* grads, void* const* exp_avgs,
diff --git a/thesis-pai-reconstruction_amd/attention.py b/thesis-pai-reconstruction_amd/attention.py
--- a/thesis-pai-reconstruction_amd/attention.py
+++ b/thesis-pai-reconstruction_amd/attention.py
@@ -56,7 +56,7 @@
         return out
 
     def _plan(self, N, H, W, dtype, device):
-        key = (N, H, W, dtype, str(device))
+        key = (N, H, W, dtype, str(device), ops.get_tunable("prune_taps", 1))
         if key in self._plans:
             return self._plans[key]
         P = super()._plan(N, H, W, dtype, device)
@@ -247,6 +247,8 @@
             cin, cout = conv.weight.shape[1], conv.weight.shape[0]
             dense = fresh and conv.weight.shape[2] == 4 and min(cin, cout) > 2
             with torch.cuda.stream(side.fork(d)):
+                if conv.weight.shape[2] == 4:
+                    A.guard_dead_taps(conv.weight, d, dense)
                 (ops.conv_wgrad_overwrite_w if dense else ops.conv_wgrad)(
                     d, x1, x2, dz, A.seg(conv.weight), A.seg(conv.bias) if with_bias else None)
                 done(last if last is not None else conv.bias)
@@ -353,6 +355,7 @@
         if not enc0_fused:
             with torch.cuda.stream(side.fork_tail()):
                 c0_in, c0_out = conv0.weight.shape[1], conv0.weight.shape[0]
+                A.guard_dead_taps(conv0.weight, P["enc_desc"][0], fresh and min(c0_in, c0_out) > 2)
                 (ops.conv_wgrad_overwrite_w if (fresh and min(c0_in, c0_out) > 2) else ops.conv_wgrad)(
                     P["enc_desc"][0], S["x"], None, G["dz_enc"][0], A.seg(conv0.weight), A.seg(conv0.bias))
         side.join()
diff --git a/thesis-pai-reconstruction_amd/csrc/api.hip b/thesis-pai-reconstruction_amd/csrc/api.hip
--- a/thesis-pai-reconstruction_amd/csrc/api.hip
+++ b/thesis-pai-reconstruction_amd/csrc/api.hip
@@ -196,6 +196,41 @@
                     g->wt[p][t] = (signed char)(khs[a] * 4 + kws[b]);
                 }
         }
+}
+
+static unsigned live_table_taps(const GG& g, int ph) {
+    unsigned m = 0;
+    for (int t = 0; t < g.ntaps; ++t) {
+        bool ylive = false, xlive = false;
+        for (int gy = 0; gy < g.OHg && !ylive; ++gy) ylive = (unsigned)(gy * g.S + g.dy[ph][t]) < (unsigned)g.H;
+        for (int gx = 0; gx < g.OWg && !xlive; ++gx) xlive = (unsigned)(gx * g.S + g.dx[ph][t]) < (unsigned)g.W;
+        if (ylive && xlive) m |= 1u << t;
+    }
+    return m;
+}
+
+void gg_prune_dead_taps(GG* g) {
+    if (g->wtaps != 16 || g->ntaps > 16 || g->Cin <= 2 || g->Cout <= 2 || !pai_tunable("prune_taps", 1)) return;
+    unsigned live[4];
+    int n = -1;
+    for (int ph = 0; ph < g->nphase; ++ph) {
+        live[ph] = live_table_taps(*g, ph);
+        const int c = __builtin_popcount(live[ph]);
+        if (n >= 0 && c != n) return;
+        n = c;
+    }
+    if (n <= 0 || n >= g->ntaps) return;
+    for (int ph = 0; ph < g->nphase; ++ph) {
+        int k = 0;
+        for (int t = 0; t < g->ntaps; ++t)
+            if (live[ph] & (1u << t)) {
+                g->dy[ph][k] = g->dy[ph][t]; g->dx[ph][k] = g->dx[ph][t]; g->wt[ph][k] = g->wt[ph][t];
+                ++k;
+            }
+        for (; k < g->ntaps; ++k) g->dy[ph][k] = g->dx[ph][k] = g->wt[ph][k] = 0;
+    }
+    g->ntaps = n;
+    g->pruned = 1;
 }
 
 int gg_build_fwd(const pai_conv_desc* d, GG* g) {
@@ -225,6 +260,7 @@
         g->OHg = d->H; g->OWg = d->W;
         fill_phase_taps(g);
     }
+    gg_prune_dead_taps(g);
     finish_gg(g);
     return 0;
 }
@@ -266,6 +302,7 @@
         g->OHg = d->H; g->OWg = d->W;
         fill_conv_taps(g, 2, -d->pad);
     }
+    gg_prune_dead_taps(g);
     finish_gg(g);
     return 0;
 }
@@ -563,6 +600,17 @@
     return 0;
 }
 
+extern "C" int pai_conv_live_taps(const pai_conv_desc* d, int op, uint32_t* mask_per_phase) {
+    GG g;
+    if (!mask_per_phase || op < 0 || op > 2) { pai_set_error("pai_conv_live_taps: bad arguments"); return -1; }
+    if (op == 1 ? gg_build_dgrad(d, &g) : gg_build_fwd(d, &g)) return -1;
+    for (int ph = 0; ph < 4; ++ph) {
+        mask_per_phase[ph] = 0;
+        for (int t = 0; ph < g.nphase && t < g.ntaps; ++t) mask_per_phase[ph] |= 1u << g.wt[ph][t];
+    }
+    return g.ntaps;
+}
+
 extern "C" int pai_conv_fwd_stats_rows_max(const pai_conv_desc* d) {
     GG g;
     if (gg_build_fwd(d, &g)) return -1;
@@ -931,13 +979,24 @@
         if (rows) bias_rows = (float*)((char*)h->wslab + (have - rows));
     }
     if (overwrite && p.overwrites) {
+        if (g.pruned && overwrite == 1) {
+            hipError_t e = pai::memset_async(dw, 0, (size_t)g.Cout * g.wtaps * g.Cin * sizeof(float), s);
+            PAI_CHECK(e == hipSuccess, "pai_conv_wgrad_overwrite: hipMemsetAsync: %s", hipGetErrorString(e));
+        }
         a.overwrite = 1;
         a.overwrite_bias = p.k != WK_GROUPED3 && overwrite == 1;
     } else if (overwrite) {
-        hipError_t e = pai::memset_async(dw, 0, (size_t)g.Cout * g.wtaps * g.Cin * sizeof(float), s);
-        PAI_CHECK(e == hipSuccess, "pai_conv_wgrad_overwrite: hipMemsetAsync: %s", hipGetErrorString(e));
+        if (g.pruned && overwrite == 2) {
+            unsigned live = 0;
+            for (int ph = 0; ph < g.nphase; ++ph)
+                for (int t = 0; t < g.ntaps; ++t) live |= 1u << g.wt[ph][t];
+            if (int rc = launch_zero_taps(dw, g.Cout, g.wtaps, g.Cin, live, s)) return rc;
+        } else {
+            hipError_t e = pai::memset_async(dw, 0, (size_t)g.Cout * g.wtaps * g.Cin * sizeof(float), s);
+            PAI_CHECK(e == hipSuccess, "pai_conv_wgrad_overwrite: hipMemsetAsync: %s", hipGetErrorString(e));
+        }
         if (dbias && overwrite == 1) {
-            e = pai::memset_async(dbias, 0, (size_t)g.Cout * sizeof(float), s);
+            hipError_t e = pai::memset_async(dbias, 0, (size_t)g.Cout * sizeof(float), s);
             PAI_CHECK(e == hipSuccess, "pai_conv_wgrad_overwrite: hipMemsetAsync: %s", hipGetErrorString(e));
         }
     }
diff --git a/thesis-pai-reconstruction_amd/csrc/common.h b/thesis-pai-reconstruction_amd/csrc/common.h
--- a/thesis-pai-reconstruction_amd/csrc/common.h
+++ b/thesis-pai-reconstruction_amd/csrc/common.h
@@ -144,7 +144,10 @@
     signed char poy[4], pox[4];
     int gslice;
     int solo;
-};
+    int pruned;
+};
+
+void gg_prune_dead_taps(GG* g);
 
 struct PatchGeo {
     int groups;
@@ -282,6 +285,7 @@
     int pact;
 };
 float* wgrad_slab_acquire(int64_t bytes);
+int launch_zero_taps(float* dw, int Cout, int wtaps, int Cin, unsigned mask, hipStream_t s);
 int launch_wgrad_slab_sum(float* dw, const float* slab, int nsplits, int64_t n, int overwrite, hipStream_t s);
 bool grouped3_wgrad_ok(int dtype, const GG& g, const float* dbias);
 int64_t grouped3_wgrad_part_bytes(const GG& g);
diff --git a/thesis-pai-reconstruction_amd/csrc/gg_mfma.hip b/thesis-pai-reconstruction_amd/csrc/gg_mfma.hip
--- a/thesis-pai-reconstruction_amd/csrc/gg_mfma.hip
+++ b/thesis-pai-reconstruction_amd/csrc/gg_mfma.hip
@@ -1111,7 +1111,7 @@
 }
 
 bool pw_ok(int dtype, const GG& g, const FwdArgs& a) {
-    if (dtype != PAI_BF16 || g.ntaps != 1 || g.nphase != 1 || g.C2 != 0 || g.D2 != 0) return false;
+    if (dtype != PAI_BF16 || g.wtaps != 1 || g.nphase != 1 || g.C2 != 0 || g.D2 != 0) return false;
     if (!((g.C1 == 64 && g.Cout == 32) || (g.C1 == 32 && g.Cout == 64))) return false;
     if (a.yf32 || a.skip_d1) return false;
     if ((a.y1 != nullptr) == (a.yact != nullptr)) return false;
@@ -1243,8 +1243,8 @@
 bool wgrad_mfma_ok(int dtype, const GG& g) {
     if (dtype != PAI_BF16) return false;
     if (g.lsw < 0) return false;
-    if (g.ntaps == 1 && g.C2 == 0 && ((g.C1 == 64 && g.Cout == 32) || (g.C1 == 32 && g.Cout == 64))) return true;
-    if (g.ntaps == 1 && g.C2 == 0 && g.C1 == 64 && (g.Cout % 64) == 0) return true;
+    if (g.wtaps == 1 && g.C2 == 0 && ((g.C1 == 64 && g.Cout == 32) || (g.C1 == 32 && g.Cout == 64))) return true;
+    if (g.wtaps == 1 && g.C2 == 0 && g.C1 == 64 && (g.Cout % 64) == 0) return true;
     if (g.nphase == 1 && g.S == 1 && g.C2 == 0 && (g.C1 % 8) == 0 && (g.Cout % 8) == 0 && (g.C1 < 64 || g.Cout < 64))
         return true;
     if (g.C1 % 64 || g.C2 % 64) return false;
@@ -1755,7 +1755,7 @@
 }
 
 bool wgrad_pro_ok(int dtype, const GG& g) {
-    return wgrad_mfma_ok(dtype, g) && g.ntaps == 1 && g.nphase == 1 && g.C2 == 0 && !g.gslice && !g.relu1 && !wgrad3_ok(g);
+    return wgrad_mfma_ok(dtype, g) && g.wtaps == 1 && g.nphase == 1 && g.C2 == 0 && !g.gslice && !g.relu1 && !wgrad3_ok(g);
 }
 
 MfmaPlan wgrad_mfma_plan(const GG& g, bool has_dbias, bool has_prologue) {
@@ -1778,7 +1778,7 @@
     } else {
         p.variant = big ? WGRAD_TILE128 : WGRAD_TILE64;
         p.name = big ? "gg_wgrad_mfma_k<128>" : "gg_wgrad_mfma_k<64>";
-        p.db = p.ksplit == 1 && g.ntaps == 1 && g.nphase == 1 && (g.Cin % 4) == 0 && !g.gslice && pai_tunable("wgrad_stage", 1) != 0;
+        p.db = p.ksplit == 1 && g.wtaps == 1 && g.nphase == 1 && (g.Cin % 4) == 0 && !g.gslice && pai_tunable("wgrad_stage", 1) != 0;
         p.lds = p.db ? 64 * 132 * 4 : 2 * 64 * 256;
     }
     p.grid = tiles * p.ksplit;
diff --git a/thesis-pai-reconstruction_amd/csrc/gg_pw.hip b/thesis-pai-reconstruction_amd/csrc/gg_pw.hip
--- a/thesis-pai-reconstruction_amd/csrc/gg_pw.hip
+++ b/thesis-pai-reconstruction_amd/csrc/gg_pw.hip
@@ -20,7 +20,7 @@
 }
 
 bool pwx_ok(int dtype, const GG& g, const FwdArgs& a) {
-    if (dtype != PAI_BF16 || g.ntaps != 1 || g.nphase != 1 || g.S != 1 || g.OS != 1 || g.gslice) return false;
+    if (dtype != PAI_BF16 || g.wtaps != 1 || g.nphase != 1 || g.S != 1 || g.OS != 1 || g.gslice) return false;
     if (!pwx_shape_ok(g.Cin, g.Cout) || (g.C1 % 32) || (g.C2 % 32)) return false;
     if (g.D2 ? ((g.D1 % 8) || (g.D2 % 8) || g.D1 + g.D2 != g.Cout) : false) return false;
     if (g.relu1 || g.relu2 || a.yf32 || a.skip_d1) return false;
diff --git a/thesis-pai-reconstruction_amd/csrc/gg_tile.h b/thesis-pai-reconstruction_amd/csrc/gg_tile.h
--- a/thesis-pai-reconstruction_amd/csrc/gg_tile.h
+++ b/thesis-pai-reconstruction_amd/csrc/gg_tile.h
@@ -150,6 +150,7 @@
 }
 static inline bool patch_geo_raw(const GG& g, int th, PatchGeo* pg, int tw) {
     if ((g.OWg % tw) || (g.OHg % th)) return false;
+    if (g.pruned) return false;
     memset(pg, 0, sizeof(*pg));
     pg->TY = g.OHg / th;
     pg->TX = g.OWg / tw;
diff --git a/thesis-pai-reconstruction_amd/csrc/misc.hip b/thesis-pai-reconstruction_amd/csrc/misc.hip
--- a/thesis-pai-reconstruction_amd/csrc/misc.hip
+++ b/thesis-pai-reconstruction_amd/csrc/misc.hip
@@ -360,7 +360,7 @@
 __global__ __launch_bounds__(256) void adam_pack64_k(float* p, const float* g, float* m, float* v, int64_t numel,
                                                      int64_t w_off, int Cout, int taps, int Cin, bf16_t* wf, bf16_t* wd,
                                                      int ntiles, float lr_over_bc1, float beta1, float beta2, float omb1,
-                                                     float omb2, float eps, float inv_sqrt_bc2) {
+                                                     float omb2, float eps, float inv_sqrt_bc2, unsigned tap_mask) {
     __shared__ float tile[64][65];
     const int tid = threadIdx.x;
     if ((int)blockIdx.x >= ntiles) {
@@ -374,7 +374,13 @@
     }
     const int nci = Cin / 64, nco = Cout / 64;
     const int lb = blockIdx.x;
-    const int ci0 = (lb % nci) * 64, co0 = ((lb / nci) % nco) * 64, t = lb / (nci * nco);
+    const int ci0 = (lb % nci) * 64, co0 = ((lb / nci) % nco) * 64;
+    int t = lb / (nci * nco);
+    if (tap_mask) {
+        unsigned left = tap_mask;
+        for (int k = 0; k < t; ++k) left &= left - 1;
+        t = __builtin_ctz(left);
+    }
     const int q = tid & 15, r0 = tid >> 4;
 #pragma unroll
     for (int j = 0; j < 4; ++j) {
@@ -412,9 +418,9 @@
     }
 }
 
-extern "C" int pai_adam_pack(float* param, const float* grad, float* exp_avg, float* exp_avg_sq, int64_t numel,
-                             int64_t w_off, int Cout, int taps, int Cin, void* w_fwd, void* w_dgrad, float lr,
-                             float beta1, float beta2, float eps, int step_count, void* stream) {
+static int adam_pack_impl(float* param, const float* grad, float* exp_avg, float* exp_avg_sq, int64_t numel,
+                          int64_t w_off, int Cout, int taps, int Cin, void* w_fwd, void* w_dgrad, float lr,
+                          float beta1, float beta2, float eps, int step_count, unsigned tap_mask, void* stream) {
     PAI_CHECK(param && grad && exp_avg && exp_avg_sq && step_count >= 1 && (w_fwd || w_dgrad), "pai_adam_pack: bad arguments");
     PAI_CHECK(Cin > 0 && Cout > 0 && taps > 0 && (Cin % 64) == 0 && (Cout % 64) == 0,
               "pai_adam_pack: Cin=%d, Cout=%d must be multiples of 64 (bf16 packs)", Cin, Cout);
@@ -423,7 +429,7 @@
               (long long)w_off, (long long)(w_off + wn), (long long)numel);
     PAI_CHECK((((uintptr_t)param | (uintptr_t)grad | (uintptr_t)exp_avg | (uintptr_t)exp_avg_sq | (uintptr_t)w_fwd | (uintptr_t)w_dgrad) & 15) == 0,
               "pai_adam_pack: pointers must be 16-byte aligned");
-    const int64_t ntiles = (int64_t)(Cin / 64) * (Cout / 64) * taps;
+    const int64_t ntiles = (int64_t)(Cin / 64) * (Cout / 64) * (tap_mask ? __builtin_popcount(tap_mask) : taps);
     const int64_t rest = numel - wn;
     int64_t extra = (rest + 1023) / 1024;
     if (extra > 256) extra = 256;
@@ -434,9 +440,25 @@
     PAI_LAUNCH(adam_pack64_k, dim3((unsigned)(ntiles + extra)), dim3(256), 0, (hipStream_t)stream, param, grad,
                        exp_avg, exp_avg_sq, numel, w_off, Cout, taps, Cin, (bf16_t*)w_fwd, (bf16_t*)w_dgrad, (int)ntiles,
                        lr_over_bc1, beta1, beta2, (float)(1.0 - (double)beta1), (float)(1.0 - (double)beta2), eps,
-                       inv_sqrt_bc2);
-    PAI_LAUNCH_CHECK();
-    return 0;
+                       inv_sqrt_bc2, tap_mask);
+    PAI_LAUNCH_CHECK();
+    return 0;
+}
+
+extern "C" int pai_adam_pack(float* param, const float* grad, float* exp_avg, float* exp_avg_sq, int64_t numel,
+                             int64_t w_off, int Cout, int taps, int Cin, void* w_fwd, void* w_dgrad, float lr,
+                             float beta1, float beta2, float eps, int step_count, void* stream) {
+    return adam_pack_impl(param, grad, exp_avg, exp_avg_sq, numel, w_off, Cout, taps, Cin, w_fwd, w_dgrad, lr, beta1, beta2,
+                          eps, step_count, 0u, stream);
+}
+
+extern "C" int pai_adam_pack_taps(float* param, const float* grad, float* exp_avg, float* exp_avg_sq, int64_t numel,
+                                  int64_t w_off, int Cout, int taps, int Cin, void* w_fwd, void* w_dgrad, float lr,
+                                  float beta1, float beta2, float eps, int step_count, uint32_t tap_mask, void* stream) {
+    PAI_CHECK(taps > 0 && taps <= 32 && tap_mask != 0 && (taps == 32 || (tap_mask >> taps) == 0),
+              "pai_adam_pack_taps: mask 0x%x names no tap or one beyond the %d of the layer", tap_mask, taps);
+    return adam_pack_impl(param, grad, exp_avg, exp_avg_sq, numel, w_off, Cout, taps, Cin, w_fwd, w_dgrad, lr, beta1, beta2,
+                          eps, step_count, tap_mask, stream);
 }
 
 __global__ void adam_coeff_k(long long* step, float* coeff, float lr, float beta1, float beta2) {
@@ -639,6 +661,30 @@
     return 0;
 }
 
+__global__ __launch_bounds__(256) void zero_taps_k(float* dw, int Cout, int wtaps, int Cin, unsigned mask, int nlive) {
+    const int64_t total = (int64_t)Cout * nlive * Cin;
+    for (int64_t i = (int64_t)blockIdx.x * 256 + threadIdx.x; i < total; i += (int64_t)gridDim.x * 256) {
+        const int ci = (int)(i % Cin);
+        const int k = (int)((i / Cin) % nlive);
+        const int64_t co = i / ((int64_t)Cin * nlive);
+        unsigned left = mask;
+        for (int j = 0; j < k; ++j) left &= left - 1;
+        const int t = __builtin_ctz(left);
+        dw[(co * wtaps + t) * Cin + ci] = 0.f;
+    }
+}
+
+int launch_zero_taps(float* dw, int Cout, int wtaps, int Cin, unsigned mask, hipStream_t s) {
+    mask &= wtaps >= 32 ? ~0u : ((1u << wtaps) - 1u);
+    const int nlive = __builtin_popcount(mask);
+    if (!nlive) return 0;
+    int64_t blocks = ((int64_t)Cout * nlive * Cin + 1023) / 1024;
+    if (blocks > 1024) blocks = 1024;
+    PAI_LAUNCH(zero_taps_k, dim3((unsigned)blocks), dim3(256), 0, s, dw, Cout, wtaps, Cin, mask, nlive);
+    PAI_LAUNCH_CHECK();
+    return 0;
+}
+
 struct LerpChunk {
     float* d[ADAM_CHUNK];
     const float* s[ADAM_CHUNK];
diff --git a/thesis-pai-reconstruction_amd/engine.py b/thesis-pai-reconstruction_amd/engine.py
--- a/thesis-pai-reconstruction_amd/engine.py
+++ b/thesis-pai-reconstruction_amd/engine.py
@@ -60,6 +60,12 @@
         self.views = {}
         self.params = []
         self._zero_small = self._zero_all = None
+        self.tap_written = {}
+        self.tap_union = {}
+        self.taps_cleared = False
+        self._zero_seg = {}
+        self._no_skip = False
+        self._conv_cout = {}
         self._small = []
         for p, mod in entries:
             o, n = self.offsets[id(p)]
@@ -67,6 +73,7 @@
             if mod is not None and p.dim() == 4:
                 cin, cout = _cin_cout(mod)
                 v = seg.view(cout, 4, 4, cin).permute(_logical_perm(mod))
+                self._conv_cout[id(p)] = cout
                 if min(cin, cout) <= 2:
                     self._small.append(seg)
             else:
@@ -88,6 +95,7 @@
 
     def begin_backward(self, params, overwrite_weights: bool = False) -> bool:
         grads = [p.grad for p in params if p.requires_grad]
+        self.taps_cleared = False
         if all(g is None for g in grads):
             if overwrite_weights and self._small:
                 if self.flat.is_cuda:
@@ -96,18 +104,61 @@
                     self._zero_small()
                 else:
                     torch._foreach_zero_(self._small)
-            elif self.flat.is_cuda:
-                if self._zero_all is None:
-                    self._zero_all = ops.ZeroList([self.flat])
-                self._zero_all()
             else:
-                self.flat.zero_()
+                if self.flat.is_cuda:
+                    if self._zero_all is None:
+                        self._zero_all = ops.ZeroList([self.flat])
+                    self._zero_all()
+                else:
+                    self.flat.zero_()
+                for k in self.tap_written:
+                    self.tap_written[k] = 0
             return True
         for p in params:
             if p.requires_grad and (p.grad is None or p.grad.data_ptr() != self.view(p).data_ptr()):
                 raise ops.PaiError("gradient arena: parameters carry foreign .grad tensors; call "
                                    "zero_grad(set_to_none=True) before backward")
         return False
+
+    ALL_TAPS = 0xFFFF
+
+    def guard_dead_taps(self, p, d, overwriting: bool) -> int:
+        live = ops.conv_live_mask(d, 2)
+        k = id(p)
+        written = self.tap_written.get(k, self.ALL_TAPS)
+        if overwriting:
+            if written & ~live:
+                z = self._zero_seg.get(k)
+                if z is None:
+                    z = self._zero_seg[k] = ops.ZeroList([self.seg(p)])
+                z()
+                self.taps_cleared = True
+            written = live
+        else:
+            written |= live
+        self.tap_written[k] = written
+        self.tap_union[k] = self.tap_union.get(k, 0) | live
+        return live
+
+    def no_tap_skipping(self) -> None:
+        self._no_skip = True
+
+    def fold_loaded_moments(self) -> None:
+        for p in self.params:
+            if p.dim() != 4 or id(p) not in self.offsets:
+                continue
+            o, n = self.offsets[id(p)]
+            cout = self._conv_cout.get(id(p))
+            if cout is None:
+                continue
+            nz = (self.mflat[o:o + n] != 0) | (self.vflat[o:o + n] != 0)
+            taps = nz.view(cout, 16, n // (16 * cout)).any(dim=2).any(dim=0).tolist()
+            mask = sum(1 << t for t, on in enumerate(taps) if on)
+            self.tap_union[id(p)] = self.tap_union.get(id(p), 0) | mask
+
+    def skippable_taps(self, p, taps: int) -> int:
+        u = self.tap_union.get(id(p))
+        return 0 if (u is None or self._no_skip) else ((1 << taps) - 1) & ~u
 
     def attach(self, params) -> None:
         for p in params:
@@ -158,6 +209,9 @@
         self.dtype = None
         self.wf = None
         self.wd = None
+        self._full = []
+        self._repacked = None
+        self._spare_write_full = False
 
     def _stale(self, dtype):
         w = self.mod.weight
@@ -179,9 +233,13 @@
             if self.wd is None or self.wd.dtype != dtype:
                 self.wd = torch.empty(w.numel(), dtype=dtype, device=w.device)
             wd_out = self.wd
+        self._full = []
+        self._repacked = self.wf
         return w, cout, w.shape[2] * w.shape[3], cin, wf_out, wd_out
 
     def _mark(self, dtype):
+        if self._repacked is not None:
+            self._full, self._repacked = [self._repacked], None
         w = self.mod.weight
         self.version = (w._version, w.data_ptr(), self.gen[0])
         self.dtype = dtype
@@ -193,8 +251,17 @@
             self._spare = (torch.empty_like(self.wf), torch.empty_like(self.wd) if self.wd is not None else None)
         return self._spare
 
+    def spare_holds_all(self) -> bool:
+        sp = getattr(self, "_spare", None)
+        return sp is not None and any(t is sp[0] for t in self._full)
+
+    def note_spare_write(self, full: bool):
+        self._spare_write_full = bool(full)
+
     def commit(self):
         (self.wf, self.wd), self._spare = self._spare, (self.wf, self.wd)
+        if self._spare_write_full and not any(t is self.wf for t in self._full):
+            self._full.append(self.wf)
         self._mark(self.dtype)
 
     def commit_replayed(self):
@@ -390,13 +457,14 @@
         return self.enc_packs + self.dec_packs
 
     def _plan(self, N, H, W, dtype, device):
-        key = (N, H, W, dtype, str(device))
+        key = (N, H, W, dtype, str(device), ops.get_tunable("prune_taps", 1))
         if key in self._plans:
             return self._plans[key]
         L = self.L
         if H % (1 << L) or W % (1 << L):
             raise ops.PaiError(f"input {H}x{W} must be divisible by 2^{L}")
         P = {"N": N, "H": H, "W": W, "dtype": dtype, "device": device, "slots": [], "free": []}
+        P["wgrad_batch"] = (int(os.environ.get("PAI_WGRAD_BATCH", "3")), int(os.environ.get("PAI_WGRAD_BATCH_PIX", "1024")))
         eh = [H >> (i + 1) for i in range(L)]
         ew = [W >> (i + 1) for i in range(L)]
         P["eh"], P["ew"] = eh, ew
@@ -600,7 +668,7 @@
 
         conv_wgrad = ops.conv_wgrad_overwrite_w if fresh else ops.conv_wgrad
 
-        batch_n = int(os.environ.get("PAI_WGRAD_BATCH", "3"))
+        batch_n, batch_pix = P["wgrad_batch"]
         held = []
 
         def flush_held():
@@ -614,11 +682,12 @@
             def run():
                 thin = min(_cin_cout(conv)) <= 2
                 fn = ops.conv_wgrad if thin else conv_wgrad
+                A.guard_dead_taps(conv.weight, d, fresh and not thin)
                 fn(d, x1, x2, dz, A.seg(conv.weight), A.seg(conv.bias) if with_bias else None)
                 if thin:
                     side.mark_scratch()
                 done(conv.bias)
-            if batch_n > 1 and dz.numel() // max(1, conv.weight.shape[1] if isinstance(conv, nn.ConvTranspose2d) else conv.weight.shape[0]) <= int(os.environ.get("PAI_WGRAD_BATCH_PIX", "1024")):
+            if batch_n > 1 and dz.numel() // _cin_cout(conv)[1] <= batch_pix:
                 held.append(run)
                 if len(held) >= batch_n:
                     flush_held()
@@ -723,6 +792,7 @@
         flush_held()
         if not enc0_fused:
             with torch.cuda.stream(side.fork_tail()):
+                A.guard_dead_taps(conv0.weight, P["enc_desc"][0], fresh and min(_cin_cout(conv0)) > 2)
                 (ops.conv_wgrad if min(_cin_cout(conv0)) <= 2 else conv_wgrad)(
                     P["enc_desc"][0], S["x"], None, G["dz_enc"][0], A.seg(conv0.weight), A.seg(conv0.bias))
         side.join()
@@ -945,10 +1015,12 @@
                 break
             if need_params and k == 0:
                 with torch.cuda.stream(side.fork_tail()):
+                    A.guard_dead_taps(conv.weight, d, fresh and min(_cin_cout(conv)) > 2)
                     (ops.conv_wgrad if min(_cin_cout(conv)) <= 2 else conv_wgrad)(
                         d, S["xin"], S["yin"], self._du0(S), A.seg(conv.weight), A.seg(conv.bias))
             elif need_params:
                 with torch.cuda.stream(side.fork(d)):
+                    A.guard_dead_taps(conv.weight, self._wgrad_desc(P, k), fresh)
                     conv_wgrad(self._wgrad_desc(P, k), S["a"][k - 1], None, G["du"][k], A.seg(conv.weight), A.seg(conv.bias))
                     if hook is not None:
                         hook(A, A.end_of(conv.bias))
diff --git a/thesis-pai-reconstruction_amd/lib.py b/thesis-pai-reconstruction_amd/lib.py
--- a/thesis-pai-reconstruction_amd/lib.py
+++ b/thesis-pai-reconstruction_amd/lib.py
@@ -66,6 +66,7 @@
     "pai_bn_stats_buffer_rows": (_I, [_I]),
     "pai_conv_kernel_id": (_I, [_D, _I]),
     "pai_conv_kernel_name": (_I, [_D, _I, C.c_char_p, _I]),
+    "pai_conv_live_taps": (_I, [_D, _I, C.POINTER(C.c_uint32)]),
     "pai_set_workspace": (_I, [_P, _L]),
     "pai_conv_workspace_bytes": (_L, [_D, _I]),
     "pai_set_scratch": (_I, [_P, _L]),
@@ -157,6 +158,7 @@
     "pai_adam": (_I, [_P, _P, _P, _P, _L, _F, _F, _F, _F, _I, _P]),
     "pai_adam_dev": (_I, [_P, _P, _P, _P, _L, _F, _F, _F, _F, _P, _P, _P]),
     "pai_adam_pack": (_I, [_P, _P, _P, _P, _L, _L, _I, _I, _I, _P, _P, _F, _F, _F, _F, _I, _P]),
+    "pai_adam_pack_taps": (_I, [_P, _P, _P, _P, _L, _L, _I, _I, _I, _P, _P, _F, _F, _F, _F, _I, C.c_uint32, _P]),
     "pai_comm_unique_id": (_I, [_P]),
     "pai_comm_init": (_I, [_P, _I, _I, C.POINTER(_P)]),
     "pai_allreduce": (_I, [_P, _P, _L, _I, _P]),
diff --git a/thesis-pai-reconstruction_amd/ops.py b/thesis-pai-reconstruction_amd/ops.py
--- a/thesis-pai-reconstruction_amd/ops.py
+++ b/thesis-pai-reconstruction_amd/ops.py
@@ -96,6 +96,21 @@
     if L.load().pai_conv_kernel_name(C.byref(d), op, buf, 96) != 0:
         L.check(1, "pai_conv_kernel_name")
     return buf.value.decode()
+
+
+def conv_live_taps(d: ConvDesc, op: int):
+    m = (C.c_uint32 * 4)()
+    if L.load().pai_conv_live_taps(C.byref(d), int(op), m) < 0:
+        L.check(1, "pai_conv_live_taps")
+    out = tuple(int(v) for v in m)
+    return out[:1] if not any(out[1:]) else out
+
+
+def conv_live_mask(d: ConvDesc, op: int = 2) -> int:
+    u = 0
+    for v in conv_live_taps(d, op):
+        u |= v
+    return u
 
 
 def conv_flops(d: ConvDesc) -> int:
@@ -866,6 +881,20 @@
                                        _stream()), "pai_adam_pack")
 
 
+def adam_pack_taps(param, grad, exp_avg, exp_avg_sq, w_off, cout, taps, cin, w_fwd, w_dgrad, lr, beta1, beta2, eps, step,
+                   tap_mask):
+    dt = torch.bfloat16
+    live = bin(int(tap_mask)).count("1")
+    skipped = cout * (taps - live) * cin
+    packs = 2 * cout * live * cin * ((w_fwd is not None) + (w_dgrad is not None))
+    with _TimedBytes("adam", 28 * (param.numel() - skipped) + packs):
+        L.check(L.load().pai_adam_pack_taps(_p(param, torch.float32), _p(grad, torch.float32), _p(exp_avg, torch.float32),
+                                            _p(exp_avg_sq, torch.float32), param.numel(), int(w_off), cout, taps, cin,
+                                            _p(w_fwd, dt) if w_fwd is not None else None,
+                                            _p(w_dgrad, dt) if w_dgrad is not None else None, lr, beta1, beta2, eps, step,
+                                            int(tap_mask), _stream()), "pai_adam_pack_taps")
+
+
 def adam_dev(param, grad, exp_avg, exp_avg_sq, lr, beta1, beta2, eps, step_dev, coeff_dev):
     L.check(L.load().pai_adam_dev(_p(param, torch.float32), _p(grad, torch.float32), _p(exp_avg, torch.float32),
                                   _p(exp_avg_sq, torch.float32), param.numel(), lr, beta1, beta2, eps,
diff --git a/thesis-pai-reconstruction_amd/optim.py b/thesis-pai-reconstruction_amd/optim.py
--- a/thesis-pai-reconstruction_amd/optim.py
+++ b/thesis-pai-reconstruction_amd/optim.py
@@ -49,8 +49,16 @@
             for t in eng.pack_targets():
                 if t[5].dtype == torch.bfloat16 and t[5]._stale(t[5].dtype):
                     return None
+        taps = [ops.get_tunable("prune_taps", 1)]
+        if mode == "hook" and self._fuse_packs:
+            for t in eng.pack_targets():
+                skip = arena.skippable_taps(t[5].mod.weight, t[3])
+                taps.append(skip if (skip and t[5].spare_holds_all()) else 0)
         return (mode, float(g["lr"]), float(g["betas"][0]), float(g["betas"][1]), float(g["eps"]), arena.flat.data_ptr(),
-                arena.pflat.data_ptr(), tuple(ptrs))
+                arena.pflat.data_ptr(), tuple(ptrs), tuple(taps))
+
+    def plan_settled(self) -> bool:
+        return not self._engine.arena().taps_cleared
 
     def plan_commits(self):
         return list(self._last_commits)
@@ -120,9 +128,16 @@
             if spare is None:
                 continue
             end = inside[k + 1][0] if k + 1 < len(inside) else b
-            ops.adam_pack(arena.pflat[cur:end], arena.flat[cur:end], arena.mflat[cur:end], arena.vflat[cur:end], o - cur,
-                          cout, taps, cin, spare[0], spare[1], float(group["lr"]), float(group["betas"][0]),
-                          float(group["betas"][1]), float(group["eps"]), step)
+            args = (arena.pflat[cur:end], arena.flat[cur:end], arena.mflat[cur:end], arena.vflat[cur:end], o - cur,
+                    cout, taps, cin, spare[0], spare[1], float(group["lr"]), float(group["betas"][0]),
+                    float(group["betas"][1]), float(group["eps"]), step)
+            skip = arena.skippable_taps(pk.mod.weight, taps)
+            if skip and pk.spare_holds_all():
+                ops.adam_pack_taps(*args, ((1 << taps) - 1) & ~skip)
+                pk.note_spare_write(False)
+            else:
+                ops.adam_pack(*args)
+                pk.note_spare_write(True)
             self._packs_written.append(pk)
             cur = end
         self._adam_range(arena, cur, b, step)
@@ -196,6 +211,8 @@
                                    "not the arena's any more")
             if self._arena_steps:
                 self._mirror_state(self._engine.arena())
+            if getattr(self._engine, "_arena", None) is not None:
+                self._engine._arena.no_tap_skipping()
             return super().step(closure)
         group = self.param_groups[0]
         if streamed is not None:
@@ -243,6 +260,7 @@
                 v.copy_(st["exp_avg_sq"].to(v.device).reshape(v.shape))
                 st["exp_avg"], st["exp_avg_sq"] = m, v
                 st["step"] = torch.as_tensor(float(st["step"]), dtype=torch.float32)
+            arena.fold_loaded_moments()
         self._arena_steps = 0
         if self._dev_step is not None:
             self._dev_step.fill_(self.total_steps)
diff --git a/thesis-pai-reconstruction_amd/plan.py b/thesis-pai-reconstruction_amd/plan.py
--- a/thesis-pai-reconstruction_amd/plan.py
+++ b/thesis-pai-reconstruction_amd/plan.py
@@ -211,6 +211,8 @@
                              (", ..." if len(kinds) > 8 else "") + "): it cannot be replayed from a plan")
             self.plans.clear()
             return out
+        if not all(getattr(opt, "plan_settled", lambda: True)() for opt in m._all_optimizers()):
+            return out
         after = self._total_steps()
         if any(b - a != 1 for a, b in zip(rec.step0, after)):
             self.disabled = "an optimizer did not take exactly one step in the recorded call"
```

Result: no change. 11880 images/s (median of 6 runs) (+0.9%).
